# yudaohai666/Sparse_Matrix_Tuning

Hardware: AMD Instinct MI355X
Metric: train tokens/sec + peak GB HBM, LLaMA-3-8B SMT(0.71%) at 1/2/4/8 MI355X (higher is better)
Workload: dtype bf16

## Files before the change

### include/smt_attention.h

```cpp
#ifndef SMT_ATTENTION_H
#define SMT_ATTENTION_H

#include <stdint.h>
#include <hip/hip_runtime_api.h>

#ifdef __cplusplus
extern "C" {
#endif

#define SMT_ATTN_HEAD_DIM 128

typedef struct smt_attn_tensor {
    void* ptr;
    int64_t sb, sh, ss;
} smt_attn_tensor;

typedef struct smt_attn_shape {
    int32_t B, Hq, Hkv, S;
    float scale;
    int32_t dtype;
} smt_attn_shape;

const char* smt_attn_last_error(void);

int smt_attn_fwd(const smt_attn_tensor* q, const smt_attn_tensor* k, const smt_attn_tensor* v,
                 const smt_attn_tensor* o, float* lse, const smt_attn_shape* shape, hipStream_t stream);

int smt_attn_bwd(const smt_attn_tensor* q, const smt_attn_tensor* k, const smt_attn_tensor* v,
                 const smt_attn_tensor* o, const smt_attn_tensor* d_o, const float* lse, float* delta_ws,
                 const smt_attn_tensor* dq, const smt_attn_tensor* dk, const smt_attn_tensor* dv,
                 const smt_attn_shape* shape, hipStream_t stream);

int smt_attn_fwd_kmask(const smt_attn_tensor* q, const smt_attn_tensor* k, const smt_attn_tensor* v,
                       const smt_attn_tensor* o, float* lse, const uint64_t* key_mask, int64_t key_mask_ld,
                       const smt_attn_shape* shape, hipStream_t stream);
int smt_attn_bwd_kmask(const smt_attn_tensor* q, const smt_attn_tensor* k, const smt_attn_tensor* v,
                       const smt_attn_tensor* o, const smt_attn_tensor* d_o, const float* lse, float* delta_ws,
                       const smt_attn_tensor* dq, const smt_attn_tensor* dk, const smt_attn_tensor* dv,
                       const uint64_t* key_mask, int64_t key_mask_ld, const smt_attn_shape* shape,
                       hipStream_t stream);

#ifdef __cplusplus
}
#endif
#endif
```

### sparse_matrix_tuning_amd/_hip.py

```python
from __future__ import annotations

import ctypes
import os
import threading
from typing import NamedTuple, Optional, Sequence

import torch

from . import build as _build

BLOCK = 256
TILE_ELEMS = BLOCK * BLOCK

DTYPE_BF16, DTYPE_FP32, DTYPE_FP16 = 0, 1, 2
SCORE_MEAN_ABS, SCORE_ABS_MEAN, SCORE_L1, SCORE_L2 = 0, 1, 2, 3
ADAM_DEEPSPEED, ADAM_TORCH = 0, 1

_DT = {torch.bfloat16: DTYPE_BF16, torch.float32: DTYPE_FP32, torch.float16: DTYPE_FP16}
ABI_VERSION = 13

ABI_FUNCTIONS = (
    "smt_last_error", "smt_abi_version", "smt_wgrad_workspace_bytes", "smt_tile_wgrad", "smt_wgrad_batch_workspace_bytes",
    "smt_tile_wgrad_batch", "smt_wgrad_seq_workspace_bytes", "smt_tile_wgrad_batch_seq", "smt_colblock_gather", "smt_tile_scatter_t",
    "smt_tile_gather", "smt_tile_scatter", "smt_grad_accumulate", "smt_block_score",
    "smt_sq_norm", "smt_adamw_step", "smt_adamw_multi",
    "smt_mx_quant_cols", "smt_wgrad_mx_workspace_bytes", "smt_tile_wgrad_mx", "smt_tile_wgrad_mx_batch",
    "smt_row_gather", "smt_row_scatter", "smt_column_gather", "smt_act_accumulate",
    "smt_channel_score_workspace_bytes", "smt_channel_score",
    "smt_channel_mean_aten_workspace_bytes", "smt_channel_mean_aten",
    "smt_model_ops_last_error", "smt_rmsnorm_fwd", "smt_rmsnorm_bwd_waves", "smt_rmsnorm_bwd", "smt_rmsnorm_bwd_add_dw",
    "smt_add_rmsnorm_fwd", "smt_rmsnorm_bwd_add", "smt_colblock_recompute",
    "smt_rope_fwd", "smt_rope_bwd", "smt_swiglu_fwd", "smt_swiglu_bwd", "smt_ce_fwd", "smt_ce_bwd",
    "smt_attn_last_error", "smt_attn_fwd", "smt_attn_bwd", "smt_attn_fwd_kmask", "smt_attn_bwd_kmask",
    "smt_fp8_last_error", "smt_quant_rows_e4m3", "smt_quant_cols_t_e4m3", "smt_quant_rows_cat_e4m3",
    "smt_swiglu_fwd_quant_e4m3", "smt_swiglu_bwd_quant_e4m3", "smt_swiglu_bwd_quant_e4m3_packed",
    "smt_rmsnorm_fwd_quant_e4m3",
    "smt_rmsnorm_bwd_add_quant_e4m3",
)


class TileDesc(ctypes.Structure):
    _fields_ = [("weight", ctypes.c_void_p), ("ld_weight", ctypes.c_int64),
                ("row_block", ctypes.c_int32), ("col_block", ctypes.c_int32),
                ("flat_offset", ctypes.c_int64)]


class WgradModule(ctypes.Structure):
    _fields_ = [("grad_out", ctypes.c_void_p), ("x", ctypes.c_void_p), ("ld_grad_out", ctypes.c_int64),
                ("ld_x", ctypes.c_int64), ("x_block_stride", ctypes.c_int64), ("grad_tiles", ctypes.c_void_p),
                ("accumulate", ctypes.c_int32), ("operand_dtype", ctypes.c_int32)]


class WgradMxModule(ctypes.Structure):
    _fields_ = [("qg", ctypes.c_void_p), ("sg", ctypes.c_void_p), ("qx", ctypes.c_void_p), ("sx", ctypes.c_void_p),
                ("grad_tiles", ctypes.c_void_p), ("accumulate", ctypes.c_int32), ("reserved", ctypes.c_int32)]


WGRAD_MAX_MODULES = 16


class AccumEntry(ctypes.Structure):
    _fields_ = [("src", ctypes.c_void_p), ("dst", ctypes.c_void_p), ("n", ctypes.c_int64),
                ("chunk_begin", ctypes.c_int64), ("src_dtype", ctypes.c_int32), ("assign", ctypes.c_int32)]


class ScoreEntry(ctypes.Structure):
    _fields_ = [("src", ctypes.c_void_p), ("ld", ctypes.c_int64), ("d1", ctypes.c_int32),
                ("d2", ctypes.c_int32), ("block_begin", ctypes.c_int64), ("out", ctypes.c_void_p),
                ("strategy", ctypes.c_int32), ("pad_", ctypes.c_int32)]


class AdamWArgs(ctypes.Structure):
    _fields_ = [("lr", ctypes.c_float), ("beta1", ctypes.c_float), ("beta2", ctypes.c_float),
                ("eps", ctypes.c_float), ("weight_decay", ctypes.c_float),
                ("bias_correction1", ctypes.c_float), ("bias_correction2", ctypes.c_float),
                ("max_grad_norm", ctypes.c_float), ("grad_scale", ctypes.c_float),
                ("mode", ctypes.c_int32), ("grad_dtype", ctypes.c_int32),
                ("param_dtype", ctypes.c_int32), ("reserved", ctypes.c_int32)]


class AdamWTensor(ctypes.Structure):
    _fields_ = [("grad", ctypes.c_void_p), ("master", ctypes.c_void_p), ("exp_avg", ctypes.c_void_p),
                ("exp_avg_sq", ctypes.c_void_p), ("param", ctypes.c_void_p), ("n", ctypes.c_int64)]


class RopeTensor(ctypes.Structure):
    _fields_ = [("inp", ctypes.c_void_p), ("out", ctypes.c_void_p),
                ("in_sb", ctypes.c_int64), ("in_sh", ctypes.c_int64), ("in_ss", ctypes.c_int64),
                ("out_sb", ctypes.c_int64), ("out_sh", ctypes.c_int64), ("out_ss", ctypes.c_int64),
                ("heads", ctypes.c_int32), ("pad_", ctypes.c_int32)]


class QuantSrc(ctypes.Structure):
    _fields_ = [("ptr", ctypes.c_void_p), ("ld", ctypes.c_int64), ("cols", ctypes.c_int32), ("pad_", ctypes.c_int32)]


class AttnTensor(ctypes.Structure):
    _fields_ = [("ptr", ctypes.c_void_p), ("sb", ctypes.c_int64), ("sh", ctypes.c_int64), ("ss", ctypes.c_int64)]


class AttnShape(ctypes.Structure):
    _fields_ = [("B", ctypes.c_int32), ("Hq", ctypes.c_int32), ("Hkv", ctypes.c_int32), ("S", ctypes.c_int32),
                ("scale", ctypes.c_float), ("dtype", ctypes.c_int32)]


ACC_CHUNK = 4096
_lock = threading.Lock()
_lib: Optional[ctypes.CDLL] = None

_P, _I64, _I32, _SZ = ctypes.c_void_p, ctypes.c_int64, ctypes.c_int32, ctypes.c_size_t
_SIGS = {
    "smt_last_error": (ctypes.c_char_p, []),
    "smt_abi_version": (ctypes.c_int, []),
    "smt_wgrad_workspace_bytes": (_SZ, [_I64, _I32]),
    "smt_tile_wgrad": (ctypes.c_int, [_P, _I64, _P, _I64, _I64, _I64, _P, _P, _I32, _P, _I32, _I32, _P, _SZ, _P]),
    "smt_wgrad_batch_workspace_bytes": (_SZ, [_I64, _I32]),
    "smt_tile_wgrad_batch": (ctypes.c_int, [ctypes.POINTER(WgradModule), _I32, _I64, _P, _P, _I32, _I32, _P, _SZ, _P]),
    "smt_wgrad_seq_workspace_bytes": (_SZ, [_I64, _I64, _I32]),
    "smt_tile_wgrad_batch_seq": (ctypes.c_int, [ctypes.POINTER(WgradModule), _I32, _I64, _I64, _P, _P, _I32, _I32, _P,
                                                _SZ, _P]),
    "smt_colblock_gather": (ctypes.c_int, [_P, _I64, _I64, _P, _I32, _P, _P]),
    "smt_tile_scatter_t": (ctypes.c_int, [_P, _I32, _P, _P]),
    "smt_tile_gather": (ctypes.c_int, [_P, _I64, _I32, _P, _I32, _P, _P]),
    "smt_tile_scatter": (ctypes.c_int, [_P, _I64, _I32, _P, _I32, _P, _P]),
    "smt_grad_accumulate": (ctypes.c_int, [_P, _I32, _I64, _P]),
    "smt_block_score": (ctypes.c_int, [_P, _I32, _I64, _P]),
    "smt_sq_norm": (ctypes.c_int, [_P, _I64, _P, _I32, _P, _P]),
    "smt_adamw_step": (ctypes.c_int, [_P, _P, _P, _P, _P, _P, _I32, _I64, _P, ctypes.POINTER(AdamWArgs), _P]),
    "smt_adamw_multi": (ctypes.c_int, [_P, _P, _I32, _I64, _P, ctypes.POINTER(AdamWArgs), _P]),
    "smt_mx_quant_cols": (ctypes.c_int, [_P, _I64, _I64, _P, _I32, _I64, _P, _P, _P]),
    "smt_wgrad_mx_workspace_bytes": (_SZ, [_I64, _I32]),
    "smt_tile_wgrad_mx": (ctypes.c_int, [_P, _P, _P, _P, _I64, _P, _P, _I32, _P, _I32, _I32, _P, _SZ, _P]),
    "smt_tile_wgrad_mx_batch": (ctypes.c_int, [ctypes.POINTER(WgradMxModule), _I32, _I64, _P, _P, _I32, _I32, _P, _SZ, _P]),
    "smt_row_gather": (ctypes.c_int, [_P, _I64, _I32, _I64, _P, _I32, _P, _I64, _P]),
    "smt_row_scatter": (ctypes.c_int, [_P, _I64, _I32, _I64, _P, _I32, _P, _I64, _P]),
    "smt_column_gather": (ctypes.c_int, [_P, _I64, _I64, _I64, _P, _I32, _P, _I64, _P]),
    "smt_act_accumulate": (ctypes.c_int, [_P, _I32, _I64, _I64, _I32, _I32, _I32, _P, _I32, _P]),
    "smt_channel_score_workspace_bytes": (_SZ, [_I32, _I32]),
    "smt_channel_score": (ctypes.c_int, [_P, _I32, _I32, _I32, _I32, _P, _SZ, _P, _P]),
    "smt_channel_mean_aten_workspace_bytes": (_SZ, [_I32, _I32]),
    "smt_channel_mean_aten": (ctypes.c_int, [_P, _I32, _I32, _I32, _P, _SZ, _P, _P]),
    "smt_attn_last_error": (ctypes.c_char_p, []),
    "smt_attn_fwd": (ctypes.c_int, [ctypes.POINTER(AttnTensor)] * 4 + [_P, ctypes.POINTER(AttnShape), _P]),
    "smt_attn_bwd": (ctypes.c_int, [ctypes.POINTER(AttnTensor)] * 5 + [_P, _P] + [ctypes.POINTER(AttnTensor)] * 3
                     + [ctypes.POINTER(AttnShape), _P]),
    "smt_attn_fwd_kmask": (ctypes.c_int, [ctypes.POINTER(AttnTensor)] * 4 + [_P, _P, _I64, ctypes.POINTER(AttnShape), _P]),
    "smt_attn_bwd_kmask": (ctypes.c_int, [ctypes.POINTER(AttnTensor)] * 5 + [_P, _P] + [ctypes.POINTER(AttnTensor)] * 3
                           + [_P, _I64, ctypes.POINTER(AttnShape), _P]),
    "smt_model_ops_last_error": (ctypes.c_char_p, []),
    "smt_rmsnorm_fwd": (ctypes.c_int, [_P, _I64, _P, _P, _I64, _P, _I64, _I32, ctypes.c_float, _I32, _P]),
    "smt_rmsnorm_bwd_waves": (ctypes.c_int, [_I64]),
    "smt_add_rmsnorm_fwd": (ctypes.c_int, [_P, _I64, _P, _I64, _P, _P, _I64, _P, _I64, _P, _I64, _I32, ctypes.c_float,
                                           _I32, _P]),
    "smt_rmsnorm_bwd_add": (ctypes.c_int, [_P, _I64, _P, _I64, _P, _P, _P, _I64, _P, _I64, _I64, _I32, _I32, _P]),
    "smt_rmsnorm_bwd": (ctypes.c_int, [_P, _I64, _P, _I64, _P, _P, _P, _I64, _P, _P, _I64, _I32, _I32, _P]),
    "smt_rmsnorm_bwd_add_dw": (ctypes.c_int, [_P, _I64, _P, _I64, _P, _P, _P, _I64, _P, _I64, _P, _P, _I64, _I32, _I32, _P]),
    "smt_rope_fwd": (ctypes.c_int, [ctypes.POINTER(RopeTensor), ctypes.POINTER(RopeTensor), _P, _P, _I64, _I64, _I64, _I32,
                                    _I32, _I32, _P]),
    "smt_rope_bwd": (ctypes.c_int, [ctypes.POINTER(RopeTensor), ctypes.POINTER(RopeTensor), _P, _P, _I64, _I64, _I64, _I32,
                                    _I32, _I32, _P]),
    "smt_swiglu_fwd": (ctypes.c_int, [_P, _P, _P, _I64, _I32, _P]),
    "smt_colblock_recompute": (ctypes.c_int, [_I32, _P, _I64, _P, _I64, _P, _P, _I64, _P, _I32, _P, _I32, _P]),
    "smt_swiglu_bwd": (ctypes.c_int, [_P, _P, _P, _P, _P, _I64, _I32, _P]),
    "smt_ce_fwd": (ctypes.c_int, [_P, _I64, _P, _I64, _I64, _I64, _P, _P, _I32, _P]),
    "smt_ce_bwd": (ctypes.c_int, [_P, _I64, _P, _P, _P, _I64, _I64, _I64, _P, _I64, _I32, _P]),
    "smt_fp8_last_error": (ctypes.c_char_p, []),
    "smt_quant_rows_e4m3": (ctypes.c_int, [_P, _I64, _I64, _I32, _P, _I32, _P, _I64, _P, _P]),
    "smt_quant_cols_t_e4m3": (ctypes.c_int, [_P, _I64, _I32, _I32, _P, _I32, _P, _I64, _P, _P]),
    "smt_quant_rows_cat_e4m3": (ctypes.c_int, [ctypes.POINTER(QuantSrc), _I32, _I64, _P, _I64, _P, _P]),
    "smt_rmsnorm_fwd_quant_e4m3": (ctypes.c_int, [_P, _I64, _P, _I64, _P, _P, _I64, _P, _I64, _P, _P, _I64, _P,
                                                   _I64, _I32, ctypes.c_float, _P]),
    "smt_rmsnorm_bwd_add_quant_e4m3": (ctypes.c_int, [_P, _I64, _P, _I64, _P, _P, _P, _I64, _P, _I64, _P, _I64, _P,
                                                       _I64, _I32, _P]),
    "smt_swiglu_fwd_quant_e4m3": (ctypes.c_int, [_P, _P, _I64, _I32, _P, _I64, _P, _P, _P]),
    "smt_swiglu_bwd_quant_e4m3": (ctypes.c_int, [_P, _P, _P, _I64, _I32, _P, _I64, _P, _P, _P, _P]),
    "smt_swiglu_bwd_quant_e4m3_packed": (ctypes.c_int, [_P, _P, _P, _I64, _I32, _P, _I64, _P, _P, _P, _I64, _P, _P,
                                                         _I64, _P]),
}


def dtype_code16(dtype: torch.dtype, what: str) -> int:
    if dtype == torch.bfloat16:
        return DTYPE_BF16
    if dtype == torch.float16:
        return DTYPE_FP16
    raise RuntimeError(f"{what}: bf16 or fp16 tensors only (got {dtype})")


def lib_path() -> str:
    return _build.LIB_PATH


def load(build_if_missing: bool = False) -> ctypes.CDLL:
    global _lib
    if _lib is not None:
        return _lib
    with _lock:
        if _lib is None:
            if build_if_missing and _build.is_stale():
                _build.build()
            path = os.environ.get("SMT_HIP_LIB") or _build.LIB_PATH
            if not os.path.exists(path):
                raise RuntimeError(
                    f"SMT HIP library not built ({path}); run `python -c 'import __graft_entry__ as g; g.build()'`"
                    " or `python -m sparse_matrix_tuning_amd.build`")
            lib = ctypes.CDLL(path)
            for name, (res, args) in _SIGS.items():
                fn = getattr(lib, name)
                fn.restype = res
                fn.argtypes = args
            if lib.smt_abi_version() != ABI_VERSION:
                raise RuntimeError(f"{path} implements C ABI v{lib.smt_abi_version()}, this package v{ABI_VERSION}: "
                                   "rebuild it (`python -c 'import __graft_entry__ as g; g.build()'`)")
            _lib = lib
    return _lib


def _check(rc: int, what: str) -> None:
    if rc != 0:
        lib = load()
        if what.startswith(("smt_quant", "smt_swiglu_fwd_quant", "smt_swiglu_bwd_quant")):
            err = lib.smt_fp8_last_error
        elif what.startswith(("smt_rmsnorm", "smt_add_rmsnorm", "smt_rope", "smt_swiglu", "smt_ce_",
                              "smt_colblock_recompute")):
            err = lib.smt_model_ops_last_error
        elif what.startswith("smt_attn"):
            err = lib.smt_attn_last_error
        else:
            err = lib.smt_last_error
        raise RuntimeError(f"{what} failed (status {rc}): {err().decode(errors='replace')}")


def _require_device(*tensors: torch.Tensor) -> torch.device:
    dev = None
    for t in tensors:
        if t is None:
            continue
        if t.device.type != "cuda":
            raise RuntimeError(
                f"SMT HIP path needs tensors on a ROCm device, got {t.device} "
                "(there is no CPU fallback: the CPU restatement lives in oracle/ and is test-only)")
        if dev is None:
            dev = t.device
        elif t.device != dev:
            raise RuntimeError(f"tensors on different devices: {dev} vs {t.device}")
    return dev


def _stream(dev: torch.device) -> int:
    return torch.cuda.current_stream(dev).cuda_stream


def _ptr(t: Optional[torch.Tensor]) -> Optional[int]:
    return None if t is None else t.data_ptr()


def _device_table(structs: Sequence[ctypes.Structure], cls, dev: torch.device) -> torch.Tensor:
    n = len(structs)
    arr = (cls * n)(*structs)
    host = torch.frombuffer(bytearray(bytes(arr)), dtype=torch.uint8)
    return host.to(dev, non_blocking=False)


def tile_table(index_list: Sequence[Sequence[int]], device: torch.device) -> torch.Tensor:
    flat = [int(v) for rc in index_list for v in (rc[0], rc[1])]
    return torch.tensor(flat, dtype=torch.int32).view(-1, 2).to(device)


def schedule_order(index_list: Sequence[Sequence[int]]) -> list:
    rows = {int(rc[0]) for rc in index_list}
    cols = {int(rc[1]) for rc in index_list}
    if len(cols) <= len(rows):
        key = lambda i: (int(index_list[i][1]), int(index_list[i][0]))
    else:
        key = lambda i: (int(index_list[i][0]), int(index_list[i][1]))
    return sorted(range(len(index_list)), key=key)


def order_table(index_list: Sequence[Sequence[int]], device: torch.device) -> torch.Tensor:
    return torch.tensor(schedule_order(index_list), dtype=torch.int32).to(device)


def wgrad_workspace_bytes(T: int, n_tiles: int) -> int:
    return int(load().smt_wgrad_workspace_bytes(int(T), int(n_tiles)))


def tile_wgrad(grad_out2d: torch.Tensor, x: torch.Tensor, tile_rc: torch.Tensor, out: torch.Tensor,
               accumulate: bool = False, order: Optional[torch.Tensor] = None,
               seq_len: Optional[int] = None) -> torch.Tensor:
    if grad_out2d.dtype != torch.bfloat16 and grad_out2d.shape[0] == 0:
        if not accumulate:
            out.zero_()
        return out
    if seq_len or grad_out2d.dtype != torch.bfloat16:
        n = tile_rc.shape[0]
        tab = torch.zeros(n, 4, dtype=torch.int32, device=tile_rc.device)
        tab[:, 1:3] = tile_rc
        tab[:, 3] = torch.arange(n, dtype=torch.int32, device=tile_rc.device)
        tile_wgrad_batch([(grad_out2d, x, out, accumulate)], tab, order, seq_len=seq_len)
        return out
    dev = _require_device(grad_out2d, x, tile_rc, out, order)
    if grad_out2d.dtype != torch.bfloat16 or x.dtype != torch.bfloat16:
        raise NotImplementedError(f"tile_wgrad: bf16 operands only (got {grad_out2d.dtype}, {x.dtype})")
    if out.dtype not in (torch.bfloat16, torch.float32) or not out.is_contiguous():
        raise ValueError("tile_wgrad: out must be a contiguous bf16/fp32 tensor")
    n = tile_rc.shape[0]
    if out.numel() != n * TILE_ELEMS:
        raise ValueError(f"tile_wgrad: out has {out.numel()} elements, expected {n * TILE_ELEMS}")
    T = grad_out2d.shape[0]
    if x.dim() == 3:
        if not x.is_contiguous() or x.shape[1:] != (T, BLOCK):
            raise ValueError("tile_wgrad: a block-major x must be a contiguous [n_cb, T, 256] tensor")
        ld_x, xbs = BLOCK, T * BLOCK
    else:
        if x.dim() != 2 or x.shape[0] != T or x.stride(1) != 1:
            raise ValueError("tile_wgrad: x must be [T, features] with unit feature stride")
        ld_x, xbs = x.stride(0), BLOCK
    if grad_out2d.stride(1) != 1:
        raise ValueError("tile_wgrad: grad_out must be [T, features] with unit feature stride")
    ws_bytes = wgrad_workspace_bytes(T, n)
    ws = torch.empty(max(ws_bytes, 16), dtype=torch.uint8, device=dev)
    if order is not None and (order.dtype != torch.int32 or order.numel() != n):
        raise ValueError("tile_wgrad: order must be int32 [n_tiles]")
    rc = load().smt_tile_wgrad(_ptr(grad_out2d), grad_out2d.stride(0), _ptr(x), ld_x, xbs, T,
                               _ptr(tile_rc), _ptr(order), n, _ptr(out), _DT[out.dtype], int(bool(accumulate)),
                               _ptr(ws), ws_bytes, _stream(dev))
    _check(rc, "smt_tile_wgrad")
    return out


def _wgrad_x_layout(x: torch.Tensor, T: int, what: str):
    if x.dim() == 3:
        if not x.is_contiguous() or x.shape[1:] != (T, BLOCK):
            raise ValueError(f"{what}: a block-major x must be a contiguous [n_cb, T, 256] tensor")
        return BLOCK, T * BLOCK
    if x.dim() != 2 or x.shape[0] != T or x.stride(1) != 1:
        raise ValueError(f"{what}: x must be [T, features] with unit feature stride")
    return x.stride(0), BLOCK


def tile_wgrad_batch(items: Sequence[tuple], tile_tab: torch.Tensor, order: Optional[torch.Tensor] = None,
                     seq_len: Optional[int] = None) -> None:
    if not items:
        return
    if len(items) > WGRAD_MAX_MODULES:
        raise ValueError(f"tile_wgrad_batch: {len(items)} modules > {WGRAD_MAX_MODULES}")
    dev = _require_device(tile_tab, order, *[t for it in items for t in it[:3]])
    T = items[0][0].shape[0]
    out_dtype = items[0][2].dtype
    op_dtype = items[0][0].dtype
    if op_dtype not in (torch.bfloat16, torch.float16, torch.float32):
        raise NotImplementedError(f"tile_wgrad_batch: operands bf16, fp16 or fp32 (got {op_dtype})")
    if out_dtype not in (op_dtype, torch.float32) or out_dtype == torch.float64:
        raise ValueError(f"tile_wgrad_batch: {op_dtype} operands give {op_dtype} or fp32 tiles (got {out_dtype})")
    mods = (WgradModule * len(items))()
    for i, (g, x, out, acc) in enumerate(items):
        if g.dtype != op_dtype or x.dtype != op_dtype:
            raise NotImplementedError(f"tile_wgrad_batch: one operand dtype per launch (got {g.dtype}, {x.dtype})")
        if g.dim() != 2 or g.shape[0] != T or g.stride(1) != 1:
            raise ValueError("tile_wgrad_batch: every grad_out must be [T, features] with the same T")
        if out.dtype != out_dtype or not out.is_contiguous():
            raise ValueError("tile_wgrad_batch: outputs must be contiguous and of one dtype")
        ld_x, xbs = _wgrad_x_layout(x, T, "tile_wgrad_batch")
        mods[i] = WgradModule(_ptr(g), _ptr(x), g.stride(0), ld_x, xbs, _ptr(out), int(bool(acc)), _DT[op_dtype])
    if tile_tab.dtype != torch.int32 or tile_tab.dim() != 2 or tile_tab.shape[1] != 4:
        raise ValueError("tile_wgrad_batch: tile_tab must be int32 [n, 4]")
    n = tile_tab.shape[0]
    if order is not None and (order.dtype != torch.int32 or order.numel() != n):
        raise ValueError("tile_wgrad_batch: order must be int32 [n_tiles]")
    if seq_len:
        if T % int(seq_len):
            raise ValueError(f"tile_wgrad_batch: T = {T} is not a whole number of {seq_len}-row samples")
        ws_bytes = int(load().smt_wgrad_seq_workspace_bytes(T, int(seq_len), n))
        ws = torch.empty(max(ws_bytes, 16), dtype=torch.uint8, device=dev)
        rc = load().smt_tile_wgrad_batch_seq(mods, len(items), T, int(seq_len), _ptr(tile_tab), _ptr(order), n,
                                             _DT[out_dtype], _ptr(ws), ws_bytes, _stream(dev))
        _check(rc, "smt_tile_wgrad_batch_seq")
        return
    ws_bytes = int(load().smt_wgrad_batch_workspace_bytes(T, n))
    ws = torch.empty(max(ws_bytes, 16), dtype=torch.uint8, device=dev)
    rc = load().smt_tile_wgrad_batch(mods, len(items), T, _ptr(tile_tab), _ptr(order), n, _DT[out_dtype],
                                     _ptr(ws), ws_bytes, _stream(dev))
    _check(rc, "smt_tile_wgrad_batch")


def wgrad_batch_table(module_tiles: Sequence[Sequence[Sequence[int]]], device: torch.device):
    rows, order = [], []
    for m, tl in enumerate(module_tiles):
        base = len(rows)
        rows.extend((m, int(r), int(c), k) for k, (r, c) in enumerate(tl))
        order.extend(base + i for i in schedule_order(tl))
    flat = [v for row in rows for v in row]
    tab = torch.tensor(flat, dtype=torch.int32).view(-1, 4).to(device)
    return tab, torch.tensor(order, dtype=torch.int32).to(device)


def colblock_gather(x2d: torch.Tensor, col_blocks: torch.Tensor) -> torch.Tensor:
    dev = _require_device(x2d, col_blocks)
    if x2d.dim() != 2 or x2d.stride(1) != 1 or x2d.element_size() != 2:
        raise ValueError("colblock_gather: x must be a 2-D row-major 16-bit tensor")
    n_cb = col_blocks.numel()
    out = torch.empty(n_cb, x2d.shape[0], BLOCK, dtype=x2d.dtype, device=dev)
    rc = load().smt_colblock_gather(_ptr(x2d), x2d.stride(0), x2d.shape[0], _ptr(col_blocks), n_cb, _ptr(out),
                                    _stream(dev))
    _check(rc, "smt_colblock_gather")
    return out


RECOMPUTE_RMSNORM, RECOMPUTE_SWIGLU = 0, 1


def colblock_recompute(op: int, a2d: torch.Tensor, col_blocks: torch.Tensor, b2d: torch.Tensor = None,
                       weight: torch.Tensor = None, rstd: torch.Tensor = None) -> torch.Tensor:
    dev = _require_device(a2d, col_blocks, b2d, weight, rstd)
    for t in (a2d, b2d):
        if t is not None and (t.dim() != 2 or t.stride(1) != 1 or t.dtype not in (torch.bfloat16, torch.float16)):
            raise ValueError("colblock_recompute: operands must be 2-D row-major bf16 / fp16")
    if b2d is not None and b2d.dtype != a2d.dtype or weight is not None and weight.dtype != a2d.dtype:
        raise ValueError("colblock_recompute: operands of one dtype")
    if b2d is not None and b2d.shape != a2d.shape:
        raise ValueError("colblock_recompute: gate and up shapes differ")
    if rstd is not None and (rstd.dtype != torch.float32 or rstd.numel() != a2d.shape[0] or not rstd.is_contiguous()):
        raise ValueError("colblock_recompute: rstd must be a contiguous fp32 [T]")
    if weight is not None and (weight.numel() != a2d.shape[1] or not weight.is_contiguous()):
        raise ValueError("colblock_recompute: weight must be a contiguous [cols]")
    n_cb = col_blocks.numel()
    out = torch.empty(n_cb, a2d.shape[0], BLOCK, dtype=a2d.dtype, device=dev)
    rc = load().smt_colblock_recompute(op, _ptr(a2d), a2d.stride(0), _ptr(b2d) if b2d is not None else None,
                                       b2d.stride(0) if b2d is not None else 0,
                                       _ptr(weight) if weight is not None else None,
                                       _ptr(rstd) if rstd is not None else None, a2d.shape[0], _ptr(col_blocks), n_cb,
                                       _ptr(out), dtype_code16(a2d.dtype, "colblock_recompute"), _stream(dev))
    _check(rc, "smt_colblock_recompute")
    return out


class MxBlocks(NamedTuple):
    q: torch.Tensor
    scales: torch.Tensor
    T: int

    @property
    def ldq(self) -> int:
        return self.q.shape[1] * 64


def mx_ld(T: int) -> int:
    return (T + 63) // 64 * 64


def mx_quant_cols(x2d: torch.Tensor, blocks: torch.Tensor) -> MxBlocks:
# ... 304 lines not shown
```

### sparse_matrix_tuning_amd/build.py

```python
from __future__ import annotations

import os
import shutil
import subprocess
import sys

PKG_DIR = os.path.dirname(os.path.abspath(__file__))
REPO_DIR = os.path.dirname(PKG_DIR)
SRCS = [os.path.join(PKG_DIR, "csrc", n) for n in ("smt_kernels.hip", "llama_kernels.hip", "attn_kernels.hip",
                                                   "fp8_kernels.hip")]
HEADERS = [os.path.join(REPO_DIR, "include", n) for n in ("smt_hip.h", "smt_model_ops.h", "smt_attention.h",
                                                          "smt_fp8.h")]
HEADERS += [os.path.join(PKG_DIR, "csrc", n) for n in ("silu_math.h", "fp8_math.h")]
LIB_DIR = os.path.join(PKG_DIR, "_lib")
LIB_PATH = os.path.join(LIB_DIR, "libsmt_hip.so")
ARCH = "gfx950"


def hipcc() -> str:
    for cand in (os.environ.get("HIPCC"), "/opt/rocm/bin/hipcc", shutil.which("hipcc")):
        if cand and os.path.exists(cand):
            return cand
    raise RuntimeError("hipcc not found (set HIPCC or install ROCm under /opt/rocm)")


def is_stale() -> bool:
    if not os.path.exists(LIB_PATH):
        return True
    t = os.path.getmtime(LIB_PATH)
    return any(os.path.getmtime(p) > t for p in (*SRCS, *HEADERS, __file__))


FILE_FLAGS = {"attn_kernels.hip": ["-fno-slp-vectorize"]}


def compile_commands(out: str, defines=()) -> list:
    base = [hipcc(), f"--offload-arch={ARCH}", "-O3", "-std=c++17", "-fPIC", "-Wall", "-Wno-unused-function",
            "-I", os.path.join(REPO_DIR, "include"), *defines]
    objs, cmds = [], []
    for src in SRCS:
        obj = out + "." + os.path.splitext(os.path.basename(src))[0] + ".o"
        objs.append(obj)
        cmds.append(base + FILE_FLAGS.get(os.path.basename(src), []) + ["-c", "-o", obj, src])
    link = [hipcc(), f"--offload-arch={ARCH}", "-shared", "-fPIC", "-o", out, *objs]
    return cmds, link, objs


def run_build(out: str, defines=(), verbose: bool = False) -> None:
    cmds, link, objs = compile_commands(out, defines)
    if verbose:
        for c in cmds + [link]:
            print(" ".join(c), file=sys.stderr)
    procs = [subprocess.Popen(c, stdout=subprocess.PIPE, stderr=subprocess.PIPE, text=True) for c in cmds]
    errs = []
    for c, p in zip(cmds, procs):
        so, se = p.communicate()
        if p.returncode != 0:
            errs.append(f"{' '.join(c)}\n{so}\n{se}")
    if not errs:
        res = subprocess.run(link, capture_output=True, text=True)
        if res.returncode != 0:
            errs.append(f"{' '.join(link)}\n{res.stdout}\n{res.stderr}")
    for o in objs:
        if os.path.exists(o):
            os.remove(o)
    if errs:
        raise RuntimeError("hipcc failed:\n" + "\n".join(errs))


def build(force: bool = False, verbose: bool = False) -> str:
    if not force and not is_stale():
        return LIB_PATH
    os.makedirs(LIB_DIR, exist_ok=True)
    tmp = f"{LIB_PATH}.tmp{os.getpid()}"
    run_build(tmp, verbose=verbose)
    os.replace(tmp, LIB_PATH)
    return LIB_PATH


if __name__ == "__main__":
    print(build(force="--force" in sys.argv, verbose=True))
```

### sparse_matrix_tuning_amd/csrc/attn_kernels.hip

```cpp
#include <hip/hip_runtime.h>
#include <stdarg.h>
#include <stdint.h>
#include <stdio.h>
#include <stdlib.h>

#include <utility>

#include "smt_attention.h"
#include "smt_hip.h"

namespace {

thread_local char g_err[512] = "";

int fail(int code, const char* fmt, ...) {
    va_list ap;
    va_start(ap, fmt);
    vsnprintf(g_err, sizeof(g_err), fmt, ap);
    va_end(ap);
    return code;
}

int check_launch(const char* what) {
    hipError_t e = hipGetLastError();
    if (e != hipSuccess) return fail(-4, "%s: %s", what, hipGetErrorString(e));
    return 0;
}

typedef __bf16 bf16x8_t __attribute__((ext_vector_type(8)));
typedef __bf16 bf16x2_t __attribute__((ext_vector_type(2)));
typedef _Float16 f16x8_t __attribute__((ext_vector_type(8)));
typedef _Float16 f16x2_t __attribute__((ext_vector_type(2)));
typedef float f32x2_t __attribute__((ext_vector_type(2)));
typedef short s16x4_t __attribute__((ext_vector_type(4)));
typedef short s16x8_t __attribute__((ext_vector_type(8)));
typedef float f32x16_t __attribute__((ext_vector_type(16)));
typedef uint32_t u32x4_t __attribute__((ext_vector_type(4)));
typedef __attribute__((address_space(3))) s16x4_t lds_s16x4_t;

constexpr int kD = 128;
constexpr int kRowB = 256;
constexpr float kNegInf = -__builtin_huge_valf();

struct Tns {
    const uint16_t* p;
    int64_t sb, sh, ss;
};

__device__ __forceinline__ uint32_t swz(uint32_t row) { return ((row & 3u) << 2) | ((row >> 2) & 3u); }
__device__ __forceinline__ uint32_t lds_off(uint32_t row, uint32_t byte) { return row * kRowB + (byte ^ (swz(row) << 4)); }

__device__ __forceinline__ bf16x8_t row_frag(const uint8_t* img, uint32_t row, uint32_t byte) {
    return *reinterpret_cast<const bf16x8_t*>(img + lds_off(row, byte));
}

struct TrLane {
    uint32_t krow, feat_byte;
};
__device__ __forceinline__ TrLane tr_lane(int lane) {
    const int gi = lane >> 4, q = (lane >> 2) & 3, p = lane & 3;
    return TrLane{8u * (gi >> 1) + q, 2u * (16u * (gi & 1) + 4u * p)};
}
__device__ __forceinline__ bf16x8_t tr_frag(const uint8_t* img, TrLane tl, uint32_t row0, uint32_t col0) {
    const uint32_t r = row0 + tl.krow, byte = 2u * col0 + tl.feat_byte;
    s16x4_t lo = __builtin_amdgcn_ds_read_tr16_b64_v4i16((lds_s16x4_t*)(img + lds_off(r, byte)));
    s16x4_t hi = __builtin_amdgcn_ds_read_tr16_b64_v4i16((lds_s16x4_t*)(img + lds_off(r + 4, byte)));
    const s16x8_t both = __builtin_shufflevector(lo, hi, 0, 1, 2, 3, 4, 5, 6, 7);
    return __builtin_bit_cast(bf16x8_t, both);
}

template <int F>
__device__ __forceinline__ f32x16_t mfma(bf16x8_t a, bf16x8_t b, f32x16_t c) {
    if constexpr (F == SMT_DTYPE_FP16)
        return __builtin_amdgcn_mfma_f32_32x32x16_f16(__builtin_bit_cast(f16x8_t, a), __builtin_bit_cast(f16x8_t, b), c,
                                                      0, 0, 0);
    else return __builtin_amdgcn_mfma_f32_32x32x16_bf16(a, b, c, 0, 0, 0);
}

constexpr bool kPkFwd = false, kPkDq = true, kPkDkv = true;
template <bool PK>
__device__ __forceinline__ f32x2_t fma2(f32x2_t a, f32x2_t b, f32x2_t c) {
    if (PK) return __builtin_elementwise_fma(a, b, c);
    return f32x2_t{__builtin_fmaf(a.x, b.x, c.x), __builtin_fmaf(a.y, b.y, c.y)};
}
template <bool PK>
__device__ __forceinline__ f32x2_t submul2(f32x2_t a, f32x2_t d, f32x2_t p) {
    if (PK) return (a - d) * p;
    return f32x2_t{(a.x - d.x) * p.x, (a.y - d.y) * p.y};
}
template <bool PK>
__device__ __forceinline__ f32x2_t add2(f32x2_t a, f32x2_t b) {
    if (PK) return a + b;
    return f32x2_t{a.x + b.x, a.y + b.y};
}

template <int F>
__device__ __forceinline__ uint32_t pk16(float a, float b) {
    f32x2_t v = {a, b};
    if constexpr (F == SMT_DTYPE_FP16) return __builtin_bit_cast(uint32_t, __builtin_convertvector(v, f16x2_t));
    else return __builtin_bit_cast(uint32_t, __builtin_convertvector(v, bf16x2_t));
}
template <int F>
__device__ __forceinline__ float lo16(uint32_t w) {
    if constexpr (F == SMT_DTYPE_FP16) return (float)__builtin_bit_cast(_Float16, (uint16_t)(w & 0xffffu));
    else return __uint_as_float(w << 16);
}
template <int F>
__device__ __forceinline__ float hi16(uint32_t w) {
    if constexpr (F == SMT_DTYPE_FP16) return (float)__builtin_bit_cast(_Float16, (uint16_t)(w >> 16));
    else return __uint_as_float(w & 0xffff0000u);
}

__device__ __forceinline__ float other_half_max(float x) {
    auto r = __builtin_amdgcn_permlane32_swap(__float_as_uint(x), __float_as_uint(x), false, false);
    return fmaxf(__uint_as_float(r[0]), __uint_as_float(r[1]));
}
__device__ __forceinline__ float halves_sum(float x) {
    auto r = __builtin_amdgcn_permlane32_swap(__float_as_uint(x), __float_as_uint(x), false, false);
    return __uint_as_float(r[0]) + __uint_as_float(r[1]);
}

template <int F>
__device__ __forceinline__ void pack_b_frags(const float (&p)[16], bf16x8_t& f0, bf16x8_t& f1) {
    uint32_t w[8];
#pragma unroll
    for (int i = 0; i < 8; ++i) w[i] = pk16<F>(p[2 * i], p[2 * i + 1]);
#pragma unroll
    for (int h = 0; h < 2; ++h) {
        auto a = __builtin_amdgcn_permlane32_swap(w[4 * h + 0], w[4 * h + 2], false, false);
        auto b = __builtin_amdgcn_permlane32_swap(w[4 * h + 1], w[4 * h + 3], false, false);
        u32x4_t v = {a[0], b[0], a[1], b[1]};
        if (h == 0) f0 = __builtin_bit_cast(bf16x8_t, v);
        else f1 = __builtin_bit_cast(bf16x8_t, v);
    }
}

__device__ __forceinline__ int xcd_logical(int bid, int total) {
    const int q8 = total >> 3, r8 = total & 7, xcd = bid & 7;
    return (xcd < r8 ? xcd * (q8 + 1) : r8 * (q8 + 1) + (xcd - r8) * q8) + (bid >> 3);
}

__device__ __forceinline__ uint32_t opaque(uint32_t v) {
    asm volatile("" : "+v"(v));
    return v;
}
template <int IMG>
__device__ __forceinline__ bf16x8_t rowx(const uint8_t* lds, uint32_t lo, int ks) {
    return *reinterpret_cast<const bf16x8_t*>(lds + IMG + (lo ^ (uint32_t)(ks << 5)));
}
template <int IMG>
__device__ __forceinline__ bf16x8_t trx(const uint8_t* lds, uint32_t t0, uint32_t t4, int kq, int dt) {
    const uint32_t x = (uint32_t)(dt << 6);
    s16x4_t lo = __builtin_amdgcn_ds_read_tr16_b64_v4i16((lds_s16x4_t*)(lds + IMG + 4096 * kq + (t0 ^ x)));
    s16x4_t hi = __builtin_amdgcn_ds_read_tr16_b64_v4i16((lds_s16x4_t*)(lds + IMG + 4096 * kq + (t4 ^ x)));
    const s16x8_t both = __builtin_shufflevector(lo, hi, 0, 1, 2, 3, 4, 5, 6, 7);
    return __builtin_bit_cast(bf16x8_t, both);
}

typedef __attribute__((address_space(3))) uint8_t lds_u8_t;
__device__ __forceinline__ void dma16(__amdgpu_buffer_rsrc_t rsrc, uint32_t lds_base, int voff) {
    uint32_t keep;
    asm volatile("s_mov_b32 %0, m0\n\ts_mov_b32 m0, %3\n\ts_nop 0\n\t"
                 "buffer_load_dwordx4 %1, %2, 0 offen lds\n\ts_mov_b32 m0, %0"
                 : "=&s"(keep) : "v"(voff), "s"(rsrc), "s"(lds_base) : "memory");
}
__device__ __forceinline__ uint32_t lds_addr(const uint8_t* p) { return (uint32_t)(uintptr_t)(const lds_u8_t*)p; }
__device__ __forceinline__ __amdgpu_buffer_rsrc_t uniform_rsrc(const void* base, int64_t bytes) {
    const uint64_t a = (uint64_t)(uintptr_t)base;
    const uint32_t lo = __builtin_amdgcn_readfirstlane((uint32_t)a);
    const uint32_t hi = __builtin_amdgcn_readfirstlane((uint32_t)(a >> 32));
    const int n = __builtin_amdgcn_readfirstlane((int)bytes);
    return __builtin_amdgcn_make_buffer_rsrc((void*)(((uint64_t)hi << 32) | lo), 0, n, 0x00020000);
}
__device__ __forceinline__ void vm_wait_all() { asm volatile("s_waitcnt vmcnt(0)" ::: "memory"); }
__device__ __forceinline__ void vm_wait_all_known() { __builtin_amdgcn_s_waitcnt(0x0F70); }
__device__ __forceinline__ void vm_wait_upto(int n) {
    if (n >= 8) asm volatile("s_waitcnt vmcnt(8)" ::: "memory");
    else if (n >= 6) asm volatile("s_waitcnt vmcnt(6)" ::: "memory");
    else if (n >= 4) asm volatile("s_waitcnt vmcnt(4)" ::: "memory");
    else if (n >= 3) asm volatile("s_waitcnt vmcnt(3)" ::: "memory");
    else if (n >= 2) asm volatile("s_waitcnt vmcnt(2)" ::: "memory");
    else asm volatile("s_waitcnt vmcnt(0)" ::: "memory");
}

__device__ __forceinline__ void dma_rows(__amdgpu_buffer_rsrc_t rsrc, int64_t ss, uint32_t img, int img_row0,
                                         int row0, int pieces, int lane) {
#pragma unroll 4
    for (int i = 0; i < pieces; ++i) {
        const int r = row0 + 4 * i + (lane >> 4);
        const uint32_t ir = (uint32_t)(r - img_row0);
        const uint32_t ch = (uint32_t)(lane & 15) ^ swz(ir);
        const uint32_t base = __builtin_amdgcn_readfirstlane(img + (uint32_t)(r - (lane >> 4) - img_row0) * kRowB);
        dma16(rsrc, base, (int)((int64_t)r * ss * 2 + ch * 16));
    }
}

constexpr int kFwdQW = 32, kFwdWaves = 4, kFwdQB = kFwdQW * kFwdWaves, kKV = 64;
constexpr int kDqWaves = 4, kDqQB = kFwdQW * kDqWaves;
constexpr int kTileB = kKV * kRowB;

__device__ __forceinline__ bool key_bit(uint64_t w, int key) { return (w >> (key & 63)) & 1ull; }

struct FwdArgs {
    Tns q, k, v;
    uint16_t* o;
    int64_t o_sb, o_sh, o_ss;
    float* lse;
    const uint64_t* kmask;
    int64_t kmask_ld;
    int B, Hq, Hkv, S;
    float sl2;
};

struct PairTask {
    int b, hk, hh, blk[2], n;
};
__device__ __forceinline__ PairTask pair_task(int L, int nblk, int G, int Hkv) {
    const int npair = (nblk + 1) / 2;
    const int per_group = G * npair;
    const int grp = L / per_group;
    const int rem = L - grp * per_group;
    const int p = rem / G;
    PairTask t;
    t.b = grp / Hkv;
    t.hk = grp % Hkv;
    t.hh = rem % G;
    t.blk[0] = nblk - 1 - p;
    t.blk[1] = p;
    t.n = (t.blk[1] == t.blk[0]) ? 1 : 2;
    return t;
}

constexpr float kFwdThr = 8.f;


__device__ __forceinline__ float max3f(float a, float b, float c) {
    float r;
    asm("v_max3_f32 %0, %1, %2, %3" : "=v"(r) : "v"(a), "v"(b), "v"(c));
    return r;
}

template <bool KMASK, int F>
struct FwdLean {
    const FwdArgs& a;
    uint8_t* lds;
    __amdgpu_buffer_rsrc_t rk, rv;
    uint32_t lds0;
    const uint64_t* km;
    bf16x8_t qf[8];
    f32x16_t o[4];
    float m_run, l_run;
    int qw, qrow, hi, l32, wave, lane, nt, last;
    TrLane tl;

    __device__ __forceinline__ FwdLean(const FwdArgs& a_, uint8_t* lds_) : a(a_), lds(lds_) {}

    __device__ __forceinline__ void issue(int t) {
        const uint32_t slot = lds0 + (uint32_t)((t & 1) * 2 * kTileB);
        dma_rows(rk, a.k.ss, slot, t * kKV, t * kKV + 16 * wave, 4, lane);
        dma_rows(rv, a.v.ss, slot + kTileB, t * kKV, t * kKV + 16 * wave, 4, lane);
    }

    template <int SLOT, bool DIAG_>
    __device__ __forceinline__ void compute(int t, bool DIAG) {
        const uint8_t* K = lds + SLOT * 2 * kTileB;
        const uint8_t* V = K + kTileB;
        const int k0 = t * kKV;
        f32x16_t sc[2];
        bf16x8_t kf[3][2];
#pragma unroll
        for (int p = 0; p < 2; ++p)
#pragma unroll
            for (int j = 0; j < 2; ++j) kf[p][j] = row_frag(K, 32 * j + l32, 32 * p + 16 * hi);
#pragma unroll
        for (int ks = 0; ks < 8; ++ks) {
            if (ks + 2 < 8) {
#pragma unroll
                for (int j = 0; j < 2; ++j) kf[(ks + 2) % 3][j] = row_frag(K, 32 * j + l32, 32 * (ks + 2) + 16 * hi);
            }
            __builtin_amdgcn_sched_barrier(0);
#pragma unroll
            for (int j = 0; j < 2; ++j) sc[j] = mfma<F>(kf[ks % 3][j], qf[ks], ks ? sc[j] : f32x16_t{});
            __builtin_amdgcn_sched_barrier(0);
        }
        bf16x8_t vf[3];
        vf[0] = tr_frag(V, tl, 0, 0);
        vf[1] = tr_frag(V, tl, 16, 0);
        float x[32];
#pragma unroll
        for (int j = 0; j < 2; ++j)
#pragma unroll
            for (int i = 0; i < 16; ++i) x[16 * j + i] = sc[j][i];
        if (DIAG) {
#pragma unroll
            for (int i = 0; i < 32; ++i) {
                const int key = k0 + 32 * (i >> 4) + (i & 3) + 8 * ((i & 15) >> 2) + 4 * hi;
                if (key > qrow) x[i] = kNegInf;
            }
        }
        if (KMASK) {
            const uint64_t w = km[k0 >> 6];
            if (~w != 0ull) {
#pragma unroll
                for (int i = 0; i < 32; ++i) {
                    const int key = k0 + 32 * (i >> 4) + (i & 3) + 8 * ((i & 15) >> 2) + 4 * hi;
                    if (!key_bit(w, key)) x[i] = kNegInf;
                }
            }
        }
        float mx[11];
#pragma unroll
        for (int i = 0; i < 10; ++i) mx[i] = max3f(x[3 * i], x[3 * i + 1], x[3 * i + 2]);
        mx[10] = max3f(x[30], x[31], mx[0]);
        mx[0] = max3f(mx[0], mx[1], mx[2]);
        mx[3] = max3f(mx[3], mx[4], mx[5]);
        mx[6] = max3f(mx[6], mx[7], mx[8]);
        mx[9] = max3f(mx[9], mx[10], mx[0]);
        const float m_tile = other_half_max(max3f(mx[3], mx[6], mx[9])) * a.sl2;
        const bool move = m_tile > m_run + kFwdThr;
        const float m_new = move ? m_tile : m_run;
        const float alpha = move ? __builtin_amdgcn_exp2f(m_run - m_new) : 1.f;
        const float m_use = (KMASK && m_new == kNegInf) ? 0.f : m_new;
        const f32x2_t sl2v = {a.sl2, a.sl2}, mv = {-m_use, -m_use};
        f32x2_t sm[16];
#pragma unroll
        for (int i = 0; i < 16; ++i) {
            const f32x2_t e = fma2<kPkFwd>(f32x2_t{x[2 * i], x[2 * i + 1]}, sl2v, mv);
            x[2 * i] = __builtin_amdgcn_exp2f(e.x);
            x[2 * i + 1] = __builtin_amdgcn_exp2f(e.y);
            sm[i] = f32x2_t{x[2 * i], x[2 * i + 1]};
        }
#pragma unroll
        for (int w = 8; w >= 1; w >>= 1)
#pragma unroll
            for (int i = 0; i < w; ++i) sm[i] = add2<kPkFwd>(sm[i], sm[i + w]);
        l_run = l_run * alpha + (sm[0].x + sm[0].y);
        m_run = m_new;
        if (__builtin_amdgcn_ballot_w64(move) != 0) {
#pragma unroll
            for (int dt = 0; dt < 4; ++dt)
#pragma unroll
                for (int i = 0; i < 16; ++i) o[dt][i] *= alpha;
        }
        bf16x8_t pf[4];
        pack_b_frags<F>(*reinterpret_cast<const float(*)[16]>(&x[0]), pf[0], pf[1]);
        pack_b_frags<F>(*reinterpret_cast<const float(*)[16]>(&x[16]), pf[2], pf[3]);
#pragma unroll
        for (int n = 0; n < 16; ++n) {
            if (n + 2 < 16) vf[(n + 2) % 3] = tr_frag(V, tl, 16 * ((n + 2) & 3), 32 * ((n + 2) >> 2));
            __builtin_amdgcn_sched_barrier(0);
            o[n >> 2] = mfma<F>(vf[n % 3], pf[n & 3], o[n >> 2]);
            __builtin_amdgcn_sched_barrier(0);
        }
    }

    template <int SLOT>
    __device__ __forceinline__ void tile(int t) {
        if (t + 1 < nt) issue(t + 1);
        if (t <= last) compute<SLOT, true>(t, t == last);
        vm_wait_all();
        __syncthreads();
    }

    __device__ __forceinline__ void run(int b, int h, int hk, int qb) {
        const int tid = threadIdx.x;
        lane = tid & 63;
        wave = __builtin_amdgcn_readfirstlane(tid >> 6);
        hi = lane >> 5;
        l32 = lane & 31;
        const int q0 = qb * kFwdQB;
        qw = q0 + wave * kFwdQW;
        qrow = qw + l32;
        const uint16_t* qp = a.q.p + b * a.q.sb + h * a.q.sh;
        const uint16_t* kp = a.k.p + b * a.k.sb + hk * a.k.sh;
        const uint16_t* vp = a.v.p + b * a.v.sb + hk * a.v.sh;
        km = KMASK ? a.kmask + (int64_t)b * a.kmask_ld : nullptr;
#pragma unroll
        for (int ks = 0; ks < 8; ++ks) {
            if (qrow < a.S) qf[ks] = *reinterpret_cast<const bf16x8_t*>(qp + qrow * a.q.ss + 16 * ks + 8 * hi);
            else qf[ks] = __builtin_bit_cast(bf16x8_t, u32x4_t{0u, 0u, 0u, 0u});
        }
        const int kv_end = min(a.S, q0 + kFwdQB);
        nt = (kv_end + kKV - 1) / kKV;
        last = min(nt - 1, qw / kKV);
        rk = uniform_rsrc(kp, (int64_t)a.S * a.k.ss * 2);
        rv = uniform_rsrc(vp, (int64_t)a.S * a.v.ss * 2);
        lds0 = lds_addr(lds);
        tl = tr_lane(lane);
#pragma unroll
        for (int dt = 0; dt < 4; ++dt)
#pragma unroll
            for (int i = 0; i < 16; ++i) o[dt][i] = 0.f;
        m_run = kNegInf;
        l_run = 0.f;
        issue(0);
        vm_wait_all();
        vm_wait_all_known();
        __syncthreads();
        for (int t = 0; t < nt; t += 2) {
            tile<0>(t);
            if (t + 1 < nt) tile<1>(t + 1);
        }
        const float l_tot = halves_sum(l_run);
        if (qrow < a.S) {
            const float inv = (KMASK && !(l_tot > 0.f)) ? 0.f : 1.f / l_tot;
            uint16_t* op = a.o + b * a.o_sb + h * a.o_sh + (int64_t)qrow * a.o_ss;
#pragma unroll
            for (int dt = 0; dt < 4; ++dt)
#pragma unroll
                for (int g = 0; g < 4; ++g) {
                    const int d = 32 * dt + 8 * g + 4 * hi;
                    uint2 w;
                    w.x = pk16<F>(o[dt][4 * g] * inv, o[dt][4 * g + 1] * inv);
                    w.y = pk16<F>(o[dt][4 * g + 2] * inv, o[dt][4 * g + 3] * inv);
                    *reinterpret_cast<uint2*>(op + d) = w;
                }
            if (hi == 0)
                a.lse[((int64_t)b * a.Hq + h) * a.S + qrow] =
                    (KMASK && !(l_tot > 0.f)) ? __builtin_huge_valf() : m_run + __log2f(l_tot);
        }
    }
};

template <bool KMASK, int F>
__global__ __launch_bounds__(64 * kFwdWaves, 2)
void attn_fwd_kernel(FwdArgs a) {
    __shared__ __attribute__((aligned(16))) uint8_t lds[2 * 2 * kTileB];
    const int nqb = (a.S + kFwdQB - 1) / kFwdQB;
    const int G = a.Hq / a.Hkv;
    const int total = nqb * a.Hq * a.B;
    const int L = xcd_logical(blockIdx.x, total);
    const int per_group = G * nqb;
    const int grp = L / per_group;
    const int rem = L - grp * per_group;
    const int hk = grp % a.Hkv;
    FwdLean<KMASK, F> fl(a, lds);
    fl.run(grp / a.Hkv, hk * G + rem % G, hk, nqb - 1 - rem / G);
}


struct DqArgs {
    Tns q, k, v, dout, o;
    uint16_t* dq;
    int64_t dq_sb, dq_sh, dq_ss;
    const float* lse;
    float* delta;
    const uint64_t* kmask;
    int64_t kmask_ld;
    int B, Hq, Hkv, S;
    float sl2, scale;
};

template <bool KMASK, int F>
struct DqLean {
    const DqArgs& a;
    uint8_t* lds;
    bf16x8_t qf[8], df[8];
    f32x16_t dq[4];
    float lse, dlt;
    const uint64_t* km;
    __amdgpu_buffer_rsrc_t rk, rv;
    uint32_t lds0, lo_row, lo_t0, lo_t4;
    int lane, wave, hi, l32, qw, qrow, nt, last;

    __device__ __forceinline__ DqLean(const DqArgs& a_, uint8_t* lds_) : a(a_), lds(lds_) {}

    __device__ __forceinline__ void issue(int t) {
        const uint32_t slot = lds0 + (uint32_t)((t & 1) * 2 * kTileB);
        constexpr int rows_w = kKV / kDqWaves;
        dma_rows(rk, a.k.ss, slot, t * kKV, t * kKV + rows_w * wave, rows_w / 4, lane);
        dma_rows(rv, a.v.ss, slot + kTileB, t * kKV, t * kKV + rows_w * wave, rows_w / 4, lane);
    }

    template <int SLOT>
    __device__ __forceinline__ void compute(int t, bool diag) {
        constexpr int KI = SLOT * 2 * kTileB, VI = KI + kTileB;
        const int k0 = t * kKV;
        const uint32_t lr = opaque(lo_row);
        constexpr int KH = KI + 32 * kRowB, VH = VI + 32 * kRowB;
        f32x16_t s[2], dp[2];
        s[0] = mfma<F>(rowx<KI>(lds, lr, 0), qf[0], f32x16_t{});
        s[1] = mfma<F>(rowx<KH>(lds, lr, 0), qf[0], f32x16_t{});
        dp[0] = mfma<F>(rowx<VI>(lds, lr, 0), df[0], f32x16_t{});
        dp[1] = mfma<F>(rowx<VH>(lds, lr, 0), df[0], f32x16_t{});
#pragma unroll
        for (int ks = 1; ks < 8; ++ks) {
            s[0] = mfma<F>(rowx<KI>(lds, lr, ks), qf[ks], s[0]);
            s[1] = mfma<F>(rowx<KH>(lds, lr, ks), qf[ks], s[1]);
            dp[0] = mfma<F>(rowx<VI>(lds, lr, ks), df[ks], dp[0]);
            dp[1] = mfma<F>(rowx<VH>(lds, lr, ks), df[ks], dp[1]);
            if (ks & 1) __builtin_amdgcn_sched_barrier(0);
        }
        float pr[32];
        const f32x2_t sl2v = {a.sl2, a.sl2}, lv = {-lse, -lse}, dv = {dlt, dlt};
#pragma unroll
        for (int i = 0; i < 32; i += 2) {
            const int j = i >> 4, ii = i & 15;
            const f32x2_t e = fma2<kPkDq>(f32x2_t{s[j][ii], s[j][ii + 1]}, sl2v, lv);
            pr[i] = __builtin_amdgcn_exp2f(e.x);
            pr[i + 1] = __builtin_amdgcn_exp2f(e.y);
        }
        if (diag) {
#pragma unroll
            for (int i = 0; i < 32; ++i) {
                const int key = k0 + 32 * (i >> 4) + (i & 3) + 8 * ((i & 15) >> 2) + 4 * hi;
                if (key > qrow) pr[i] = 0.f;
            }
        }
        if (KMASK) {
            const uint64_t w = km[k0 >> 6];
            if (~w != 0ull) {
#pragma unroll
                for (int i = 0; i < 32; ++i) {
                    const int key = k0 + 32 * (i >> 4) + (i & 3) + 8 * ((i & 15) >> 2) + 4 * hi;
                    if (!key_bit(w, key)) pr[i] = 0.f;
                }
            }
        }
#pragma unroll
        for (int i = 0; i < 32; i += 2) {
            const int j = i >> 4, ii = i & 15;
            const f32x2_t r = submul2<kPkDq>(f32x2_t{dp[j][ii], dp[j][ii + 1]}, dv, f32x2_t{pr[i], pr[i + 1]});
            pr[i] = r.x;
            pr[i + 1] = r.y;
        }
        bf16x8_t sf[4];
        pack_b_frags<F>(*reinterpret_cast<const float(*)[16]>(&pr[0]), sf[0], sf[1]);
        pack_b_frags<F>(*reinterpret_cast<const float(*)[16]>(&pr[16]), sf[2], sf[3]);
        const uint32_t t0 = opaque(lo_t0), t4 = opaque(lo_t4);
#pragma unroll
        for (int dt = 0; dt < 4; ++dt) {
#pragma unroll
            for (int kst = 0; kst < 4; ++kst) dq[dt] = mfma<F>(trx<KI>(lds, t0, t4, kst, dt), sf[kst], dq[dt]);
            __builtin_amdgcn_sched_barrier(0);
        }
    }

    template <int SLOT>
    __device__ __forceinline__ void tile(int t) {
        if (t + 1 < nt) issue(t + 1);
        if (t <= last) compute<SLOT>(t, t == last);
        vm_wait_all();
        __syncthreads();
    }

    __device__ __forceinline__ void run(int b, int h, int hk, int qb) {
        const int tid = threadIdx.x;
        lane = tid & 63;
        wave = __builtin_amdgcn_readfirstlane(tid >> 6);
        hi = lane >> 5;
        l32 = lane & 31;
        const int q0 = qb * kDqQB;
        qw = q0 + wave * kFwdQW;
        qrow = qw + l32;
        const bool qvalid = qrow < a.S;
        const uint16_t* qp = a.q.p + b * a.q.sb + h * a.q.sh;
        const uint16_t* dop = a.dout.p + b * a.dout.sb + h * a.dout.sh;
        const uint16_t* kp = a.k.p + b * a.k.sb + hk * a.k.sh;
        const uint16_t* vp = a.v.p + b * a.v.sb + hk * a.v.sh;
        km = KMASK ? a.kmask + (int64_t)b * a.kmask_ld : nullptr;
#pragma unroll
        for (int ks = 0; ks < 8; ++ks) {
            if (qvalid) {
                qf[ks] = *reinterpret_cast<const bf16x8_t*>(qp + qrow * a.q.ss + 16 * ks + 8 * hi);
                df[ks] = *reinterpret_cast<const bf16x8_t*>(dop + qrow * a.dout.ss + 16 * ks + 8 * hi);
            } else {
                qf[ks] = __builtin_bit_cast(bf16x8_t, u32x4_t{0u, 0u, 0u, 0u});
                df[ks] = qf[ks];
            }
        }
        const int64_t srow = ((int64_t)b * a.Hq + h) * a.S + (qvalid ? qrow : 0);
        lse = qvalid ? a.lse[srow] : 0.f;
        {
            const uint16_t* op = a.o.p + b * a.o.sb + h * a.o.sh;
            float part = 0.f;
#pragma unroll
            for (int ks = 0; ks < 8; ++ks) {
                const u32x4_t ov = qvalid ? *reinterpret_cast<const u32x4_t*>(op + qrow * a.o.ss + 16 * ks + 8 * hi)
                                          : u32x4_t{0u, 0u, 0u, 0u};
                const u32x4_t dv = __builtin_bit_cast(u32x4_t, df[ks]);
#pragma unroll
                for (int j = 0; j < 4; ++j) {
                    part += lo16<F>(ov[j]) * lo16<F>(dv[j]);
                    part += hi16<F>(ov[j]) * hi16<F>(dv[j]);
                }
            }
            dlt = halves_sum(part);
            if (qvalid && hi == 0) a.delta[srow] = dlt;
        }
        const int kv_end = min(a.S, q0 + kDqQB);
        nt = (kv_end + kKV - 1) / kKV;
        last = min(nt - 1, qw / kKV);
        rk = uniform_rsrc(kp, (int64_t)a.S * a.k.ss * 2);
        rv = uniform_rsrc(vp, (int64_t)a.S * a.v.ss * 2);
        lds0 = lds_addr(lds);
        {
            const uint32_t r = (uint32_t)l32;
            lo_row = r * kRowB + ((16u * hi) ^ (swz(r) << 4));
            const TrLane tl = tr_lane(lane);
            lo_t0 = tl.krow * kRowB + (tl.feat_byte ^ (swz(tl.krow) << 4));
            lo_t4 = (tl.krow + 4) * kRowB + (tl.feat_byte ^ (swz(tl.krow + 4) << 4));
        }
#pragma unroll
        for (int dt = 0; dt < 4; ++dt)
#pragma unroll
            for (int i = 0; i < 16; ++i) dq[dt][i] = 0.f;
        if (nt > 0) issue(0);
        vm_wait_all();
        vm_wait_all_known();
        __syncthreads();
        for (int t = 0; t < nt; t += 2) {
            tile<0>(t);
            if (t + 1 < nt) tile<1>(t + 1);
        }
        if (qvalid) {
            uint16_t* out = a.dq + b * a.dq_sb + h * a.dq_sh + (int64_t)qrow * a.dq_ss;
#pragma unroll
            for (int dt = 0; dt < 4; ++dt)
#pragma unroll
                for (int g = 0; g < 4; ++g) {
                    const int d = 32 * dt + 8 * g + 4 * hi;
                    uint2 w;
                    w.x = pk16<F>(dq[dt][4 * g] * a.scale, dq[dt][4 * g + 1] * a.scale);
                    w.y = pk16<F>(dq[dt][4 * g + 2] * a.scale, dq[dt][4 * g + 3] * a.scale);
                    *reinterpret_cast<uint2*>(out + d) = w;
                }
        }
    }
};

template <bool KMASK, int F>
__global__ __launch_bounds__(64 * kDqWaves, 8 / kDqWaves)
void attn_dq_kernel(DqArgs a) {
    __shared__ __attribute__((aligned(16))) uint8_t lds[2 * 2 * kTileB];
    const int nqb = (a.S + kDqQB - 1) / kDqQB;
    const int G = a.Hq / a.Hkv;
    const int total = nqb * a.Hq * a.B;
    const int L = xcd_logical(blockIdx.x, total);
    const int per_group = G * nqb;
    const int grp = L / per_group;
    const int rem = L - grp * per_group;
    const int hk = grp % a.Hkv;
    DqLean<KMASK, F> dl(a, lds);
    dl.run(grp / a.Hkv, hk * G + rem % G, hk, nqb - 1 - rem / G);
}

constexpr int kKB = 256, kKW = 32, kDkvWaves = kKB / kKW, kSlice = 32;
constexpr int kSliceB = kSlice * kRowB;
constexpr int kSliceBuf = 2 * kSliceB + 256;
constexpr int kVImg = kKB * kRowB;

struct DkvArgs {
    Tns q, k, v, dout;
    uint16_t* dk;
    int64_t dk_sb, dk_sh, dk_ss;
    uint16_t* dv;
    int64_t dv_sb, dv_sh, dv_ss;
    const float* lse;
    const float* delta;
    const uint64_t* kmask;
    int64_t kmask_ld;
    int B, Hq, Hkv, S;
    float sl2, scale;
};

constexpr int kDkvLeanRing = 2;
static_assert(kDkvLeanRing >= 2 && kDkvLeanRing * kSliceBuf + kVImg <= 160 * 1024, "dK/dV lean ring");
template <bool KMASK, int F>
struct DkvLean {
    const DkvArgs& a;
    uint8_t* lds;
    bf16x8_t kf[8];
    f32x16_t dvt[4], dkt[4];
    int G, lane, wave, hi, l32, k0, kw, key, n_sl, n_it, b, hk, per_slice;
    bool kvalid;
    uint32_t lds0;
    uint32_t lo_row, lo_v, lo_t0, lo_t4;

    __device__ __forceinline__ DkvLean(const DkvArgs& a_, uint8_t* lds_) : a(a_), lds(lds_) {}

    __device__ __forceinline__ void issue(int it) {
        const int hh = it / n_sl, sl = n_sl - 1 - (it - hh * n_sl);
        const int h = hk * G + hh;
        const int s0 = k0 + sl * kSlice;
        const uint32_t buf = lds0 + (uint32_t)((it % kDkvLeanRing) * kSliceBuf);
        if (kDkvWaves == 8) {
            const bool is_q = wave < 4;
            const Tns& src = is_q ? a.q : a.dout;
            const uint16_t* base = src.p + b * src.sb + h * src.sh;
            dma_rows(uniform_rsrc(base, (int64_t)a.S * src.ss * 2), src.ss, buf + (is_q ? 0u : (uint32_t)kSliceB), s0,
                     s0 + 8 * (wave & 3), 2, lane);
        } else {
            const uint16_t* qb = a.q.p + b * a.q.sb + h * a.q.sh;
            const uint16_t* db = a.dout.p + b * a.dout.sb + h * a.dout.sh;
            dma_rows(uniform_rsrc(qb, (int64_t)a.S * a.q.ss * 2), a.q.ss, buf, s0, s0 + 8 * wave, 2, lane);
            dma_rows(uniform_rsrc(db, (int64_t)a.S * a.dout.ss * 2), a.dout.ss, buf + (uint32_t)kSliceB, s0,
                     s0 + 8 * wave, 2, lane);
        }
        if (wave < 2 && lane < 8) {
            const float* row = (wave == 0 ? a.lse : a.delta) + ((int64_t)b * a.Hq + h) * a.S;
            dma16(uniform_rsrc(row, (int64_t)a.S * 4), __builtin_amdgcn_readfirstlane(buf + 2 * kSliceB + 128 * wave),
                  (s0 + 4 * lane) * 4);
        }
    }

    __device__ __forceinline__ int slice_s0(int it) const {
        const int sl = n_sl - 1 - it % n_sl;
        const int s0 = k0 + sl * kSlice;
        return (s0 + kSlice - 1 < kw) ? -1 : s0;
    }

    template <int SLOT>
    __device__ __forceinline__ void qk(f32x16_t& s, f32x16_t& dp) {
        constexpr int QI = SLOT * kSliceBuf, DI = QI + kSliceB;
        const uint32_t lr = opaque(lo_row), lv = opaque(lo_v);
        s = mfma<F>(rowx<QI>(lds, lr, 0), kf[0], f32x16_t{});
        dp = mfma<F>(rowx<DI>(lds, lr, 0), rowx<0>(lds, lv, 0), f32x16_t{});
#pragma unroll
        for (int ks = 1; ks < 8; ++ks) {
            s = mfma<F>(rowx<QI>(lds, lr, ks), kf[ks], s);
            dp = mfma<F>(rowx<DI>(lds, lr, ks), rowx<0>(lds, lv, ks), dp);
            if (ks & 1) __builtin_amdgcn_sched_barrier(0);
        }
    }

    template <int SLOT>
    __device__ __forceinline__ void pv(int s0, const f32x16_t& s, const f32x16_t& dp) {
        constexpr int QI = SLOT * kSliceBuf, DI = QI + kSliceB;
        const float* cst = reinterpret_cast<const float*>(lds + QI + 2 * kSliceB);
        float pr[16], dsv[16];
        const f32x2_t sl2v = {a.sl2, a.sl2};
#pragma unroll
        for (int g = 0; g < 4; ++g) {
            const float4 lz = *reinterpret_cast<const float4*>(cst + 8 * g + 4 * hi);
#pragma unroll
            for (int h = 0; h < 2; ++h) {
                const int i = 4 * g + 2 * h;
                const f32x2_t l2 = h ? f32x2_t{lz.z, lz.w} : f32x2_t{lz.x, lz.y};
                const f32x2_t e = fma2<kPkDkv>(f32x2_t{s[i], s[i + 1]}, sl2v, -l2);
                pr[i] = __builtin_amdgcn_exp2f(e.x);
                pr[i + 1] = __builtin_amdgcn_exp2f(e.y);
            }
        }
        if (s0 < kw + kKW - 1) {
#pragma unroll
            for (int i = 0; i < 16; ++i) {
                const int q = s0 + (i & 3) + 8 * (i >> 2) + 4 * hi;
                if (key > q) pr[i] = 0.f;
            }
        }
        if (KMASK && !kvalid) {
#pragma unroll
            for (int i = 0; i < 16; ++i) pr[i] = 0.f;
        }
#pragma unroll
        for (int g = 0; g < 4; ++g) {
            const float4 dz = *reinterpret_cast<const float4*>(cst + 32 + 8 * g + 4 * hi);
#pragma unroll
            for (int h = 0; h < 2; ++h) {
                const int i = 4 * g + 2 * h;
                const f32x2_t d2 = h ? f32x2_t{dz.z, dz.w} : f32x2_t{dz.x, dz.y};
                const f32x2_t r = submul2<kPkDkv>(f32x2_t{dp[i], dp[i + 1]}, d2, f32x2_t{pr[i], pr[i + 1]});
                dsv[i] = r.x;
                dsv[i + 1] = r.y;
            }
        }
        bf16x8_t pf[2], sf[2];
        pack_b_frags<F>(pr, pf[0], pf[1]);
        pack_b_frags<F>(dsv, sf[0], sf[1]);
        const uint32_t t0 = opaque(lo_t0), t4 = opaque(lo_t4);
#pragma unroll
        for (int dt = 0; dt < 4; ++dt)
#pragma unroll
            for (int kq = 0; kq < 2; ++kq) {
                dvt[dt] = mfma<F>(trx<DI>(lds, t0, t4, kq, dt), pf[kq], dvt[dt]);
                dkt[dt] = mfma<F>(trx<QI>(lds, t0, t4, kq, dt), sf[kq], dkt[dt]);
                if (kq) __builtin_amdgcn_sched_barrier(0);
            }
    }

    template <int SLOT>
    __device__ __forceinline__ void step(int it) {
        constexpr int R = kDkvLeanRing;
        if (it + R - 1 < n_it) issue(it + R - 1);
        const int s0 = slice_s0(it);
        if (s0 >= 0) {
            f32x16_t s, dp;
            qk<SLOT>(s, dp);
            pv<SLOT>(s0, s, dp);
        }
        vm_wait_upto(per_slice * max(0, min(R - 2, n_it - 2 - it)));
        __syncthreads();
    }

    template <int SLOT>
    __device__ __forceinline__ void steps(int it0) {
        if (it0 + SLOT < n_it) {
            step<SLOT>(it0 + SLOT);
            if constexpr (SLOT + 1 < kDkvLeanRing) steps<SLOT + 1>(it0);
        }
    }

    __device__ __forceinline__ void run(int b_, int hk_, int kb) {
        b = b_;
        hk = hk_;
        G = a.Hq / a.Hkv;
        const int tid = threadIdx.x;
        lane = tid & 63;
        wave = __builtin_amdgcn_readfirstlane(tid >> 6);
        hi = lane >> 5;
        l32 = lane & 31;
        k0 = kb * kKB;
        kw = k0 + wave * kKW;
        key = kw + l32;
        kvalid = !KMASK || (key < a.S && key_bit(a.kmask[(int64_t)b * a.kmask_ld + (key >> 6)], key));
        const uint16_t* kp = a.k.p + b * a.k.sb + hk * a.k.sh;
        const uint16_t* vp = a.v.p + b * a.v.sb + hk * a.v.sh;
        lds0 = lds_addr(lds);
        dma_rows(uniform_rsrc(vp, (int64_t)a.S * a.v.ss * 2), a.v.ss, lds0 + kDkvLeanRing * kSliceBuf, k0, kw, kKW / 4, lane);
        {
            const uint32_t r = (uint32_t)l32;
            lo_row = r * kRowB + ((16u * hi) ^ (swz(r) << 4));
            lo_v = lo_row + (uint32_t)(kDkvLeanRing * kSliceBuf + wave * kKW * kRowB);
            const TrLane tl = tr_lane(lane);
            lo_t0 = tl.krow * kRowB + (tl.feat_byte ^ (swz(tl.krow) << 4));
            lo_t4 = (tl.krow + 4) * kRowB + (tl.feat_byte ^ (swz(tl.krow + 4) << 4));
        }
#pragma unroll
        for (int ks = 0; ks < 8; ++ks) {
            if (key < a.S) kf[ks] = *reinterpret_cast<const bf16x8_t*>(kp + (int64_t)key * a.k.ss + 16 * ks + 8 * hi);
            else kf[ks] = __builtin_bit_cast(bf16x8_t, u32x4_t{0u, 0u, 0u, 0u});
        }
        n_sl = (a.S - k0 + kSlice - 1) / kSlice;
        n_it = G * n_sl;
#pragma unroll
        for (int dt = 0; dt < 4; ++dt)
#pragma unroll
            for (int i = 0; i < 16; ++i) { dvt[dt][i] = 0.f; dkt[dt][i] = 0.f; }
        per_slice = (kDkvWaves == 8 ? 2 : 4) + (wave < 2 ? 1 : 0);
#pragma unroll
        for (int i = 0; i < kDkvLeanRing - 1; ++i)
            if (i < n_it) issue(i);
        vm_wait_all();
        vm_wait_all_known();
        __syncthreads();
        for (int it = 0; it < n_it; it += kDkvLeanRing) steps<0>(it);
        if (key < a.S) {
            uint16_t* dkr = a.dk + b * a.dk_sb + hk * a.dk_sh + (int64_t)key * a.dk_ss;
            uint16_t* dvr = a.dv + b * a.dv_sb + hk * a.dv_sh + (int64_t)key * a.dv_ss;
#pragma unroll
            for (int dt = 0; dt < 4; ++dt)
#pragma unroll
                for (int g = 0; g < 4; ++g) {
                    const int d = 32 * dt + 8 * g + 4 * hi;
                    uint2 w;
                    w.x = pk16<F>(dkt[dt][4 * g] * a.scale, dkt[dt][4 * g + 1] * a.scale);
                    w.y = pk16<F>(dkt[dt][4 * g + 2] * a.scale, dkt[dt][4 * g + 3] * a.scale);
                    *reinterpret_cast<uint2*>(dkr + d) = w;
                    w.x = pk16<F>(dvt[dt][4 * g], dvt[dt][4 * g + 1]);
                    w.y = pk16<F>(dvt[dt][4 * g + 2], dvt[dt][4 * g + 3]);
                    *reinterpret_cast<uint2*>(dvr + d) = w;
                }
        }
    }
};

template <bool KMASK, int F>
__global__ __launch_bounds__(kDkvWaves * 64, 2)
void attn_dkdv_kernel(DkvArgs a) {
    __shared__ __attribute__((aligned(16))) uint8_t lds[kVImg + kDkvLeanRing * kSliceBuf];
    const int nkb = (a.S + kKB - 1) / kKB;
    const int total = ((nkb + 1) / 2) * a.Hkv * a.B;
    const PairTask t = pair_task(xcd_logical(blockIdx.x, total), nkb, 1, a.Hkv);
#pragma nounroll
    for (int i = 0; i < t.n; ++i) {
        if (i) __syncthreads();
        DkvLean<KMASK, F> dl(a, lds);
        dl.run(t.b, t.hk, t.blk[1 - i]);
    }
}

inline bool al16(const void* p) { return (reinterpret_cast<uintptr_t>(p) & 15u) == 0; }

int check_tensor(const smt_attn_tensor* t, const char* what, const char* fn) {
    if (!t || !t->ptr) return fail(-1, "%s: null %s", fn, what);
    if (!al16(t->ptr) || (t->sb & 7) || (t->sh & 7) || (t->ss & 7))
        return fail(-2, "%s: %s needs 16-byte aligned rows (strides %% 8 == 0)", fn, what);
    return 0;
}

int check_shape(const smt_attn_shape* s, const char* fn) {
    if (!s) return fail(-1, "%s: null shape", fn);
    if (s->B <= 0 || s->Hq <= 0 || s->Hkv <= 0 || s->S <= 0 || s->Hq % s->Hkv)
        return fail(-1, "%s: bad shape B=%d Hq=%d Hkv=%d S=%d", fn, s->B, s->Hq, s->Hkv, s->S);
    if (!(s->scale > 0.f)) return fail(-1, "%s: scale must be > 0", fn);
    if (s->dtype != SMT_DTYPE_BF16 && s->dtype != SMT_DTYPE_FP16)
        return fail(-1, "%s: dtype %d is not a 16-bit format (SMT_DTYPE_BF16 / SMT_DTYPE_FP16)", fn, (int)s->dtype);
    return 0;
}

#define SMT_ATTN_LAUNCH(kernel, kmask, dtype, grid, block, stream, args)                                         \
    do {                                                                                                      \
        if ((dtype) == SMT_DTYPE_FP16) {                                                                      \
            if (kmask) hipLaunchKernelGGL((kernel<true, SMT_DTYPE_FP16>), grid, block, 0, stream, args);     \
            else hipLaunchKernelGGL((kernel<false, SMT_DTYPE_FP16>), grid, block, 0, stream, args);          \
        } else {                                                                                              \
            if (kmask) hipLaunchKernelGGL((kernel<true, SMT_DTYPE_BF16>), grid, block, 0, stream, args);     \
            else hipLaunchKernelGGL((kernel<false, SMT_DTYPE_BF16>), grid, block, 0, stream, args);          \
        }                                                                                                     \
    } while (0)

Tns tns(const smt_attn_tensor* t) { return Tns{static_cast<const uint16_t*>(t->ptr), t->sb, t->sh, t->ss}; }

}

extern "C" {

const char* smt_attn_last_error(void) { return g_err; }


int smt_attn_fwd_kmask(const smt_attn_tensor* q, const smt_attn_tensor* k, const smt_attn_tensor* v,
                       const smt_attn_tensor* o, float* lse, const uint64_t* key_mask, int64_t key_mask_ld,
                       const smt_attn_shape* shape, hipStream_t stream) {
    int rc;
    const char* fn = key_mask ? "smt_attn_fwd_kmask" : "smt_attn_fwd";
    if ((rc = check_shape(shape, fn)) || (rc = check_tensor(q, "q", fn)) || (rc = check_tensor(k, "k", fn)) ||
        (rc = check_tensor(v, "v", fn)) || (rc = check_tensor(o, "o", fn)))
        return rc;
    if (!lse) return fail(-1, "%s: null lse", fn);
    if (key_mask && key_mask_ld < (shape->S + 63) / 64)
        return fail(-1, "%s: key_mask_ld %lld < ceil(S / 64)", fn, (long long)key_mask_ld);
    FwdArgs a;
    a.q = tns(q); a.k = tns(k); a.v = tns(v);
    a.o = static_cast<uint16_t*>(o->ptr); a.o_sb = o->sb; a.o_sh = o->sh; a.o_ss = o->ss;
    a.lse = lse;
    a.kmask = key_mask; a.kmask_ld = key_mask_ld;
    a.B = shape->B; a.Hq = shape->Hq; a.Hkv = shape->Hkv; a.S = shape->S;
    a.sl2 = shape->scale * 1.4426950408889634f;
    const int64_t nqb = (shape->S + kFwdQB - 1) / kFwdQB;
    const int64_t blocks = nqb * shape->Hq * shape->B;
    if (blocks > 0x7fffffffLL) return fail(-1, "%s: too many blocks", fn);
    SMT_ATTN_LAUNCH(attn_fwd_kernel, key_mask, shape->dtype, dim3((unsigned)blocks), dim3(64 * kFwdWaves), stream, a);
    return check_launch("attn_fwd_kernel");
}

int smt_attn_fwd(const smt_attn_tensor* q, const smt_attn_tensor* k, const smt_attn_tensor* v,
                 const smt_attn_tensor* o, float* lse, const smt_attn_shape* shape, hipStream_t stream) {
    return smt_attn_fwd_kmask(q, k, v, o, lse, nullptr, 0, shape, stream);
}

int smt_attn_bwd_kmask(const smt_attn_tensor* q, const smt_attn_tensor* k, const smt_attn_tensor* v,
                       const smt_attn_tensor* o, const smt_attn_tensor* d_o, const float* lse, float* delta_ws,
                       const smt_attn_tensor* dq, const smt_attn_tensor* dk, const smt_attn_tensor* dv,
                       const uint64_t* key_mask, int64_t key_mask_ld, const smt_attn_shape* shape,
                       hipStream_t stream) {
    int rc;
    const char* fn = key_mask ? "smt_attn_bwd_kmask" : "smt_attn_bwd";
    if ((rc = check_shape(shape, fn)) || (rc = check_tensor(q, "q", fn)) || (rc = check_tensor(k, "k", fn)) ||
        (rc = check_tensor(v, "v", fn)) || (rc = check_tensor(o, "o", fn)) || (rc = check_tensor(d_o, "do", fn)) ||
        (rc = check_tensor(dq, "dq", fn)) || (rc = check_tensor(dk, "dk", fn)) || (rc = check_tensor(dv, "dv", fn)))
        return rc;
    if (!lse || !delta_ws) return fail(-1, "%s: null lse / delta workspace", fn);
    if (!al16(lse) || !al16(delta_ws) || (shape->S & 3)) return fail(-2, "%s: lse / delta need 16-byte rows (S %% 4 == 0)", fn);
    if (key_mask && key_mask_ld < (shape->S + 63) / 64)
        return fail(-1, "%s: key_mask_ld %lld < ceil(S / 64)", fn, (long long)key_mask_ld);
    const int B = shape->B, Hq = shape->Hq, Hkv = shape->Hkv, S = shape->S;
    const float sl2 = shape->scale * 1.4426950408889634f;

    DqArgs qa;
    qa.q = tns(q); qa.k = tns(k); qa.v = tns(v); qa.dout = tns(d_o); qa.o = tns(o);
    qa.dq = static_cast<uint16_t*>(dq->ptr); qa.dq_sb = dq->sb; qa.dq_sh = dq->sh; qa.dq_ss = dq->ss;
    qa.lse = lse; qa.delta = delta_ws;
    qa.kmask = key_mask; qa.kmask_ld = key_mask_ld;
    qa.B = B; qa.Hq = Hq; qa.Hkv = Hkv; qa.S = S; qa.sl2 = sl2; qa.scale = shape->scale;
    const int64_t nqb = (S + kDqQB - 1) / kDqQB;
    const dim3 qgrid((unsigned)(nqb * Hq * B)), qblock(64 * kDqWaves);
    SMT_ATTN_LAUNCH(attn_dq_kernel, key_mask, shape->dtype, qgrid, qblock, stream, qa);
    if ((rc = check_launch("attn_dq_kernel"))) return rc;

    DkvArgs ka;
    ka.q = tns(q); ka.k = tns(k); ka.v = tns(v); ka.dout = tns(d_o);
    ka.dk = static_cast<uint16_t*>(dk->ptr); ka.dk_sb = dk->sb; ka.dk_sh = dk->sh; ka.dk_ss = dk->ss;
    ka.dv = static_cast<uint16_t*>(dv->ptr); ka.dv_sb = dv->sb; ka.dv_sh = dv->sh; ka.dv_ss = dv->ss;
    ka.lse = lse; ka.delta = delta_ws;
    ka.kmask = key_mask; ka.kmask_ld = key_mask_ld;
    ka.B = B; ka.Hq = Hq; ka.Hkv = Hkv; ka.S = S; ka.sl2 = sl2; ka.scale = shape->scale;
    const int64_t nkb = (S + kKB - 1) / kKB;
    const dim3 grid((unsigned)(((nkb + 1) / 2) * Hkv * B));
    SMT_ATTN_LAUNCH(attn_dkdv_kernel, key_mask, shape->dtype, grid, dim3(kDkvWaves * 64), stream, ka);
    return check_launch("attn_dkdv_kernel");
}

int smt_attn_bwd(const smt_attn_tensor* q, const smt_attn_tensor* k, const smt_attn_tensor* v,
                 const smt_attn_tensor* o, const smt_attn_tensor* d_o, const float* lse, float* delta_ws,
                 const smt_attn_tensor* dq, const smt_attn_tensor* dk, const smt_attn_tensor* dv,
                 const smt_attn_shape* shape, hipStream_t stream) {
    return smt_attn_bwd_kmask(q, k, v, o, d_o, lse, delta_ws, dq, dk, dv, nullptr, 0, shape, stream);
}

}
```

### sparse_matrix_tuning_amd/csrc/llama_kernels.hip

```cpp

#include <hip/hip_runtime.h>
#include <stdint.h>
#include <stdarg.h>
#include <stdio.h>

#include "smt_hip.h"
#include "smt_model_ops.h"
#include "silu_math.h"
#include "fp8_math.h"
#include "smt_fp8.h"

namespace {

thread_local char g_err[512] = "";

int fail(int code, const char* fmt, ...) {
    va_list ap;
    va_start(ap, fmt);
    vsnprintf(g_err, sizeof(g_err), fmt, ap);
    va_end(ap);
    return code;
}

int check_launch(const char* what) {
    hipError_t e = hipGetLastError();
    if (e != hipSuccess) return fail(-4, "%s: %s", what, hipGetErrorString(e));
    return 0;
}

inline bool aligned16(const void* p) { return (reinterpret_cast<uintptr_t>(p) & 15u) == 0; }

template <int F> __device__ __forceinline__ float u2f(uint32_t b16) {
    if constexpr (F == SMT_DTYPE_FP16) return (float)__builtin_bit_cast(_Float16, (uint16_t)b16);
    else return __uint_as_float(b16 << 16);
}
template <int F> __device__ __forceinline__ uint32_t f2u(float f) {
    if constexpr (F == SMT_DTYPE_FP16) return (uint32_t)__builtin_bit_cast(uint16_t, (_Float16)f);
    else return (uint32_t)__builtin_bit_cast(uint16_t, (__bf16)f);
}
template <int F> __device__ __forceinline__ float rnd(float f) {
    uint32_t b = f2u<F>(f);
    if constexpr (F == SMT_DTYPE_FP16) asm("" : "+v"(b));
    return u2f<F>(b);
}

struct F8 { float v[8]; };

template <int F> __device__ __forceinline__ F8 unpack8(const uint4 a) {
    F8 r;
    const uint32_t w[4] = {a.x, a.y, a.z, a.w};
#pragma unroll
    for (int j = 0; j < 4; ++j) { r.v[2 * j] = u2f<F>(w[j] & 0xffffu); r.v[2 * j + 1] = u2f<F>(w[j] >> 16); }
    return r;
}

template <int F> __device__ __forceinline__ F8 ld8(const uint16_t* p) {
    return unpack8<F>(*reinterpret_cast<const uint4*>(p));
}

template <int F> __device__ __forceinline__ uint4 pack8(const F8& r) {
    uint32_t w[4];
#pragma unroll
    for (int j = 0; j < 4; ++j) w[j] = f2u<F>(r.v[2 * j]) | (f2u<F>(r.v[2 * j + 1]) << 16);
    return make_uint4(w[0], w[1], w[2], w[3]);
}

template <int F> __device__ __forceinline__ F8 rnd8(const F8& v) {
    F8 r;
#pragma unroll
    for (int j = 0; j < 8; ++j) r.v[j] = rnd<F>(v.v[j]);
    return r;
}
template <bool PACK, int F> struct RowReg;
template <int F> struct RowReg<false, F> {
    typedef F8 T;
    static __device__ __forceinline__ T keep(const uint4 raw) { return unpack8<F>(raw); }
    static __device__ __forceinline__ T put(const F8& v) { return v; }
    static __device__ __forceinline__ F8 get(const T& v) { return v; }
};
template <int F> struct RowReg<true, F> {
    typedef uint4 T;
    static __device__ __forceinline__ T keep(const uint4 raw) { return raw; }
    static __device__ __forceinline__ T put(const F8& v) { return pack8<F>(v); }
    static __device__ __forceinline__ F8 get(const T& v) { return unpack8<F>(v); }
};

template <int F> __device__ __forceinline__ void st8(uint16_t* p, const F8& r) {
    *reinterpret_cast<uint4*>(p) = pack8<F>(r);
}

__device__ __forceinline__ float wave_max_f(float v) {
#pragma unroll
    for (int off = 32; off > 0; off >>= 1) v = fmaxf(v, __shfl_xor(v, off, 64));
    return v;
}

__device__ __forceinline__ float wave_sum_f(float v) {
#pragma unroll
    for (int off = 32; off > 0; off >>= 1) v += __shfl_xor(v, off, 64);
    return v;
}

template <int F>
__global__ __launch_bounds__(256)
void rmsnorm_fwd_kernel(const uint16_t* __restrict__ x, int64_t ldx, const uint16_t* __restrict__ w,
                        uint16_t* __restrict__ y, int64_t ldy, float* __restrict__ rstd,
                        int64_t rows, int H, float eps) {
    const int lane = threadIdx.x & 63;
    const int64_t row = (int64_t)blockIdx.x * 4 + (threadIdx.x >> 6);
    if (row >= rows) return;
    const uint16_t* xr = x + row * ldx;
    const int nch = H >> 3;
    float ss = 0.f;
    for (int c = lane; c < nch; c += 64) {
        const F8 v = ld8<F>(xr + c * 8);
#pragma unroll
        for (int j = 0; j < 8; ++j) ss += v.v[j] * v.v[j];
    }
    ss = wave_sum_f(ss);
    const float r = 1.0f / sqrtf(ss / (float)H + eps);
    if (lane == 0) rstd[row] = r;
    uint16_t* yr = y + row * ldy;
    for (int c = lane; c < nch; c += 64) {
        const F8 v = ld8<F>(xr + c * 8);
        const F8 wv = ld8<F>(w + c * 8);
        F8 o;
#pragma unroll
        for (int j = 0; j < 8; ++j) o.v[j] = wv.v[j] * rnd<F>(v.v[j] * r);
        st8<F>(yr + c * 8, o);
    }
}

template <int F>
__global__ __launch_bounds__(256)
void rmsnorm_bwd_kernel(const uint16_t* __restrict__ dy, int64_t lddy, const uint16_t* __restrict__ x, int64_t ldx,
                        const uint16_t* __restrict__ w, const float* __restrict__ rstd,
                        uint16_t* __restrict__ dx, int64_t lddx, int64_t rows, int H) {
    const int lane = threadIdx.x & 63;
    const int64_t wave = (int64_t)blockIdx.x * 4 + (threadIdx.x >> 6);
    const int64_t n_waves = (int64_t)gridDim.x * 4;
    const int nch = H >> 3;
    for (int64_t row = wave; row < rows; row += n_waves) {
        const float r = rstd[row];
        const uint16_t* xr = x + row * ldx;
        const uint16_t* dyr = dy + row * lddy;
        float dot = 0.f;
        for (int c = lane; c < nch; c += 64) {
            const F8 xv = ld8<F>(xr + c * 8), gv = ld8<F>(dyr + c * 8), wv = ld8<F>(w + c * 8);
#pragma unroll
            for (int j = 0; j < 8; ++j) dot += rnd<F>(gv.v[j] * wv.v[j]) * xv.v[j];
        }
        dot = wave_sum_f(dot);
        const float coef = r * r * r * dot / (float)H;
        uint16_t* dxr = dx + row * lddx;
        for (int c = lane; c < nch; c += 64) {
            const F8 xv = ld8<F>(xr + c * 8), gv = ld8<F>(dyr + c * 8), wv = ld8<F>(w + c * 8);
            F8 o;
#pragma unroll
            for (int j = 0; j < 8; ++j) o.v[j] = r * rnd<F>(gv.v[j] * wv.v[j]) - xv.v[j] * coef;
            st8<F>(dxr + c * 8, o);
        }
    }
}

constexpr int kDwChunk = 64;

__global__ __launch_bounds__(256)
void rmsnorm_dw_chunk_kernel(float* __restrict__ partial, int64_t n_waves, int H) {
    const int col = blockIdx.x * 256 + threadIdx.x;
    if (col >= H) return;
    const int64_t r0 = (int64_t)blockIdx.y * kDwChunk;
    const int64_t r1 = r0 + kDwChunk < n_waves ? r0 + kDwChunk : n_waves;
    float s = 0.f;
    for (int64_t i = r0; i < r1; ++i) s += partial[i * H + col];
    partial[r0 * H + col] = s;
}

template <int F>
__global__ __launch_bounds__(256)
void rmsnorm_dw_kernel(const float* __restrict__ partial, int64_t n_waves, int H, uint16_t* __restrict__ dw) {
    const int col = blockIdx.x * 256 + threadIdx.x;
    if (col >= H) return;
    float s = 0.f;
    for (int64_t i = 0; i < n_waves; i += kDwChunk) s += partial[i * H + col];
    dw[col] = (uint16_t)f2u<F>(s);
}

template <int CPL, bool ADD, bool QUANT = false, int F = SMT_DTYPE_BF16>
__global__ __launch_bounds__(256)
void rmsnorm_fwd_reg_kernel(const uint16_t* __restrict__ x, int64_t ldx, const uint16_t* __restrict__ res, int64_t ldr,
                            const uint16_t* __restrict__ w, uint16_t* __restrict__ h, int64_t ldh,
                            uint16_t* __restrict__ y, int64_t ldy, float* __restrict__ rstd, int64_t rows, int H,
                            float eps, uint8_t* __restrict__ q8, int64_t ldq, float* __restrict__ qscale) {
    const int lane = threadIdx.x & 63;
    const int64_t row = (int64_t)blockIdx.x * 4 + (threadIdx.x >> 6);
    if (row >= rows) return;
    F8 v[CPL];
    float ss = 0.f;
#pragma unroll
    for (int k = 0; k < CPL; ++k) {
        const int c = lane + 64 * k;
        v[k] = ld8<F>(x + row * ldx + c * 8);
        if (ADD) {
            const F8 rv = ld8<F>(res + row * ldr + c * 8);
#pragma unroll
            for (int j = 0; j < 8; ++j) v[k].v[j] = rnd<F>(v[k].v[j] + rv.v[j]);
            st8<F>(h + row * ldh + c * 8, v[k]);
        }
#pragma unroll
        for (int j = 0; j < 8; ++j) ss += v[k].v[j] * v[k].v[j];
    }
    ss = wave_sum_f(ss);
    const float r = 1.0f / sqrtf(ss / (float)H + eps);
    if (lane == 0) rstd[row] = r;
    if (!QUANT) {
#pragma unroll
        for (int k = 0; k < CPL; ++k) {
            const int c = lane + 64 * k;
            const F8 wv = ld8<F>(w + c * 8);
            F8 o;
#pragma unroll
            for (int j = 0; j < 8; ++j) o.v[j] = wv.v[j] * rnd<F>(v[k].v[j] * r);
            st8<F>(y + row * ldy + c * 8, o);
        }
        return;
    }
    float amax = 0.f;
#pragma unroll
    for (int k = 0; k < CPL; ++k) {
        const int c = lane + 64 * k;
        const F8 wv = ld8<F>(w + c * 8);
#pragma unroll
        for (int j = 0; j < 8; ++j) {
            v[k].v[j] = rnd<F>(wv.v[j] * rnd<F>(v[k].v[j] * r));
            amax = fmaxf(amax, fabsf(v[k].v[j]));
        }
        if (y) st8<F>(y + row * ldy + c * 8, v[k]);
    }
    amax = wave_max_f(amax);
    const float scale = e4m3_scale(amax);
    if (lane == 0) qscale[row] = scale;
#pragma unroll
    for (int k = 0; k < CPL; ++k) {
        const int c = lane + 64 * k;
        uint2 o;
        o.x = pack4(qv(v[k].v[0], scale), qv(v[k].v[1], scale), qv(v[k].v[2], scale), qv(v[k].v[3], scale));
        o.y = pack4(qv(v[k].v[4], scale), qv(v[k].v[5], scale), qv(v[k].v[6], scale), qv(v[k].v[7], scale));
        *reinterpret_cast<uint2*>(q8 + row * ldq + c * 8) = o;
    }
}

template <int CPL, bool ADD, bool QUANT = false, int F = SMT_DTYPE_BF16>
__global__ __launch_bounds__(256, CPL <= 10 ? 2 : 1)
void rmsnorm_bwd_reg_kernel(const uint16_t* __restrict__ dy, int64_t lddy, const uint16_t* __restrict__ x, int64_t ldx,
                            const uint16_t* __restrict__ w, const float* __restrict__ rstd,
                            const uint16_t* __restrict__ dres, int64_t lddr, uint16_t* __restrict__ dx, int64_t lddx,
                            int64_t rows, int H, uint8_t* __restrict__ q8 = nullptr, int64_t ldq = 0,
                            float* __restrict__ qscale = nullptr) {
    const int lane = threadIdx.x & 63;
    const int64_t row = (int64_t)blockIdx.x * 4 + (threadIdx.x >> 6);
    if (row >= rows) return;
    const float r = rstd[row];
    constexpr bool PACK = CPL > 8;
    typename RowReg<PACK, F>::T xr[CPL], gr[CPL];
    constexpr bool PRE = ADD && !PACK;
    uint4 drr[PRE ? CPL : 1];
    if constexpr (PRE) {
#pragma unroll
        for (int k = 0; k < CPL; ++k) drr[k] = *reinterpret_cast<const uint4*>(dres + row * lddr + (lane + 64 * k) * 8);
    }
    float dot = 0.f;
#pragma unroll
    for (int k = 0; k < CPL; ++k) {
        const int c = lane + 64 * k;
        const uint4 xraw = *reinterpret_cast<const uint4*>(x + row * ldx + c * 8);
        xr[k] = RowReg<PACK, F>::keep(xraw);
        const F8 xv = unpack8<F>(xraw), gv = ld8<F>(dy + row * lddy + c * 8), wv = ld8<F>(w + c * 8);
        F8 gw;
#pragma unroll
        for (int j = 0; j < 8; ++j) {
            gw.v[j] = rnd<F>(gv.v[j] * wv.v[j]);
            dot += gw.v[j] * xv.v[j];
        }
        gr[k] = RowReg<PACK, F>::put(gw);
    }
    if constexpr (PRE) {
#pragma unroll
        for (int k = 0; k < CPL; ++k)
            asm volatile("" : "+v"(drr[k].x), "+v"(drr[k].y), "+v"(drr[k].z), "+v"(drr[k].w));
    }
    dot = wave_sum_f(dot);
    const float coef = r * r * r * dot / (float)H;
    if constexpr (PACK) asm volatile("" ::: "memory");
#pragma unroll
    for (int k = 0; k < CPL; ++k) {
        const int c = lane + 64 * k;
        const F8 xv = RowReg<PACK, F>::get(xr[k]), gw = RowReg<PACK, F>::get(gr[k]);
        F8 o;
#pragma unroll
        for (int j = 0; j < 8; ++j) o.v[j] = r * gw.v[j] - xv.v[j] * coef;
        if (ADD) {
            F8 dr;
            if constexpr (PRE) dr = unpack8<F>(drr[k]);
            else dr = ld8<F>(dres + row * lddr + c * 8);
#pragma unroll
            for (int j = 0; j < 8; ++j) o.v[j] = rnd<F>(o.v[j]) + dr.v[j];
        }
        st8<F>(dx + row * lddx + c * 8, o);
        if (QUANT) gr[k] = RowReg<PACK, F>::put(rnd8<F>(o));
    }
    if (QUANT) {
        float amax = 0.f;
#pragma unroll
        for (int k = 0; k < CPL; ++k) {
            const F8 d = RowReg<PACK, F>::get(gr[k]);
#pragma unroll
            for (int j = 0; j < 8; ++j) amax = fmaxf(amax, fabsf(d.v[j]));
        }
        amax = wave_max_f(amax);
        const float scale = e4m3_scale(amax);
        if (lane == 0) qscale[row] = scale;
#pragma unroll
        for (int k = 0; k < CPL; ++k) {
            const int c = lane + 64 * k;
            const F8 d = RowReg<PACK, F>::get(gr[k]);
            uint2 q;
            q.x = pack4(qv(d.v[0], scale), qv(d.v[1], scale), qv(d.v[2], scale), qv(d.v[3], scale));
            q.y = pack4(qv(d.v[4], scale), qv(d.v[5], scale), qv(d.v[6], scale), qv(d.v[7], scale));
            *reinterpret_cast<uint2*>(q8 + row * ldq + c * 8) = q;
        }
    }
}

template <int F>
__global__ __launch_bounds__(256)
void rmsnorm_dw_rows_kernel(const uint16_t* __restrict__ dy, int64_t lddy, const uint16_t* __restrict__ x,
                            int64_t ldx, const float* __restrict__ rstd, float* __restrict__ dw_partial,
                            int64_t rows, int64_t rows_per_chunk, int H) {
    const int c = (blockIdx.x * 256 + threadIdx.x) * 8;
    if (c >= H) return;
    const int64_t r0 = (int64_t)blockIdx.y * rows_per_chunk;
    const int64_t r1 = r0 + rows_per_chunk < rows ? r0 + rows_per_chunk : rows;
    float acc[8];
#pragma unroll
    for (int j = 0; j < 8; ++j) acc[j] = 0.f;
#pragma unroll 4
    for (int64_t row = r0; row < r1; ++row) {
        const float r = rstd[row];
        const F8 xv = ld8<F>(x + row * ldx + c), gv = ld8<F>(dy + row * lddy + c);
#pragma unroll
        for (int j = 0; j < 8; ++j) acc[j] += rnd<F>(gv.v[j] * rnd<F>(xv.v[j] * r));
    }
    float4* d = reinterpret_cast<float4*>(dw_partial + (int64_t)blockIdx.y * H + c);
    d[0] = make_float4(acc[0], acc[1], acc[2], acc[3]);
    d[1] = make_float4(acc[4], acc[5], acc[6], acc[7]);
}

struct RopeT {
    const uint16_t* in; uint16_t* out;
    int64_t sb, sh, ss;
    int64_t ob, oh, os;
    int H;
};

template <bool BWD, int F>
__device__ __forceinline__ void rope_row(const RopeT& t, const uint16_t* cos, const uint16_t* sin, int64_t cb,
                                         int64_t cs, int64_t b, int h, int idx, int S, int D) {
    const int half = D >> 1;
    const int cpr = half >> 3;
    const int s = idx / cpr;
    if (s >= S) return;
    const int d = (idx - s * cpr) * 8;
    const uint16_t* ip = t.in + b * t.sb + h * t.sh + (int64_t)s * t.ss;
    uint16_t* op = t.out + b * t.ob + h * t.oh + (int64_t)s * t.os;
    const uint16_t* cp = cos + b * cb + (int64_t)s * cs;
    const uint16_t* sp = sin + b * cb + (int64_t)s * cs;
    const F8 lo = ld8<F>(ip + d), hi = ld8<F>(ip + half + d);
    const F8 clo = ld8<F>(cp + d), chi = ld8<F>(cp + half + d), slo = ld8<F>(sp + d), shi = ld8<F>(sp + half + d);
    F8 olo, ohi;
#pragma unroll
    for (int j = 0; j < 8; ++j) {
        if (!BWD) {
            olo.v[j] = rnd<F>(lo.v[j] * clo.v[j]) + rnd<F>(-hi.v[j] * slo.v[j]);
            ohi.v[j] = rnd<F>(hi.v[j] * chi.v[j]) + rnd<F>(lo.v[j] * shi.v[j]);
        } else {
            olo.v[j] = rnd<F>(lo.v[j] * clo.v[j]) + rnd<F>(hi.v[j] * shi.v[j]);
            ohi.v[j] = rnd<F>(hi.v[j] * chi.v[j]) - rnd<F>(lo.v[j] * slo.v[j]);
        }
    }
    st8<F>(op + d, olo);
    st8<F>(op + half + d, ohi);
}

constexpr int kRopeHG = 8;
template <bool BWD, int F>
__global__ __launch_bounds__(256)
void rope_hg_kernel(RopeT q, RopeT k, const uint16_t* __restrict__ cos, const uint16_t* __restrict__ sin,
                    int64_t cb, int64_t cs, int S, int D) {
    const int qg = q.H / kRopeHG, groups = qg + k.H / kRopeHG;
    const int y = blockIdx.y;
    const int64_t b = y / groups;
    const int g = y - (int)b * groups;
    const RopeT& t = g < qg ? q : k;
    const int h0 = (g < qg ? g : g - qg) * kRopeHG;
    const int half = D >> 1;
    const int cpr = half >> 3;
    const int idx = blockIdx.x * 256 + threadIdx.x;
    const int s = idx / cpr;
    if (s >= S) return;
    const int d = (idx - s * cpr) * 8;
    const uint16_t* cp = cos + b * cb + (int64_t)s * cs;
    const uint16_t* sp = sin + b * cb + (int64_t)s * cs;
    const F8 clo = ld8<F>(cp + d), chi = ld8<F>(cp + half + d), slo = ld8<F>(sp + d), shi = ld8<F>(sp + half + d);
#pragma unroll 4
    for (int h = h0; h < h0 + kRopeHG; ++h) {
        const uint16_t* ip = t.in + b * t.sb + h * t.sh + (int64_t)s * t.ss;
        uint16_t* op = t.out + b * t.ob + h * t.oh + (int64_t)s * t.os;
        const F8 lo = ld8<F>(ip + d), hi = ld8<F>(ip + half + d);
        F8 olo, ohi;
#pragma unroll
        for (int j = 0; j < 8; ++j) {
            if (!BWD) {
                olo.v[j] = rnd<F>(lo.v[j] * clo.v[j]) + rnd<F>(-hi.v[j] * slo.v[j]);
                ohi.v[j] = rnd<F>(hi.v[j] * chi.v[j]) + rnd<F>(lo.v[j] * shi.v[j]);
            } else {
                olo.v[j] = rnd<F>(lo.v[j] * clo.v[j]) + rnd<F>(hi.v[j] * shi.v[j]);
                ohi.v[j] = rnd<F>(hi.v[j] * chi.v[j]) - rnd<F>(lo.v[j] * slo.v[j]);
            }
        }
        st8<F>(op + d, olo);
        st8<F>(op + half + d, ohi);
    }
}

template <bool BWD, int F>
__global__ __launch_bounds__(256)
void rope_kernel(RopeT q, RopeT k, const uint16_t* __restrict__ cos, const uint16_t* __restrict__ sin,
                 int64_t cb, int64_t cs, int64_t B, int S, int D) {
    const int heads = q.H + k.H;
    const int y = blockIdx.y;
    const int64_t b = y / heads;
    const int hh = y - (int)b * heads;
    const int idx = blockIdx.x * 256 + threadIdx.x;
    if (hh < q.H) rope_row<BWD, F>(q, cos, sin, cb, cs, b, hh, idx, S, D);
    else rope_row<BWD, F>(k, cos, sin, cb, cs, b, hh - q.H, idx, S, D);
}

template <int F>
__global__ __launch_bounds__(256)
void swiglu_fwd_kernel(const uint16_t* __restrict__ g, const uint16_t* __restrict__ u, uint16_t* __restrict__ h,
                       int64_t n8) {
    const int64_t i = (int64_t)blockIdx.x * 256 + threadIdx.x;
    if (i >= n8) return;
    const F8 gv = ld8<F>(g + i * 8), uv = ld8<F>(u + i * 8);
    F8 o;
#pragma unroll
    for (int j = 0; j < 8; ++j) {
        const float s = rnd<F>(gv.v[j] * smt_sigmoid(gv.v[j]));
        o.v[j] = s * uv.v[j];
    }
    st8<F>(h + i * 8, o);
}

template <int OP, int F>
__global__ __launch_bounds__(256)
void colblock_recompute_kernel(const uint16_t* __restrict__ a, int64_t lda, const uint16_t* __restrict__ b, int64_t ldb,
                               const uint16_t* __restrict__ w, const float* __restrict__ rstd, int64_t T,
                               const int32_t* __restrict__ col_blocks, int32_t n_cb, uint16_t* __restrict__ out) {
    const int64_t per_row = (int64_t)n_cb * 32;
    const int64_t v = (int64_t)blockIdx.x * 256 + threadIdx.x;
    const int64_t t = v / per_row;
    if (t >= T) return;
    const int r = (int)(v - t * per_row);
    const int j = r >> 5, ch = r & 31;
    const int64_t c = (int64_t)col_blocks[j] * 256 + ch * 8;
    const F8 av = ld8<F>(a + t * lda + c);
    F8 o;
    if (OP == 0) {
        const float rs = rstd[t];
        const F8 wv = ld8<F>(w + c);
#pragma unroll
        for (int k = 0; k < 8; ++k) o.v[k] = wv.v[k] * rnd<F>(av.v[k] * rs);
    } else {
        const F8 bv = ld8<F>(b + t * ldb + c);
#pragma unroll
        for (int k = 0; k < 8; ++k) o.v[k] = rnd<F>(av.v[k] * smt_sigmoid(av.v[k])) * bv.v[k];
    }
    st8<F>(out + ((int64_t)j * T + t) * 256 + ch * 8, o);
}

template <int F>
__global__ __launch_bounds__(256)
void swiglu_bwd_kernel(const uint16_t* __restrict__ g, const uint16_t* __restrict__ u, const uint16_t* __restrict__ dh,
                       uint16_t* __restrict__ dg, uint16_t* __restrict__ du, int64_t n8) {
    const int64_t i = (int64_t)blockIdx.x * 256 + threadIdx.x;
    if (i >= n8) return;
    const F8 gv = ld8<F>(g + i * 8), uv = ld8<F>(u + i * 8), hv = ld8<F>(dh + i * 8);
    F8 og, ou;
#pragma unroll
    for (int j = 0; j < 8; ++j) {
        const float x = gv.v[j];
        const float sig = smt_sigmoid(x);
        const float s = rnd<F>(x * sig);
        const float ds = rnd<F>(hv.v[j] * uv.v[j]);
        ou.v[j] = hv.v[j] * s;
        og.v[j] = ds * sig * (1.0f + x * (1.0f - sig));
    }
    st8<F>(dg + i * 8, og);
    st8<F>(du + i * 8, ou);
}

constexpr float kLog2e = 1.4426950408889634f;
constexpr float kLn2 = 0.6931471805599453f;
constexpr float kNegInf = -__builtin_huge_valf();
constexpr int kCeThreads = 256;

__device__ __forceinline__ void lse_merge(float& m, float& s, float m2, float s2) {
    const float M = fmaxf(m, m2);
    if (M == kNegInf) return;
    s = s * __builtin_amdgcn_exp2f(m - M) + s2 * __builtin_amdgcn_exp2f(m2 - M);
    m = M;
}

__device__ __forceinline__ void lse_chunk(const F8& v, float& m, float& s) {
    float y[8];
    float cm = kNegInf;
#pragma unroll
    for (int j = 0; j < 8; ++j) {
        y[j] = v.v[j] * kLog2e;
        cm = fmaxf(cm, y[j]);
    }
    if (cm > m) {
        s *= __builtin_amdgcn_exp2f(m - cm);
        m = cm;
    }
    if (m == kNegInf) return;
#pragma unroll
    for (int j = 0; j < 8; ++j) s += __builtin_amdgcn_exp2f(y[j] - m);
}

template <int F>
__global__ __launch_bounds__(kCeThreads)
void ce_fwd_kernel(const uint16_t* __restrict__ logits, int64_t ld, const int64_t* __restrict__ labels, int64_t V,
                   int64_t ignore_index, float* __restrict__ lse, float* __restrict__ loss) {
    __shared__ float wm[kCeThreads / 64], wsum[kCeThreads / 64];
    const int64_t row = blockIdx.x;
    const uint16_t* xr = logits + row * ld;
    const int tid = threadIdx.x;
    const int64_t n8 = V >> 3;
    float m = kNegInf, s = 0.f;
    int64_t c = tid;
    for (; c + 3 * kCeThreads < n8; c += 4 * kCeThreads) {
        const F8 a = ld8<F>(xr + c * 8), b = ld8<F>(xr + (c + kCeThreads) * 8);
        const F8 d = ld8<F>(xr + (c + 2 * kCeThreads) * 8), e = ld8<F>(xr + (c + 3 * kCeThreads) * 8);
        lse_chunk(a, m, s);
        lse_chunk(b, m, s);
        lse_chunk(d, m, s);
        lse_chunk(e, m, s);
    }
    for (; c < n8; c += kCeThreads) lse_chunk(ld8<F>(xr + c * 8), m, s);
#pragma unroll
    for (int off = 32; off > 0; off >>= 1) {
        const float m2 = __shfl_xor(m, off, 64), s2 = __shfl_xor(s, off, 64);
        lse_merge(m, s, m2, s2);
    }
    if ((tid & 63) == 0) {
        wm[tid >> 6] = m;
        wsum[tid >> 6] = s;
    }
    __syncthreads();
    if (tid == 0) {
#pragma unroll
        for (int w = 1; w < kCeThreads / 64; ++w) lse_merge(m, s, wm[w], wsum[w]);
        const float l = (m + log2f(s)) * kLn2;
        lse[row] = l;
        const int64_t lab = labels[row];
        float out;
        if (lab == ignore_index) out = 0.f;
        else if (lab < 0 || lab >= V) out = __builtin_nanf("");
        else out = l - u2f<F>((uint32_t)xr[lab]);
        loss[row] = out;
    }
}

__device__ __forceinline__ F8 ce_grad8(const F8& v, int64_t col0, int64_t lab, float l2, float w) {
    F8 o;
#pragma unroll
    for (int j = 0; j < 8; ++j) {
        const float p = __builtin_amdgcn_exp2f(fmaf(v.v[j], kLog2e, -l2)) * w;
        o.v[j] = (col0 + j == lab) ? p - w : p;
    }
    return o;
}

template <int F>
__global__ __launch_bounds__(kCeThreads)
void ce_bwd_kernel(const uint16_t* logits, int64_t ld, const int64_t* __restrict__ labels,
                   const float* __restrict__ lse, const float* __restrict__ scale, int64_t V, int64_t ignore_index,
                   uint16_t* dlogits, int64_t ldd) {
    const int64_t row = blockIdx.x;
    const int64_t lab = labels[row];
    const float w = (lab == ignore_index) ? 0.f : scale[0];
    const float l2 = lse[row] * kLog2e;
    const uint16_t* xr = logits + row * ld;
    uint16_t* dr = dlogits + row * ldd;
    const int64_t n8 = V >> 3;
    int64_t c = threadIdx.x;
    for (; c + kCeThreads < n8; c += 2 * kCeThreads) {
        const F8 a = ld8<F>(xr + c * 8), b = ld8<F>(xr + (c + kCeThreads) * 8);
        st8<F>(dr + c * 8, ce_grad8(a, c * 8, lab, l2, w));
        st8<F>(dr + (c + kCeThreads) * 8, ce_grad8(b, (c + kCeThreads) * 8, lab, l2, w));
    }
    for (; c < n8; c += kCeThreads) st8<F>(dr + c * 8, ce_grad8(ld8<F>(xr + c * 8), c * 8, lab, l2, w));
}

template <bool ADD, int F>
int fwd_reg_dispatch(int cpl, dim3 grid, hipStream_t stream, const uint16_t* x, int64_t ldx, const uint16_t* r, int64_t ldr,
                     const uint16_t* w, uint16_t* h, int64_t ldh, uint16_t* y, int64_t ldy, float* rstd, int64_t rows,
                     int H, float eps) {
#define FWD_REG(C) case C: hipLaunchKernelGGL((rmsnorm_fwd_reg_kernel<C, ADD, false, F>), grid, dim3(256), 0, stream, x, ldx, r, ldr, w, h, ldh, y, ldy, rstd, rows, H, eps, nullptr, 0, nullptr); break;
    switch (cpl) {
        FWD_REG(1) FWD_REG(2) FWD_REG(3) FWD_REG(4) FWD_REG(5) FWD_REG(6) FWD_REG(7) FWD_REG(8)
        FWD_REG(9) FWD_REG(10) FWD_REG(11) FWD_REG(12) FWD_REG(13) FWD_REG(14) FWD_REG(15) FWD_REG(16)
        default: return fail(-1, "rmsnorm: hidden %d", H);
    }
#undef FWD_REG
    return check_launch("rmsnorm_fwd_reg_kernel");
}

template <int F>
int launch_fwd_reg(bool add, const void* x, int64_t ldx, const void* r, int64_t ldr, const void* w, void* h, int64_t ldh,
                   void* y, int64_t ldy, float* rstd, int64_t rows, int H, float eps, hipStream_t stream) {
    const dim3 grid((unsigned)((rows + 3) / 4));
    const int cpl = H / 512;
    if (add)
        return fwd_reg_dispatch<true, F>(cpl, grid, stream, (const uint16_t*)x, ldx, (const uint16_t*)r, ldr,
                                         (const uint16_t*)w, (uint16_t*)h, ldh, (uint16_t*)y, ldy, rstd, rows, H, eps);
    return fwd_reg_dispatch<false, F>(cpl, grid, stream, (const uint16_t*)x, ldx, nullptr, 0, (const uint16_t*)w, nullptr,
                                      0, (uint16_t*)y, ldy, rstd, rows, H, eps);
}

template <bool ADD, int F>
int bwd_reg_dispatch(int cpl, dim3 grid, hipStream_t stream, const uint16_t* dy, int64_t lddy, const uint16_t* x, int64_t ldx,
                     const uint16_t* w, const float* rstd, const uint16_t* dres, int64_t lddr, uint16_t* dx, int64_t lddx,
                     int64_t rows, int H) {
#define BWD_REG(C) case C: hipLaunchKernelGGL((rmsnorm_bwd_reg_kernel<C, ADD, false, F>), grid, dim3(256), 0, stream, dy, lddy, x, ldx, w, rstd, dres, lddr, dx, lddx, rows, H, nullptr, 0, nullptr); break;
    switch (cpl) {
        BWD_REG(1) BWD_REG(2) BWD_REG(3) BWD_REG(4) BWD_REG(5) BWD_REG(6) BWD_REG(7) BWD_REG(8)
        BWD_REG(9) BWD_REG(10) BWD_REG(11) BWD_REG(12) BWD_REG(13) BWD_REG(14) BWD_REG(15) BWD_REG(16)
        default: return fail(-1, "rmsnorm: hidden %d", H);
    }
#undef BWD_REG
    return check_launch("rmsnorm_bwd_reg_kernel");
}

template <int F>
int launch_bwd_reg(bool add, const void* dy, int64_t lddy, const void* x, int64_t ldx, const void* w, const float* rstd,
                   const void* dres, int64_t lddr, void* dx, int64_t lddx, int64_t rows, int H, hipStream_t stream) {
    const dim3 grid((unsigned)((rows + 3) / 4));
    const int cpl = H / 512;
    if (add)
        return bwd_reg_dispatch<true, F>(cpl, grid, stream, (const uint16_t*)dy, lddy, (const uint16_t*)x, ldx,
                                         (const uint16_t*)w, rstd, (const uint16_t*)dres, lddr, (uint16_t*)dx, lddx, rows, H);
    return bwd_reg_dispatch<false, F>(cpl, grid, stream, (const uint16_t*)dy, lddy, (const uint16_t*)x, ldx,
                                      (const uint16_t*)w, rstd, nullptr, 0, (uint16_t*)dx, lddx, rows, H);
}

template <int F>
int launch_bwd_dw(const void* dres, int64_t lddr, const void* dy, int64_t lddy, const void* x, int64_t ldx,
                  const void* w, const float* rstd, void* dx, int64_t lddx, float* dw_partial, void* dw, int64_t rows,
                  int H, hipStream_t stream) {
    if (!dw_partial || !dw || (H % 512) || H > 8192)
        return fail(-1, "smt_rmsnorm_bwd: weight grad needs hidden %% 512 == 0, <= 8192 and a partial buffer");
    int rc = launch_bwd_reg<F>(dres != nullptr, dy, lddy, x, ldx, w, rstd, dres, lddr, dx, lddx, rows, H, stream);
    if (rc) return rc;
    const int64_t cap = smt_rmsnorm_bwd_waves(rows);
    int64_t per = (rows + cap - 1) / cap;
    if (per < 64) per = 64;
    const int64_t n_chunks = (rows + per - 1) / per;
    const unsigned col_blocks = (unsigned)((H / 8 + 255) / 256);
    hipLaunchKernelGGL(rmsnorm_dw_rows_kernel<F>, dim3(col_blocks, (unsigned)n_chunks), dim3(256), 0, stream,
                       (const uint16_t*)dy, lddy, (const uint16_t*)x, ldx, rstd, dw_partial, rows, per, H);
    rc = check_launch("rmsnorm_dw_rows_kernel");
    if (rc) return rc;
    const unsigned out_blocks = (unsigned)((H + 255) / 256);
    hipLaunchKernelGGL(rmsnorm_dw_chunk_kernel, dim3(out_blocks, (unsigned)((n_chunks + kDwChunk - 1) / kDwChunk)),
                       dim3(256), 0, stream, dw_partial, n_chunks, H);
    rc = check_launch("rmsnorm_dw_chunk_kernel");
    if (rc) return rc;
    hipLaunchKernelGGL(rmsnorm_dw_kernel<F>, dim3(out_blocks), dim3(256), 0, stream, (const float*)dw_partial, n_chunks, H,
                       (uint16_t*)dw);
    return check_launch("rmsnorm_dw_kernel");
}

#define SMT_FMT_CALL(what, dtype, fn, ...)                                                                     \
    ((dtype) == SMT_DTYPE_BF16   ? fn<SMT_DTYPE_BF16>(__VA_ARGS__)                                              \
     : (dtype) == SMT_DTYPE_FP16 ? fn<SMT_DTYPE_FP16>(__VA_ARGS__)                                              \
                                 : fail(-1, "%s: dtype %d is not a 16-bit format (SMT_DTYPE_BF16 / SMT_DTYPE_FP16)", \
                                        what, (int)(dtype)))

template <int F>
int ce_fwd_impl(const void* logits, int64_t ld, const int64_t* labels, int64_t rows, int64_t vocab, int64_t ignore_index,
                float* lse, float* loss, hipStream_t stream) {
    hipLaunchKernelGGL(ce_fwd_kernel<F>, dim3((unsigned)rows), dim3(kCeThreads), 0, stream, (const uint16_t*)logits, ld,
                       labels, vocab, ignore_index, lse, loss);
    return check_launch("ce_fwd_kernel");
}

template <int F>
int ce_bwd_impl(const void* logits, int64_t ld, const int64_t* labels, const float* lse, const float* scale, int64_t rows,
                int64_t vocab, int64_t ignore_index, void* dlogits, int64_t ld_d, hipStream_t stream) {
    hipLaunchKernelGGL(ce_bwd_kernel<F>, dim3((unsigned)rows), dim3(kCeThreads), 0, stream, (const uint16_t*)logits, ld,
                       labels, lse, scale, vocab, ignore_index, (uint16_t*)dlogits, ld_d);
    return check_launch("ce_bwd_kernel");
}

template <int F>
int rmsnorm_fwd_impl(const void* x, int64_t ld_x, const void* weight, void* y, int64_t ld_y, float* rstd, int64_t rows,
                     int32_t hidden, float eps, hipStream_t stream) {
    if (hidden % 512 == 0 && hidden <= 8192)
        return launch_fwd_reg<F>(false, x, ld_x, nullptr, 0, weight, nullptr, 0, y, ld_y, rstd, rows, hidden, eps, stream);
    hipLaunchKernelGGL(rmsnorm_fwd_kernel<F>, dim3((unsigned)((rows + 3) / 4)), dim3(256), 0, stream,
                       (const uint16_t*)x, ld_x, (const uint16_t*)weight, (uint16_t*)y, ld_y, rstd, rows, hidden, eps);
    return check_launch("rmsnorm_fwd_kernel");
}

template <int F>
int rmsnorm_bwd_impl(const void* dy, int64_t ld_dy, const void* x, int64_t ld_x, const void* weight, const float* rstd,
                     void* dx, int64_t ld_dx, float* dw_partial, void* dw, int64_t rows, int32_t hidden, hipStream_t stream) {
    if (dw != nullptr)
        return launch_bwd_dw<F>(nullptr, 0, dy, ld_dy, x, ld_x, weight, rstd, dx, ld_dx, dw_partial, dw, rows, hidden,
// ... 294 lines not shown
```

### sparse_matrix_tuning_amd/fused_llama.py

```python
from __future__ import annotations

import ctypes
import os
import weakref

import torch
from torch import nn

from . import _hip


def _stream(t):
    return torch.cuda.current_stream(t.device).cuda_stream


def _need(t: torch.Tensor, what: str, like: torch.Tensor = None):
    if t.device.type != "cuda" or t.dtype not in (torch.bfloat16, torch.float16):
        raise RuntimeError(f"fused {what}: bf16 / fp16 ROCm tensors only (got {t.dtype} on {t.device})")
    if like is not None and t.dtype != like.dtype:
        raise RuntimeError(f"fused {what}: {t.dtype} beside {like.dtype} (one model dtype)")


def _dt(t: torch.Tensor) -> int:
    return _hip.dtype_code16(t.dtype, "fused op")


def _tag(out, op, a2d, b2d=None, w=None, rstd=None):
    from .smt.smt import tag_recompute
    return tag_recompute(out, op, a2d, b2d, w, rstd)


def _rows2d(t: torch.Tensor):
    t2 = t.reshape(-1, t.shape[-1])
    if t2.stride(-1) != 1 or t2.stride(0) % 8 or t2.data_ptr() % 16:
        t2 = t2.contiguous()
    return t2


class FusedRMSNormFn(torch.autograd.Function):
    @staticmethod
    def forward(ctx, x, weight, eps):
        _need(x, "rmsnorm")
        _need(weight, "rmsnorm", like=x)
        x2 = _rows2d(x)
        rows, H = x2.shape
        y = torch.empty((rows, H), dtype=x.dtype, device=x.device)
        rstd = torch.empty(rows, dtype=torch.float32, device=x.device)
        w = weight.contiguous()
        rc = _hip.load().smt_rmsnorm_fwd(x2.data_ptr(), x2.stride(0), w.data_ptr(), y.data_ptr(), y.stride(0),
                                         rstd.data_ptr(), rows, H, float(eps), _dt(x), _stream(x))
        _hip._check(rc, "smt_rmsnorm_fwd")
        ctx.save_for_backward(x2, w, rstd)
        ctx.shape = x.shape
        return _tag(y.view(x.shape), _hip.RECOMPUTE_RMSNORM, x2, None, w, rstd)

    @staticmethod
    def backward(ctx, dy):
        x2, w, rstd = ctx.saved_tensors
        dx, dw = _rmsnorm_bwd(x2, w, rstd, dy, ctx.needs_input_grad[1])
        return dx.view(ctx.shape), dw, None


def _rmsnorm_bwd(x2, w, rstd, dy, need_dw: bool, dres=None):
    rows, H = x2.shape
    dy2 = _rows2d(dy)
    dx = torch.empty_like(x2)
    lib = _hip.load()
    dw = partial = None
    if need_dw:
        waves = lib.smt_rmsnorm_bwd_waves(rows)
        partial = torch.empty(waves, H, dtype=torch.float32, device=x2.device)
        dw = torch.empty(H, dtype=w.dtype, device=w.device)
    if dres is not None and need_dw and H % 512 == 0 and H <= 8192:
        dr2 = _rows2d(dres)
        rc = lib.smt_rmsnorm_bwd_add_dw(dy2.data_ptr(), dy2.stride(0), x2.data_ptr(), x2.stride(0), w.data_ptr(),
                                        rstd.data_ptr(), dr2.data_ptr(), dr2.stride(0), dx.data_ptr(), dx.stride(0),
                                        partial.data_ptr(), dw.data_ptr(), rows, H, _dt(x2), _stream(x2))
        _hip._check(rc, "smt_rmsnorm_bwd_add_dw")
        return dx, dw
    rc = lib.smt_rmsnorm_bwd(dy2.data_ptr(), dy2.stride(0), x2.data_ptr(), x2.stride(0), w.data_ptr(),
                             rstd.data_ptr(), dx.data_ptr(), dx.stride(0),
                             None if partial is None else partial.data_ptr(),
                             None if dw is None else dw.data_ptr(), rows, H, _dt(x2), _stream(x2))
    _hip._check(rc, "smt_rmsnorm_bwd")
    if dres is not None:
        dx = dx + _rows2d(dres)
    return dx, dw


def fused_rmsnorm_forward(self, hidden_states):
    return FusedRMSNormFn.apply(hidden_states, self.weight, self.variance_epsilon)


class FusedRMSNormResFn(torch.autograd.Function):

    @staticmethod
    def forward(ctx, x, weight, eps, quant=False, need_y=True):
        if not quant:
            y = FusedRMSNormFn.forward(ctx, x, weight, eps)
            return y, x.view_as(x)
        from .fp8 import rmsnorm_quant
        _need(x, "rmsnorm")
        x2, w = _rows2d(x), weight.contiguous()
        _h, y, rstd, q, sq = rmsnorm_quant(x2, None, w, eps, need_y)
        ctx.save_for_backward(x2, w, rstd)
        ctx.shape = x.shape
        ctx.quant_grad = True
        y = y.view(x.shape) if y is not None else x.new_zeros(()).expand(x.shape)
        y._smt_q8 = (y._version, q, sq)
        return y, x.view_as(x)

    @staticmethod
    def backward(ctx, dy, dres):
        x2, w, rstd = ctx.saved_tensors
        if dres is None or ctx.needs_input_grad[1] or x2.shape[1] % 512 or x2.shape[1] > 8192:
            dx, dw = _rmsnorm_bwd(x2, w, rstd, dy, ctx.needs_input_grad[1], dres)
            return dx.view(ctx.shape), dw, None, None, None
        rows, H = x2.shape
        dy2, dr2 = _rows2d(dy), _rows2d(dres)
        if getattr(ctx, "quant_grad", False):
            from .fp8 import rmsnorm_bwd_add_quant
            dx, q, sq = rmsnorm_bwd_add_quant(dy2, x2, w, rstd, dr2)
            dx = dx.view(ctx.shape)
            dx._smt_q8 = (dx._version, q, sq)
            return dx, None, None, None, None
        dx = torch.empty_like(x2)
        rc = _hip.load().smt_rmsnorm_bwd_add(dy2.data_ptr(), dy2.stride(0), x2.data_ptr(), x2.stride(0), w.data_ptr(),
                                             rstd.data_ptr(), dr2.data_ptr(), dr2.stride(0), dx.data_ptr(), H, rows, H,
                                             _dt(x2), _stream(x2))
        _hip._check(rc, "smt_rmsnorm_bwd_add")
        return dx.view(ctx.shape), None, None, None, None


class FusedAddRMSNormFn(torch.autograd.Function):

    @staticmethod
    def forward(ctx, x, residual, weight, eps, quant=False, need_y=True):
        for t, n in ((x, "x"), (residual, "residual"), (weight, "weight")):
            _need(t, "add+rmsnorm " + n, like=x)
        x2, r2 = _rows2d(x), _rows2d(residual)
        rows, H = x2.shape
        if quant:
            from .fp8 import rmsnorm_quant
            w = weight.contiguous()
            h, y, rstd, q, sq = rmsnorm_quant(x2, r2, w, eps, need_y)
            ctx.save_for_backward(h, w, rstd)
            ctx.shape = x.shape
            ctx.quant_grad = True
            y = y.view(x.shape) if y is not None else x.new_zeros(()).expand(x.shape)
            y._smt_q8 = (y._version, q, sq)
            return h.view(x.shape), y
        h = torch.empty((rows, H), dtype=x.dtype, device=x.device)
        y = torch.empty((rows, H), dtype=x.dtype, device=x.device)
        rstd = torch.empty(rows, dtype=torch.float32, device=x.device)
        w = weight.contiguous()
        rc = _hip.load().smt_add_rmsnorm_fwd(x2.data_ptr(), x2.stride(0), r2.data_ptr(), r2.stride(0), w.data_ptr(),
                                             h.data_ptr(), H, y.data_ptr(), H, rstd.data_ptr(), rows, H, float(eps),
                                             _dt(x), _stream(x))
        _hip._check(rc, "smt_add_rmsnorm_fwd")
        ctx.save_for_backward(h, w, rstd)
        ctx.shape = x.shape
        return h.view(x.shape), _tag(y.view(x.shape), _hip.RECOMPUTE_RMSNORM, h, None, w, rstd)

    @staticmethod
    def backward(ctx, dh, dy):
        h, w, rstd = ctx.saved_tensors
        rows, H = h.shape
        lib = _hip.load()
        dw = None
        if dy is None:
            dx = dh
        elif ctx.needs_input_grad[2] or dh is None:
            dx, dw = _rmsnorm_bwd(h, w, rstd, dy, ctx.needs_input_grad[2], dh)
            dx = dx.view(ctx.shape)
        elif getattr(ctx, "quant_grad", False):
            from .fp8 import rmsnorm_bwd_add_quant
            dx, q, sq = rmsnorm_bwd_add_quant(_rows2d(dy), h, w, rstd, _rows2d(dh))
            dx = dx.view(ctx.shape)
            dx._smt_q8 = (dx._version, q, sq)
        else:
            dy2, dh2 = _rows2d(dy), _rows2d(dh)
            dx = torch.empty_like(h)
            rc = lib.smt_rmsnorm_bwd_add(dy2.data_ptr(), dy2.stride(0), h.data_ptr(), H, w.data_ptr(), rstd.data_ptr(),
                                         dh2.data_ptr(), dh2.stride(0), dx.data_ptr(), H, rows, H, _dt(h), _stream(h))
            _hip._check(rc, "smt_rmsnorm_bwd_add")
            dx = dx.view(ctx.shape)
        return dx, dx, dw, None, None, None


_RESIDUAL_NORM = os.environ.get("SMT_FUSED_RESIDUAL_NORM", "1") != "0"
_LAYER_TAIL = os.environ.get("SMT_FUSED_LAYER_TAIL", "1") != "0"


def _recomputed(layer) -> bool:
    return bool(getattr(layer, "gradient_checkpointing", False) and layer.training)


def _attn_quant(attn, H):
    if H in (1024, 2048, 4096, 8192) and all(hasattr(attn, n) for n in ("q_proj", "k_proj", "v_proj")):
        from .fp8 import norm_consumers
        return norm_consumers(attn.q_proj, attn.k_proj, attn.v_proj)
    return (False, True)


def fused_decoder_layer_forward(self, hidden_states, attention_mask=None, position_ids=None, past_key_values=None,
                                use_cache=False, position_embeddings=None, **kwargs):
    norm1 = self.input_layernorm
    attn, mlp = self.self_attn, self.mlp
    H = hidden_states.shape[-1]
    q1 = q2 = (False, True)
    if H in (1024, 2048, 4096, 8192) and all(hasattr(attn, n) for n in ("q_proj", "k_proj", "v_proj")):
        from .fp8 import norm_consumers
        q1 = norm_consumers(attn.q_proj, attn.k_proj, attn.v_proj)
        if hasattr(mlp, "gate_proj") and hasattr(mlp, "up_proj"):
            q2 = norm_consumers(mlp.gate_proj, mlp.up_proj)
    st = hidden_states.__dict__.pop("_smt_normed", None)
    if (st is not None and st[0] is norm1.weight and st[1] == q1 and st[3] == hidden_states._version
            and not _recomputed(self)):
        residual, hidden_states = hidden_states, st[2]
    elif _RESIDUAL_NORM:
        hidden_states, residual = FusedRMSNormResFn.apply(hidden_states, norm1.weight, norm1.variance_epsilon, *q1)
    else:
        residual = hidden_states
        hidden_states = norm1(hidden_states)
    hidden_states, _ = self.self_attn(hidden_states=hidden_states, attention_mask=attention_mask,
                                      position_ids=position_ids, past_key_values=past_key_values, use_cache=use_cache,
                                      position_embeddings=position_embeddings, **kwargs)
    norm = self.post_attention_layernorm
    residual, hidden_states = FusedAddRMSNormFn.apply(hidden_states, residual, norm.weight, norm.variance_epsilon, *q2)
    hidden_states = self.mlp(hidden_states)
    ref = self.__dict__.get("_smt_next_layer")
    nxt = ref() if ref is not None else None
    if _LAYER_TAIL and _RESIDUAL_NORM and nxt is not None and not _recomputed(self) and not _recomputed(nxt):
        qn = _attn_quant(nxt.self_attn, H)
        n1 = nxt.input_layernorm
        h, y = FusedAddRMSNormFn.apply(hidden_states, residual, n1.weight, n1.variance_epsilon, *qn)
        h.__dict__["_smt_normed"] = (n1.weight, qn, y, h._version)
        return h
    return residual + hidden_states


def _rope_desc(inp: torch.Tensor, out: torch.Tensor) -> _hip.RopeTensor:
    sb, sh, ss, sd = inp.stride()
    ob, oh, os_, od = out.stride()
    if sd != 1 or od != 1:
        raise RuntimeError("fused rope: head_dim must be the innermost dimension")
    return _hip.RopeTensor(inp.data_ptr(), out.data_ptr(), sb, sh, ss, ob, oh, os_, inp.shape[1], 0)


def _rope_launch(fn_name, q, k, cos, sin, q_layout=None, k_layout=None, in_place=False):
    B, _Hq, S, D = q.shape
    if cos.dim() != 3 or cos.stride(-1) != 1 or cos.shape != sin.shape or cos.stride() != sin.stride():
        cos, sin = cos.contiguous(), sin.contiguous()
    if cos.shape[0] != B:
        cos, sin = cos.expand(B, -1, -1), sin.expand(B, -1, -1)
    q = _rope_ready(q)
    k = _rope_ready(k)
    qs, qst = q_layout or (q.shape, q.stride())
    ks, kst = k_layout or (k.shape, k.stride())
    if in_place:
        qo, ko = q, k
    else:
        qo = torch.empty_strided(qs, qst, dtype=q.dtype, device=q.device)
        ko = torch.empty_strided(ks, kst, dtype=k.dtype, device=k.device)
    dq, dk = _rope_desc(q, qo), _rope_desc(k, ko)
    lib = _hip.load()
    rc = getattr(lib, fn_name)(ctypes.byref(dq), ctypes.byref(dk), cos.data_ptr(), sin.data_ptr(), cos.stride(0),
                               cos.stride(1), B, S, D, _dt(q), _stream(q))
    _hip._check(rc, fn_name)
    return qo, ko


def _rope_ready(t: torch.Tensor) -> torch.Tensor:
    if t.stride(-1) == 1 and not any(s % 8 for s in t.stride()[:3]) and t.data_ptr() % 16 == 0:
        return t
    return t.contiguous()


class FusedRoPEFn(torch.autograd.Function):
    @staticmethod
    def forward(ctx, q, k, cos, sin):
        for t, n in ((q, "q"), (k, "k"), (cos, "cos"), (sin, "sin")):
            _need(t, "rope " + n, like=q)
        qo, ko = _rope_launch("smt_rope_fwd", q, k, cos, sin)
        ctx.save_for_backward(cos, sin)
        ctx.layouts = ((q.shape, q.stride()), (k.shape, k.stride()))
        return qo, ko

    @staticmethod
    def backward(ctx, dqo, dko):
        cos, sin = ctx.saved_tensors
        ql, kl = ctx.layouts
        if dqo is None:
            dqo = torch.zeros(ql[0], dtype=cos.dtype, device=cos.device)
        if dko is None:
            dko = torch.zeros(kl[0], dtype=cos.dtype, device=cos.device)
        joint = (getattr(dqo, "_smt_joint", False) and getattr(dko, "_smt_joint", False)
                 and _rope_ready(dqo) is dqo and _rope_ready(dko) is dko)
        dq, dk = _rope_launch("smt_rope_bwd", dqo, dko, cos, sin, ql, kl, in_place=joint)
        return dq, dk, None, None


def fused_apply_rotary_pos_emb(q, k, cos, sin, unsqueeze_dim=1):
    if unsqueeze_dim != 1:
        raise NotImplementedError("fused rope: unsqueeze_dim=1 layout only")
    return FusedRoPEFn.apply(q, k, cos, sin)


class FusedSwiGLUFn(torch.autograd.Function):

    @staticmethod
    def forward(ctx, gate, up, quant_out=False, need_bf16_out=True):
        _need(gate, "swiglu")
        _need(up, "swiglu", like=gate)
        from .fp8 import swiglu_group
        ctx.fp8 = swiglu_group(gate, up)
        g = gate.contiguous()
        u = up.contiguous()
        ctx.save_for_backward(g, u)
        if quant_out:
            from .fp8 import swiglu_fwd_quant
            q, sq, h = swiglu_fwd_quant(g, u, need_bf16_out)
            if h is None:
                h = g.new_zeros(()).expand(g.shape)
            h._smt_q8 = (h._version, q, sq)
            return h
        h = torch.empty_like(g)
        rc = _hip.load().smt_swiglu_fwd(g.data_ptr(), u.data_ptr(), h.data_ptr(), g.numel(), _dt(g), _stream(g))
        _hip._check(rc, "smt_swiglu_fwd")
        return _tag(h, _hip.RECOMPUTE_SWIGLU, _rows2d(g), _rows2d(u))

    @staticmethod
    def backward(ctx, dh):
        g, u = ctx.saved_tensors
        dh = dh.contiguous()
        if ctx.fp8 is not None and not ctx.fp8[0].parts and ctx.fp8[0].prequant is None:
            from .fp8 import swiglu_bwd_quant
            acc, need_dg, need_du = ctx.fp8
            q, sq, dg, du = swiglu_bwd_quant(g, u, dh, need_dg, need_du)
            out_g, out_u = _grad_or_placeholder(g, dg, need_dg), _grad_or_placeholder(u, du, need_du)
            acc.prequant = (q, sq, (out_g, out_u))
            return out_g, out_u, None, None
        dg = torch.empty_like(g)
        du = torch.empty_like(u)
        rc = _hip.load().smt_swiglu_bwd(g.data_ptr(), u.data_ptr(), dh.data_ptr(), dg.data_ptr(), du.data_ptr(),
                                        g.numel(), _dt(g), _stream(g))
        _hip._check(rc, "smt_swiglu_bwd")
        return dg, du, None, None


def _grad_or_placeholder(like: torch.Tensor, grad, need) -> torch.Tensor:
    if grad is not None and need is True:
        return grad
    ph = like.new_zeros(()).expand_as(like)
    if grad is not None:
        ph._smt_gpack = grad
        from .fp8 import MxRowsNeed
        if isinstance(need, MxRowsNeed):
            need.delivered = True
    return ph


def fused_mlp_forward(self, x):
    from .fp8 import sole_swiglu_consumer
    with sole_swiglu_consumer():
        gate, up = self.gate_proj(x), self.up_proj(x)
    d = self.down_proj
    if getattr(d.weight, "_smt_fp8", None) is not None and gate.shape[-1] <= 16384:
        from . import fp8
        if fp8.FUSED_SWIGLU_QUANT and fp8.FUSED_SWIGLU_FWD_QUANT:
            frozen_plain = type(d) is torch.nn.Linear and not d.weight.requires_grad
            return d(FusedSwiGLUFn.apply(gate, up, True, not frozen_plain))
    return d(FusedSwiGLUFn.apply(gate, up))


class FusedCrossEntropyFn(torch.autograd.Function):

    @staticmethod
    def forward(ctx, logits2d, labels, ignore_index, denom):
        _need(logits2d, "cross entropy logits")
        if logits2d.stride(1) != 1 or logits2d.stride(0) % 8 or logits2d.data_ptr() % 16:
            logits2d = logits2d.contiguous()
        N, V = logits2d.shape
        labels = labels.to(device=logits2d.device, dtype=torch.int64).contiguous()
        if labels.numel() != N:
            raise ValueError(f"cross entropy: {labels.numel()} labels for {N} logit rows")
        lse = torch.empty(N, dtype=torch.float32, device=logits2d.device)
        rows = torch.empty(N, dtype=torch.float32, device=logits2d.device)
        rc = _hip.load().smt_ce_fwd(logits2d.data_ptr(), logits2d.stride(0), labels.data_ptr(), N, V,
                                    int(ignore_index), lse.data_ptr(), rows.data_ptr(), _dt(logits2d), _stream(logits2d))
        _hip._check(rc, "smt_ce_fwd")
        ctx.save_for_backward(logits2d, labels, lse, denom)
        ctx.ignore_index = int(ignore_index)
        return rows.sum() / denom

    @staticmethod
    def backward(ctx, dloss):
        logits2d, labels, lse, denom = ctx.saved_tensors
        N, V = logits2d.shape
        scale = (dloss.float() / denom).reshape(1).contiguous()
        dlogits = torch.empty_like(logits2d)
        rc = _hip.load().smt_ce_bwd(logits2d.data_ptr(), logits2d.stride(0), labels.data_ptr(), lse.data_ptr(),
                                    scale.data_ptr(), N, V, ctx.ignore_index, dlogits.data_ptr(), dlogits.stride(0),
                                    _dt(logits2d), _stream(logits2d))
        _hip._check(rc, "smt_ce_bwd")
        return dlogits, None, None, None


def fused_causal_lm_loss(logits, labels, vocab_size, num_items_in_batch=None, ignore_index=-100,
                         shift_labels=None, **kwargs):
    logits2d = logits.reshape(-1, vocab_size)
    shift = _shifted_labels(labels, ignore_index, shift_labels).to(logits2d.device)
    if num_items_in_batch is None:
        denom = (shift != ignore_index).sum().to(torch.float32)
    else:
        denom = torch.as_tensor(num_items_in_batch, device=logits2d.device).to(torch.float32)
    return FusedCrossEntropyFn.apply(logits2d, shift, ignore_index, denom)


def _shifted_labels(labels, ignore_index, shift_labels):
    if shift_labels is None:
        labels = nn.functional.pad(labels, (0, 1), value=ignore_index)
        shift_labels = labels[..., 1:]
    return shift_labels.reshape(-1)


LM_HEAD_CHUNK_ROWS = int(os.environ.get("SMT_LM_HEAD_CHUNK_ROWS", "4096"))
LM_HEAD_DW_CHUNK_ROWS = int(os.environ.get("SMT_LM_HEAD_DW_CHUNK_ROWS", "16384"))


class FusedLMHeadLossFn(torch.autograd.Function):

    @staticmethod
    def forward(ctx, hidden, weight, weight_t, labels, ignore_index, denom, chunk_rows, grad_enabled=True):
        _need(hidden, "lm head loss")
        _need(weight, "lm head loss", like=hidden)
        h2 = _rows2d(hidden)
        N, H = h2.shape
        V = weight.shape[0]
        if weight.shape[1] != H:
            raise ValueError(f"lm head loss: weight {tuple(weight.shape)} for hidden size {H}")
        if V % 8:
            raise ValueError(f"lm head loss: vocabulary {V} is not a multiple of 8")
        labels = labels.to(device=hidden.device, dtype=torch.int64).contiguous()
        if labels.numel() != N:
            raise ValueError(f"lm head loss: {labels.numel()} labels for {N} rows")
        need_dh = bool(ctx.needs_input_grad[0]) and grad_enabled
        need_dw = bool(ctx.needs_input_grad[1]) and grad_enabled
        lib = _hip.load()
        stream = _stream(hidden)
        dt = _dt(hidden)
        lse = torch.empty(N, dtype=torch.float32, device=hidden.device)
        rows = torch.empty(N, dtype=torch.float32, device=hidden.device)
        dh = torch.empty((N, H), dtype=hidden.dtype, device=hidden.device) if need_dh else None
        scale = (1.0 / denom.to(torch.float32)).reshape(1).contiguous()
        C = max(1, min(max(int(chunk_rows), LM_HEAD_DW_CHUNK_ROWS if need_dw else 0), N))
        buf = torch.empty((C, V), dtype=hidden.dtype, device=hidden.device)
        w_dgrad = weight_t.t() if weight_t is not None else weight
        acc = torch.empty((V, H), dtype=torch.float32, device=hidden.device) if need_dw else None
        for r0 in range(0, N, C):
            c = min(C, N - r0)
            lg = buf[:c]
            hc = h2[r0:r0 + c]
            torch.mm(hc, weight.t(), out=lg)
            rc = lib.smt_ce_fwd(lg.data_ptr(), lg.stride(0), labels[r0:].data_ptr(), c, V, int(ignore_index),
                                lse[r0:].data_ptr(), rows[r0:].data_ptr(), dt, stream)
            _hip._check(rc, "smt_ce_fwd")
            if need_dh or need_dw:
                rc = lib.smt_ce_bwd(lg.data_ptr(), lg.stride(0), labels[r0:].data_ptr(), lse[r0:].data_ptr(),
                                    scale.data_ptr(), c, V, int(ignore_index), lg.data_ptr(), lg.stride(0), dt, stream)
                _hip._check(rc, "smt_ce_bwd")
            if need_dh:
                torch.mm(lg, w_dgrad, out=dh[r0:r0 + c])
            if need_dw:
                if r0 == 0:
                    torch.mm(lg.t(), hc, out_dtype=torch.float32, out=acc)
                else:
                    torch.addmm(acc, lg.t(), hc, out_dtype=torch.float32, out=acc)
        del buf
        dw = None
        if need_dw:
            dw = acc.to(weight.dtype)
            del acc
        ctx.save_for_backward(dh, dw)
        ctx.shape = hidden.shape
        return rows.sum() / denom

    @staticmethod
    def backward(ctx, dloss):
        dh, dw = ctx.saved_tensors
        scale = dloss.float()
        gh = torch.mul(dh, scale).view(ctx.shape) if dh is not None else None
        gw = torch.mul(dw, scale) if dw is not None else None
        return gh, gw, None, None, None, None, None, None


def fused_lm_head_loss(hidden, lm_head: nn.Linear, labels, num_items_in_batch=None, ignore_index=-100,
                       shift_labels=None, chunk_rows=None):
    shift = _shifted_labels(labels, ignore_index, shift_labels).to(hidden.device)
    if num_items_in_batch is None:
        denom = (shift != ignore_index).sum().to(torch.float32)
    else:
        denom = torch.as_tensor(num_items_in_batch, device=hidden.device).to(torch.float32)
    wt = getattr(lm_head.weight, "_smt_weight_t", None)
    return FusedLMHeadLossFn.apply(hidden, lm_head.weight, wt, shift, ignore_index, denom,
                                   LM_HEAD_CHUNK_ROWS if chunk_rows is None else chunk_rows, torch.is_grad_enabled())


def _fusable_lm_head(head) -> bool:
    w = getattr(head, "weight", None)
    return (type(head) is nn.Linear and head.bias is None and isinstance(w, torch.Tensor)
            and w.device.type == "cuda" and w.dtype in (torch.bfloat16, torch.float16)
            and getattr(w, "_smt_fp8", None) is None)


def fused_causal_lm_forward(self, input_ids=None, attention_mask=None, position_ids=None, past_key_values=None,
                            inputs_embeds=None, labels=None, use_cache=None, logits_to_keep=0, **kwargs):
    if (labels is None or not _fusable_lm_head(self.lm_head) or not isinstance(logits_to_keep, int)
            or logits_to_keep != 0 or kwargs.get("return_dict") is False
            or getattr(self, "loss_function", None) is not fused_causal_lm_loss):
        return type(self).forward(self, input_ids=input_ids, attention_mask=attention_mask, position_ids=position_ids,
                                  past_key_values=past_key_values, inputs_embeds=inputs_embeds, labels=labels,
                                  use_cache=use_cache, logits_to_keep=logits_to_keep, **kwargs)
    kwargs.pop("return_dict", None)
    from transformers.modeling_outputs import CausalLMOutputWithPast
    outputs = self.model(input_ids=input_ids, attention_mask=attention_mask, position_ids=position_ids,
                         past_key_values=past_key_values, inputs_embeds=inputs_embeds, use_cache=use_cache, **kwargs)
    loss = fused_lm_head_loss(outputs.last_hidden_state, self.lm_head, labels,
                              num_items_in_batch=kwargs.get("num_items_in_batch"),
                              shift_labels=kwargs.get("shift_labels"))
    return CausalLMOutputWithPast(loss=loss, logits=None, past_key_values=outputs.past_key_values,
                                  hidden_states=outputs.hidden_states, attentions=outputs.attentions)


def _attn_tensor(t: torch.Tensor) -> _hip.AttnTensor:
    sb, sh, ss, sd = t.stride()
    if sd != 1:
        raise RuntimeError("flash attention: head_dim must be the innermost dimension")
    return _hip.AttnTensor(t.data_ptr(), sb, sh, ss)


def _attn_ready(t: torch.Tensor) -> torch.Tensor:
    if t.stride(-1) == 1 and not any(s % 8 for s in t.stride()[:3]) and t.data_ptr() % 16 == 0:
        return t
    return t.contiguous()


class KeyMask:

    __slots__ = ("bits", "S")

    def __init__(self, bits: torch.Tensor, S: int):
        self.bits, self.S = bits, int(S)

    @classmethod
    def from_padding_mask(cls, mask2d: torch.Tensor) -> "KeyMask":
        B, S = mask2d.shape
        W = -(-S // 64)
        m = torch.zeros(B, W * 64, dtype=torch.int64, device=mask2d.device)
        m[:, :S] = mask2d.to(torch.bool).to(torch.int64)
        shifts = torch.arange(64, dtype=torch.int64, device=mask2d.device)
        bits = (m.view(B, W, 64) << shifts).sum(-1)
        return cls(bits.contiguous(), S)


class FlashAttnFn(torch.autograd.Function):

    @staticmethod
    def forward(ctx, q, k, v, scale, key_mask=None, joint=False):
        for t, n in ((q, "q"), (k, "k"), (v, "v")):
            _need(t, "flash attention " + n, like=q)
        B, Hq, S, D = q.shape
        Hkv = k.shape[1]
        if D != 128 or k.shape != (B, Hkv, S, D) or v.shape != k.shape or Hq % Hkv or S % 4:
            raise NotImplementedError(f"flash attention: head_dim 128, Hq % Hkv == 0, S % 4 == 0 "
                                      f"(q {tuple(q.shape)}, k {tuple(k.shape)})")
        q, k, v = _attn_ready(q), _attn_ready(k), _attn_ready(v)
        for t in (q, k, v):
            if S * t.stride(2) * 2 >= 2 ** 31:
                raise NotImplementedError("flash attention: per-head extent must stay below 2 GiB")
        o = torch.empty(B, S, Hq, D, dtype=q.dtype, device=q.device)
        lse = torch.empty(B, Hq, S, dtype=torch.float32, device=q.device)
        ov = o.transpose(1, 2)
        shape = _hip.AttnShape(B, Hq, Hkv, S, float(scale), _dt(q))
        km, km_ld = None, 0
        if key_mask is not None:
            if key_mask.S != S or key_mask.bits.shape[0] != B or key_mask.bits.device != q.device:
                raise ValueError(f"flash attention: key mask for [{key_mask.bits.shape[0]}, {key_mask.S}] keys, "
                                 f"batch has [{B}, {S}]")
            km, km_ld = key_mask.bits.data_ptr(), key_mask.bits.shape[1]
        rc = _hip.load().smt_attn_fwd_kmask(ctypes.byref(_attn_tensor(q)), ctypes.byref(_attn_tensor(k)),
                                            ctypes.byref(_attn_tensor(v)), ctypes.byref(_attn_tensor(ov)),
                                            lse.data_ptr(), km, km_ld, ctypes.byref(shape), _stream(q))
        _hip._check(rc, "smt_attn_fwd")
        ctx.save_for_backward(q, k, v, o, lse, key_mask.bits if key_mask is not None else None)
        ctx.scale = float(scale)
        ctx.joint = bool(joint)
        return o

    @staticmethod
    def backward(ctx, do):
        q, k, v, o, lse, km = ctx.saved_tensors
        B, Hq, S, D = q.shape
        Hkv = k.shape[1]
        do = do if (do.stride(-1) == 1 and not any(s % 8 for s in do.stride()[:3]) and do.data_ptr() % 16 == 0) \
            else do.contiguous()
        if ctx.joint:
            J = torch.empty(B, S, (Hq + 2 * Hkv) * D, dtype=q.dtype, device=q.device)
            dq = J[:, :, :Hq * D].view(B, S, Hq, D).transpose(1, 2)
            dk = J[:, :, Hq * D:(Hq + Hkv) * D].view(B, S, Hkv, D).transpose(1, 2)
            dv = J[:, :, (Hq + Hkv) * D:].view(B, S, Hkv, D).transpose(1, 2)
            dq._smt_joint = dk._smt_joint = True
        else:
            dq = torch.empty_strided(q.shape, q.stride(), dtype=q.dtype, device=q.device)
            dk = torch.empty_strided(k.shape, k.stride(), dtype=k.dtype, device=k.device)
            dv = torch.empty_strided(v.shape, v.stride(), dtype=v.dtype, device=v.device)
        delta = torch.empty(B, Hq, S, dtype=torch.float32, device=q.device)
        if do.dtype != q.dtype:
            do = do.to(q.dtype)
        shape = _hip.AttnShape(B, Hq, Hkv, S, ctx.scale, _dt(q))
        T = _attn_tensor
        rc = _hip.load().smt_attn_bwd_kmask(ctypes.byref(T(q)), ctypes.byref(T(k)), ctypes.byref(T(v)),
                                            ctypes.byref(T(o.transpose(1, 2))), ctypes.byref(T(do.transpose(1, 2))),
                                            lse.data_ptr(), delta.data_ptr(), ctypes.byref(T(dq)),
                                            ctypes.byref(T(dk)), ctypes.byref(T(dv)),
                                            km.data_ptr() if km is not None else None,
                                            km.shape[1] if km is not None else 0, ctypes.byref(shape), _stream(q))
        _hip._check(rc, "smt_attn_bwd")
        return dq, dk, dv, None, None, None


def flash_attention(q, k, v, scale=None, key_mask: "KeyMask" = None, joint: bool = False):
    return FlashAttnFn.apply(q, k, v, scale if scale is not None else q.shape[-1] ** -0.5, key_mask, joint)


def smt_flash_attention_forward(module, query, key, value, attention_mask, dropout=0.0, scaling=None,
                                is_causal=None, **kwargs):
    if attention_mask is not None and not isinstance(attention_mask, KeyMask):
        raise NotImplementedError("smt_flash attention: only key-padding masks built by smt_flash_mask are "
                                  f"supported (got {type(attention_mask).__name__})")
    if dropout:
        raise NotImplementedError("smt_flash attention: dropout is not supported")
    if is_causal is False or not getattr(module, "is_causal", True):
        raise NotImplementedError("smt_flash attention: causal attention only")
    return flash_attention(query, key, value, scaling, attention_mask,
                           joint=getattr(module, "_smt_joint_qkv_grad", False)), None


def smt_flash_mask(batch_size, q_length, kv_length, q_offset=0, kv_offset=0, mask_function=None,
                   attention_mask=None, **kwargs):
    from transformers.masking_utils import causal_mask_function
    if mask_function is not None and mask_function is not causal_mask_function:
        raise NotImplementedError("smt_flash attention: custom / packed-sequence masks are not supported")
    if q_offset or kv_offset or q_length != kv_length:
        raise NotImplementedError("smt_flash attention: training-style self-attention only (no KV cache)")
    if attention_mask is None:
        return None
    am = attention_mask
    if am.dim() != 2 or am.shape[0] != batch_size or am.shape[1] < kv_length:
        raise NotImplementedError(f"smt_flash attention: 2-D [B, S] padding mask expected, got {tuple(am.shape)}")
    am = am[:, :kv_length].to(torch.bool)
    if bool(am.all()):
        return None
    return KeyMask.from_padding_mask(am)


ATTN_NAME = "smt_flash"


def register_attention() -> str:
    from transformers import AttentionInterface
    from transformers.masking_utils import ALL_MASK_ATTENTION_FUNCTIONS
    AttentionInterface.register(ATTN_NAME, smt_flash_attention_forward)
    ALL_MASK_ATTENTION_FUNCTIONS.register(ATTN_NAME, smt_flash_mask)
    return ATTN_NAME


_EAGER = {}


def _ml():
    from transformers.models.llama import modeling_llama as ml
    if "rope" not in _EAGER:
        _EAGER["rope"] = ml.apply_rotary_pos_emb
    return ml


def eager_apply_rotary_pos_emb(*a, **k):
    return _ml() and _EAGER["rope"](*a, **k)


def patch_llama(model: nn.Module, attention: bool = True, loss: bool = True, lm_head_loss: bool = None) -> dict:
    ml = _ml()
    counts = {"rmsnorm": 0, "mlp": 0, "rope": 1, "attention": 0, "loss": 0, "decoder": 0, "lm_head_loss": 0}
    if lm_head_loss is None:
        lm_head_loss = os.environ.get("SMT_LM_HEAD_LOSS", "1") != "0"
    if loss and hasattr(type(model), "loss_function"):
        model.loss_function = fused_causal_lm_loss
        counts["loss"] = 1
        if lm_head_loss and isinstance(model, ml.LlamaForCausalLM):
            model.forward = fused_causal_lm_forward.__get__(model, type(model))
            counts["lm_head_loss"] = 1
    if attention:
        cfg = getattr(model, "config", None)
        if cfg is None:
            raise RuntimeError("patch_llama(attention=True) needs a transformers model with a config")
        if "smt_prev_attn" not in _EAGER:
            _EAGER["smt_prev_attn"] = cfg._attn_implementation
        cfg._attn_implementation = register_attention()
        counts["attention"] = sum(1 for m in model.modules() if isinstance(m, ml.LlamaAttention))
    for m in model.modules():
        if isinstance(m, ml.LlamaRMSNorm):
            m.forward = fused_rmsnorm_forward.__get__(m, type(m))
            counts["rmsnorm"] += 1
        elif isinstance(m, ml.LlamaDecoderLayer):
            m.forward = fused_decoder_layer_forward.__get__(m, type(m))
            counts["decoder"] += 1
        elif isinstance(m, ml.LlamaMLP):
            act = getattr(m, "act_fn", None)
            if act is None or "silu" not in type(act).__name__.lower():
                raise NotImplementedError(f"fused MLP: SiLU activation only (got {type(act).__name__})")
            m.forward = fused_mlp_forward.__get__(m, type(m))
            counts["mlp"] += 1
        elif isinstance(m, nn.ModuleList) and len(m) > 1 and all(isinstance(x, ml.LlamaDecoderLayer) for x in m):
            for i in range(len(m) - 1):
                m[i].__dict__["_smt_next_layer"] = weakref.ref(m[i + 1])
    ml.apply_rotary_pos_emb = fused_apply_rotary_pos_emb
    return counts


def unpatch_llama(model: nn.Module = None) -> None:
    ml = _ml()
    ml.apply_rotary_pos_emb = _EAGER["rope"]
    if model is not None and "smt_prev_attn" in _EAGER and getattr(model, "config", None) is not None:
        model.config._attn_implementation = _EAGER.pop("smt_prev_attn")
    if model is not None:
        if "_loss_function" in model.__dict__:
            del model.__dict__["_loss_function"]
        if "forward" in model.__dict__:
            del model.__dict__["forward"]
        for m in model.modules():
            if isinstance(m, (ml.LlamaRMSNorm, ml.LlamaMLP, ml.LlamaDecoderLayer)) and "forward" in m.__dict__:
                del m.__dict__["forward"]
            m.__dict__.pop("_smt_next_layer", None)
```

Baseline: 39740.

## Fold RoPE backward into flash attention dQ/dK epilogues and widen output stores

Adds a backward attention entry point that applies the inverse rotary embedding to dQ and dK inside the kernel epilogues. The separate RoPE backward kernel and its extra read/write pass over the Q/K gradients go away. dQ stages cos/sin rows in the spare LDS ring via DMA, while dK reads them from global memory. It also switches unmasked output stores to 16-byte permlane-swapped writes, and patches LlamaAttention.forward to route through the fused RoPE+flash autograd function, with an env var to disable it. This adds code complexity and extra LDS traffic in the dQ kernel.

```diff
diff --git a/include/smt_attention.h b/include/smt_attention.h
--- a/include/smt_attention.h
+++ b/include/smt_attention.h
@@ -40,6 +40,12 @@
                        const uint64_t* key_mask, int64_t key_mask_ld, const smt_attn_shape* shape,
                        hipStream_t stream);
 
+int smt_attn_bwd_rope_kmask(const smt_attn_tensor* q, const smt_attn_tensor* k, const smt_attn_tensor* v,
+                            const smt_attn_tensor* o, const smt_attn_tensor* d_o, const float* lse, float* delta_ws,
+                            const smt_attn_tensor* dq, const smt_attn_tensor* dk, const smt_attn_tensor* dv,
+                            const uint64_t* key_mask, int64_t key_mask_ld, const smt_attn_shape* shape,
+                            const void* cos, const void* sin, int64_t cb, int64_t cs, hipStream_t stream);
+
 #ifdef __cplusplus
 }
 #endif
diff --git a/sparse_matrix_tuning_amd/_hip.py b/sparse_matrix_tuning_amd/_hip.py
--- a/sparse_matrix_tuning_amd/_hip.py
+++ b/sparse_matrix_tuning_amd/_hip.py
@@ -32,6 +32,7 @@
     "smt_add_rmsnorm_fwd", "smt_rmsnorm_bwd_add", "smt_colblock_recompute",
     "smt_rope_fwd", "smt_rope_bwd", "smt_swiglu_fwd", "smt_swiglu_bwd", "smt_ce_fwd", "smt_ce_bwd",
     "smt_attn_last_error", "smt_attn_fwd", "smt_attn_bwd", "smt_attn_fwd_kmask", "smt_attn_bwd_kmask",
+    "smt_attn_bwd_rope_kmask",
     "smt_fp8_last_error", "smt_quant_rows_e4m3", "smt_quant_cols_t_e4m3", "smt_quant_rows_cat_e4m3",
     "smt_swiglu_fwd_quant_e4m3", "smt_swiglu_bwd_quant_e4m3", "smt_swiglu_bwd_quant_e4m3_packed",
     "smt_rmsnorm_fwd_quant_e4m3",
@@ -147,6 +148,8 @@
     "smt_attn_fwd_kmask": (ctypes.c_int, [ctypes.POINTER(AttnTensor)] * 4 + [_P, _P, _I64, ctypes.POINTER(AttnShape), _P]),
     "smt_attn_bwd_kmask": (ctypes.c_int, [ctypes.POINTER(AttnTensor)] * 5 + [_P, _P] + [ctypes.POINTER(AttnTensor)] * 3
                            + [_P, _I64, ctypes.POINTER(AttnShape), _P]),
+    "smt_attn_bwd_rope_kmask": (ctypes.c_int, [ctypes.POINTER(AttnTensor)] * 5 + [_P, _P] + [ctypes.POINTER(AttnTensor)] * 3
+                                + [_P, _I64, ctypes.POINTER(AttnShape), _P, _P, _I64, _I64, _P]),
     "smt_model_ops_last_error": (ctypes.c_char_p, []),
     "smt_rmsnorm_fwd": (ctypes.c_int, [_P, _I64, _P, _P, _I64, _P, _I64, _I32, ctypes.c_float, _I32, _P]),
     "smt_rmsnorm_bwd_waves": (ctypes.c_int, [_I64]),
diff --git a/sparse_matrix_tuning_amd/build.py b/sparse_matrix_tuning_amd/build.py
--- a/sparse_matrix_tuning_amd/build.py
+++ b/sparse_matrix_tuning_amd/build.py
@@ -11,7 +11,7 @@
                                                    "fp8_kernels.hip")]
 HEADERS = [os.path.join(REPO_DIR, "include", n) for n in ("smt_hip.h", "smt_model_ops.h", "smt_attention.h",
                                                           "smt_fp8.h")]
-HEADERS += [os.path.join(PKG_DIR, "csrc", n) for n in ("silu_math.h", "fp8_math.h")]
+HEADERS += [os.path.join(PKG_DIR, "csrc", n) for n in ("silu_math.h", "fp8_math.h", "rope_math.h")]
 LIB_DIR = os.path.join(PKG_DIR, "_lib")
 LIB_PATH = os.path.join(LIB_DIR, "libsmt_hip.so")
 ARCH = "gfx950"
diff --git a/sparse_matrix_tuning_amd/csrc/attn_kernels.hip b/sparse_matrix_tuning_amd/csrc/attn_kernels.hip
--- a/sparse_matrix_tuning_amd/csrc/attn_kernels.hip
+++ b/sparse_matrix_tuning_amd/csrc/attn_kernels.hip
@@ -6,6 +6,7 @@
 
 #include <utility>
 
+#include "rope_math.h"
 #include "smt_attention.h"
 #include "smt_hip.h"
 
@@ -36,6 +37,7 @@
 typedef short s16x8_t __attribute__((ext_vector_type(8)));
 typedef float f32x16_t __attribute__((ext_vector_type(16)));
 typedef uint32_t u32x4_t __attribute__((ext_vector_type(4)));
+typedef uint32_t u32x2_t __attribute__((ext_vector_type(2)));
 typedef __attribute__((address_space(3))) s16x4_t lds_s16x4_t;
 
 constexpr int kD = 128;
@@ -132,6 +134,124 @@
         u32x4_t v = {a[0], b[0], a[1], b[1]};
         if (h == 0) f0 = __builtin_bit_cast(bf16x8_t, v);
         else f1 = __builtin_bit_cast(bf16x8_t, v);
+    }
+}
+
+#ifndef SMT_ATTN_WIDE_STORE
+#define SMT_ATTN_WIDE_STORE 1
+#endif
+constexpr bool kWideStore = SMT_ATTN_WIDE_STORE != 0;
+
+struct RopeTab {
+    const uint16_t* cos;
+    const uint16_t* sin;
+    int64_t cb, cs;
+};
+
+template <int F>
+__device__ __forceinline__ u32x4_t piece16(const f32x16_t& acc, int p, float scale) {
+    const int i = 8 * p;
+    const uint32_t ax = pk16<F>(acc[i] * scale, acc[i + 1] * scale), ay = pk16<F>(acc[i + 2] * scale, acc[i + 3] * scale);
+    const uint32_t bx = pk16<F>(acc[i + 4] * scale, acc[i + 5] * scale), by = pk16<F>(acc[i + 6] * scale, acc[i + 7] * scale);
+    auto rx = __builtin_amdgcn_permlane32_swap(ax, bx, false, false);
+    auto ry = __builtin_amdgcn_permlane32_swap(ay, by, false, false);
+    return u32x4_t{rx[0], ry[0], rx[1], ry[1]};
+}
+template <int F>
+__device__ __forceinline__ u32x2_t piece8(const f32x16_t& acc, int g, float scale) {
+    const int i = 4 * g;
+    return u32x2_t{pk16<F>(acc[i] * scale, acc[i + 1] * scale), pk16<F>(acc[i + 2] * scale, acc[i + 3] * scale)};
+}
+
+struct GlobalTab {
+    const uint16_t* cosr;
+    const uint16_t* sinr;
+    __device__ __forceinline__ void ready() const {}
+    template <typename V> __device__ __forceinline__ V cos(int d) const { return *reinterpret_cast<const V*>(cosr + d); }
+    template <typename V> __device__ __forceinline__ V sin(int d) const { return *reinterpret_cast<const V*>(sinr + d); }
+};
+struct LdsTab {
+    const uint8_t* cimg;
+    const uint8_t* simg;
+    uint32_t row;
+    __device__ __forceinline__ void ready() const { asm volatile("s_waitcnt vmcnt(0)" ::: "memory"); }
+    template <typename V> __device__ __forceinline__ V cos(int d) const {
+        return *reinterpret_cast<const V*>(cimg + row * kRowB + ((uint32_t)(2 * d) ^ (swz(row) << 4)));
+    }
+    template <typename V> __device__ __forceinline__ V sin(int d) const {
+        return *reinterpret_cast<const V*>(simg + row * kRowB + ((uint32_t)(2 * d) ^ (swz(row) << 4)));
+    }
+};
+struct NoTab {};
+
+template <int F, typename V, typename TAB>
+__device__ __forceinline__ void rope_bwd_piece(V& lo, V& hi, const TAB& tab, int d) {
+    constexpr int N = sizeof(V) / 4;
+    const V clo = tab.template cos<V>(d), chi = tab.template cos<V>(d + kD / 2);
+    const V slo = tab.template sin<V>(d), shi = tab.template sin<V>(d + kD / 2);
+#pragma unroll
+    for (int w = 0; w < N; ++w) {
+        float l0, h0, l1, h1;
+        smt_rope_pair<true, F>(lo16<F>(lo[w]), lo16<F>(hi[w]), lo16<F>(clo[w]), lo16<F>(chi[w]), lo16<F>(slo[w]),
+                               lo16<F>(shi[w]), l0, h0);
+        smt_rope_pair<true, F>(hi16<F>(lo[w]), hi16<F>(hi[w]), hi16<F>(clo[w]), hi16<F>(chi[w]), hi16<F>(slo[w]),
+                               hi16<F>(shi[w]), l1, h1);
+        lo[w] = pk16<F>(l0, l1);
+        hi[w] = pk16<F>(h0, h1);
+    }
+}
+
+template <int F, bool ROPE, bool WIDE, typename TAB = NoTab>
+__device__ __forceinline__ void store_row(uint16_t* out, const f32x16_t (&acc)[4], float scale, int hi,
+                                          const TAB& tab = TAB{}) {
+    if constexpr (ROPE) {
+#pragma unroll
+        for (int dt = 0; dt < 2; ++dt) {
+            if constexpr (WIDE) {
+                u32x4_t lo[2], up[2];
+#pragma unroll
+                for (int p = 0; p < 2; ++p) {
+                    lo[p] = piece16<F>(acc[dt], p, scale);
+                    up[p] = piece16<F>(acc[dt + 2], p, scale);
+                }
+                if (dt == 0) tab.ready();
+#pragma unroll
+                for (int p = 0; p < 2; ++p) {
+                    const int d = 32 * dt + 16 * p + 8 * hi;
+                    rope_bwd_piece<F>(lo[p], up[p], tab, d);
+                    *reinterpret_cast<u32x4_t*>(out + d) = lo[p];
+                    *reinterpret_cast<u32x4_t*>(out + d + kD / 2) = up[p];
+                }
+            } else {
+                u32x2_t lo[4], up[4];
+#pragma unroll
+                for (int g = 0; g < 4; ++g) {
+                    lo[g] = piece8<F>(acc[dt], g, scale);
+                    up[g] = piece8<F>(acc[dt + 2], g, scale);
+                }
+                if (dt == 0) tab.ready();
+#pragma unroll
+                for (int g = 0; g < 4; ++g) {
+                    const int d = 32 * dt + 8 * g + 4 * hi;
+                    rope_bwd_piece<F>(lo[g], up[g], tab, d);
+                    *reinterpret_cast<u32x2_t*>(out + d) = lo[g];
+                    *reinterpret_cast<u32x2_t*>(out + d + kD / 2) = up[g];
+                }
+            }
+        }
+    } else {
+#pragma unroll
+        for (int dt = 0; dt < 4; ++dt) {
+            if constexpr (WIDE) {
+#pragma unroll
+                for (int p = 0; p < 2; ++p)
+                    *reinterpret_cast<u32x4_t*>(out + 32 * dt + 16 * p + 8 * hi) = piece16<F>(acc[dt], p, scale);
+            } else {
+#pragma unroll
+                for (int g = 0; g < 4; ++g)
+                    *reinterpret_cast<u32x2_t*>(out + 32 * dt + 8 * g + 4 * hi) = piece8<F>(acc[dt], g, scale);
+            }
+        }
     }
 }
 
@@ -242,6 +362,7 @@
 
 template <bool KMASK, int F>
 struct FwdLean {
+    static constexpr bool kWide = kWideStore && !KMASK;
     const FwdArgs& a;
     uint8_t* lds;
     __amdgpu_buffer_rsrc_t rk, rv;
@@ -405,16 +526,7 @@
         if (qrow < a.S) {
             const float inv = (KMASK && !(l_tot > 0.f)) ? 0.f : 1.f / l_tot;
             uint16_t* op = a.o + b * a.o_sb + h * a.o_sh + (int64_t)qrow * a.o_ss;
-#pragma unroll
-            for (int dt = 0; dt < 4; ++dt)
-#pragma unroll
-                for (int g = 0; g < 4; ++g) {
-                    const int d = 32 * dt + 8 * g + 4 * hi;
-                    uint2 w;
-                    w.x = pk16<F>(o[dt][4 * g] * inv, o[dt][4 * g + 1] * inv);
-                    w.y = pk16<F>(o[dt][4 * g + 2] * inv, o[dt][4 * g + 3] * inv);
-                    *reinterpret_cast<uint2*>(op + d) = w;
-                }
+            store_row<F, false, kWide>(op, o, inv, hi);
             if (hi == 0)
                 a.lse[((int64_t)b * a.Hq + h) * a.S + qrow] =
                     (KMASK && !(l_tot > 0.f)) ? __builtin_huge_valf() : m_run + __log2f(l_tot);
@@ -449,10 +561,12 @@
     int64_t kmask_ld;
     int B, Hq, Hkv, S;
     float sl2, scale;
+    RopeTab rope;
 };
 
-template <bool KMASK, int F>
+template <bool KMASK, int F, bool ROPE>
 struct DqLean {
+    static constexpr bool kWide = kWideStore && !KMASK;
     const DqArgs& a;
     uint8_t* lds;
     bf16x8_t qf[8], df[8];
@@ -613,23 +727,27 @@
             tile<0>(t);
             if (t + 1 < nt) tile<1>(t + 1);
         }
-        if (qvalid) {
-            uint16_t* out = a.dq + b * a.dq_sb + h * a.dq_sh + (int64_t)qrow * a.dq_ss;
-#pragma unroll
-            for (int dt = 0; dt < 4; ++dt)
-#pragma unroll
-                for (int g = 0; g < 4; ++g) {
-                    const int d = 32 * dt + 8 * g + 4 * hi;
-                    uint2 w;
-                    w.x = pk16<F>(dq[dt][4 * g] * a.scale, dq[dt][4 * g + 1] * a.scale);
-                    w.y = pk16<F>(dq[dt][4 * g + 2] * a.scale, dq[dt][4 * g + 3] * a.scale);
-                    *reinterpret_cast<uint2*>(out + d) = w;
-                }
+        const auto out_row = [&]() { return a.dq + b * a.dq_sb + h * a.dq_sh + (int64_t)qrow * a.dq_ss; };
+        if constexpr (ROPE) {
+            static_assert(kDqWaves * 2 * kFwdQW * kRowB <= 2 * 2 * kTileB, "cos / sin images fit the K/V ring");
+            if (qw < a.S) {
+                const uint32_t img = (uint32_t)(wave * 2 * kFwdQW * kRowB);
+                const int64_t bytes = (int64_t)a.S * a.rope.cs * 2;
+                const int ln = (int)opaque(__builtin_amdgcn_mbcnt_hi(~0u, __builtin_amdgcn_mbcnt_lo(~0u, 0u)));
+                const int eh = ln >> 5;
+                dma_rows(uniform_rsrc(a.rope.cos + b * a.rope.cb, bytes), a.rope.cs, lds0 + img, qw, qw, kFwdQW / 4, ln);
+                dma_rows(uniform_rsrc(a.rope.sin + b * a.rope.cb, bytes), a.rope.cs, lds0 + img + kFwdQW * kRowB, qw,
+                         qw, kFwdQW / 4, ln);
+                const LdsTab tab{lds + img, lds + img + kFwdQW * kRowB, (uint32_t)(ln & 31)};
+                if (qvalid) store_row<F, true, kWide>(out_row(), dq, a.scale, eh, tab);
+            }
+        } else {
+            if (qvalid) store_row<F, false, kWide>(out_row(), dq, a.scale, hi);
         }
     }
 };
 
-template <bool KMASK, int F>
+template <bool KMASK, int F, bool ROPE = false>
 __global__ __launch_bounds__(64 * kDqWaves, 8 / kDqWaves)
 void attn_dq_kernel(DqArgs a) {
     __shared__ __attribute__((aligned(16))) uint8_t lds[2 * 2 * kTileB];
@@ -641,7 +759,7 @@
     const int grp = L / per_group;
     const int rem = L - grp * per_group;
     const int hk = grp % a.Hkv;
-    DqLean<KMASK, F> dl(a, lds);
+    DqLean<KMASK, F, ROPE> dl(a, lds);
     dl.run(grp / a.Hkv, hk * G + rem % G, hk, nqb - 1 - rem / G);
 }
 
@@ -662,12 +780,14 @@
     int64_t kmask_ld;
     int B, Hq, Hkv, S;
     float sl2, scale;
+    RopeTab rope;
 };
 
 constexpr int kDkvLeanRing = 2;
 static_assert(kDkvLeanRing >= 2 && kDkvLeanRing * kSliceBuf + kVImg <= 160 * 1024, "dK/dV lean ring");
-template <bool KMASK, int F>
+template <bool KMASK, int F, bool ROPE>
 struct DkvLean {
+    static constexpr bool kWide = kWideStore && !KMASK;
     const DkvArgs& a;
     uint8_t* lds;
     bf16x8_t kf[8];
@@ -848,24 +968,15 @@
         if (key < a.S) {
             uint16_t* dkr = a.dk + b * a.dk_sb + hk * a.dk_sh + (int64_t)key * a.dk_ss;
             uint16_t* dvr = a.dv + b * a.dv_sb + hk * a.dv_sh + (int64_t)key * a.dv_ss;
-#pragma unroll
-            for (int dt = 0; dt < 4; ++dt)
-#pragma unroll
-                for (int g = 0; g < 4; ++g) {
-                    const int d = 32 * dt + 8 * g + 4 * hi;
-                    uint2 w;
-                    w.x = pk16<F>(dkt[dt][4 * g] * a.scale, dkt[dt][4 * g + 1] * a.scale);
-                    w.y = pk16<F>(dkt[dt][4 * g + 2] * a.scale, dkt[dt][4 * g + 3] * a.scale);
-                    *reinterpret_cast<uint2*>(dkr + d) = w;
-                    w.x = pk16<F>(dvt[dt][4 * g], dvt[dt][4 * g + 1]);
-                    w.y = pk16<F>(dvt[dt][4 * g + 2], dvt[dt][4 * g + 3]);
-                    *reinterpret_cast<uint2*>(dvr + d) = w;
-                }
+            const int64_t roff = ROPE ? b * a.rope.cb + (int64_t)key * a.rope.cs : 0;
+            store_row<F, false, kWide>(dvr, dvt, 1.f, hi);
+            if constexpr (ROPE) store_row<F, true, kWide>(dkr, dkt, a.scale, hi, GlobalTab{a.rope.cos + roff, a.rope.sin + roff});
+            else store_row<F, false, kWide>(dkr, dkt, a.scale, hi);
         }
     }
 };
 
-template <bool KMASK, int F>
+template <bool KMASK, int F, bool ROPE = false>
 __global__ __launch_bounds__(kDkvWaves * 64, 2)
 void attn_dkdv_kernel(DkvArgs a) {
     __shared__ __attribute__((aligned(16))) uint8_t lds[kVImg + kDkvLeanRing * kSliceBuf];
@@ -875,7 +986,7 @@
 #pragma nounroll
     for (int i = 0; i < t.n; ++i) {
         if (i) __syncthreads();
-        DkvLean<KMASK, F> dl(a, lds);
+        DkvLean<KMASK, F, ROPE> dl(a, lds);
         dl.run(t.b, t.hk, t.blk[1 - i]);
     }
 }
@@ -910,7 +1021,70 @@
         }                                                                                                     \
     } while (0)
 
+#define SMT_ATTN_LAUNCH_BWD(kernel, kmask, dtype, ROPE, grid, block, stream, args)                            \
+    do {                                                                                                      \
+        if ((dtype) == SMT_DTYPE_FP16) {                                                                      \
+            if (kmask) hipLaunchKernelGGL((kernel<true, SMT_DTYPE_FP16, ROPE>), grid, block, 0, stream, args);   \
+            else hipLaunchKernelGGL((kernel<false, SMT_DTYPE_FP16, ROPE>), grid, block, 0, stream, args);        \
+        } else {                                                                                              \
+            if (kmask) hipLaunchKernelGGL((kernel<true, SMT_DTYPE_BF16, ROPE>), grid, block, 0, stream, args);   \
+            else hipLaunchKernelGGL((kernel<false, SMT_DTYPE_BF16, ROPE>), grid, block, 0, stream, args);        \
+        }                                                                                                     \
+    } while (0)
+
 Tns tns(const smt_attn_tensor* t) { return Tns{static_cast<const uint16_t*>(t->ptr), t->sb, t->sh, t->ss}; }
+
+int attn_bwd(const char* fn, const smt_attn_tensor* q, const smt_attn_tensor* k, const smt_attn_tensor* v,
+             const smt_attn_tensor* o, const smt_attn_tensor* d_o, const float* lse, float* delta_ws,
+             const smt_attn_tensor* dq, const smt_attn_tensor* dk, const smt_attn_tensor* dv, const uint64_t* key_mask,
+             int64_t key_mask_ld, const RopeTab* rope, const smt_attn_shape* shape, hipStream_t stream) {
+    int rc;
+    if ((rc = check_shape(shape, fn)) || (rc = check_tensor(q, "q", fn)) || (rc = check_tensor(k, "k", fn)) ||
+        (rc = check_tensor(v, "v", fn)) || (rc = check_tensor(o, "o", fn)) || (rc = check_tensor(d_o, "do", fn)) ||
+        (rc = check_tensor(dq, "dq", fn)) || (rc = check_tensor(dk, "dk", fn)) || (rc = check_tensor(dv, "dv", fn)))
+        return rc;
+    if (!lse || !delta_ws) return fail(-1, "%s: null lse / delta workspace", fn);
+    if (!al16(lse) || !al16(delta_ws) || (shape->S & 3)) return fail(-2, "%s: lse / delta need 16-byte rows (S %% 4 == 0)", fn);
+    if (key_mask && key_mask_ld < (shape->S + 63) / 64)
+        return fail(-1, "%s: key_mask_ld %lld < ceil(S / 64)", fn, (long long)key_mask_ld);
+    if (rope) {
+        if (!rope->cos || !rope->sin) return fail(-1, "%s: null cos / sin", fn);
+        if (!al16(rope->cos) || !al16(rope->sin) || (rope->cb & 7) || (rope->cs & 7) || rope->cb < 0 || rope->cs < kD)
+            return fail(-2, "%s: cos / sin need 16-byte aligned rows of 128 (strides %% 8 == 0, row stride >= 128)", fn);
+        if ((int64_t)shape->S * rope->cs * 2 >= (1LL << 31))
+            return fail(-1, "%s: one sample's cos / sin table must stay below 2 GiB", fn);
+    }
+    const int B = shape->B, Hq = shape->Hq, Hkv = shape->Hkv, S = shape->S;
+    const float sl2 = shape->scale * 1.4426950408889634f;
+    const RopeTab tab = rope ? *rope : RopeTab{nullptr, nullptr, 0, 0};
+
+    DqArgs qa;
+    qa.q = tns(q); qa.k = tns(k); qa.v = tns(v); qa.dout = tns(d_o); qa.o = tns(o);
+    qa.dq = static_cast<uint16_t*>(dq->ptr); qa.dq_sb = dq->sb; qa.dq_sh = dq->sh; qa.dq_ss = dq->ss;
+    qa.lse = lse; qa.delta = delta_ws;
+    qa.kmask = key_mask; qa.kmask_ld = key_mask_ld;
+    qa.B = B; qa.Hq = Hq; qa.Hkv = Hkv; qa.S = S; qa.sl2 = sl2; qa.scale = shape->scale;
+    qa.rope = tab;
+    const int64_t nqb = (S + kDqQB - 1) / kDqQB;
+    const dim3 qgrid((unsigned)(nqb * Hq * B)), qblock(64 * kDqWaves);
+    if (rope) SMT_ATTN_LAUNCH_BWD(attn_dq_kernel, key_mask, shape->dtype, true, qgrid, qblock, stream, qa);
+    else SMT_ATTN_LAUNCH_BWD(attn_dq_kernel, key_mask, shape->dtype, false, qgrid, qblock, stream, qa);
+    if ((rc = check_launch("attn_dq_kernel"))) return rc;
+
+    DkvArgs ka;
+    ka.q = tns(q); ka.k = tns(k); ka.v = tns(v); ka.dout = tns(d_o);
+    ka.dk = static_cast<uint16_t*>(dk->ptr); ka.dk_sb = dk->sb; ka.dk_sh = dk->sh; ka.dk_ss = dk->ss;
+    ka.dv = static_cast<uint16_t*>(dv->ptr); ka.dv_sb = dv->sb; ka.dv_sh = dv->sh; ka.dv_ss = dv->ss;
+    ka.lse = lse; ka.delta = delta_ws;
+    ka.kmask = key_mask; ka.kmask_ld = key_mask_ld;
+    ka.B = B; ka.Hq = Hq; ka.Hkv = Hkv; ka.S = S; ka.sl2 = sl2; ka.scale = shape->scale;
+    ka.rope = tab;
+    const int64_t nkb = (S + kKB - 1) / kKB;
+    const dim3 grid((unsigned)(((nkb + 1) / 2) * Hkv * B)), block(kDkvWaves * 64);
+    if (rope) SMT_ATTN_LAUNCH_BWD(attn_dkdv_kernel, key_mask, shape->dtype, true, grid, block, stream, ka);
+    else SMT_ATTN_LAUNCH_BWD(attn_dkdv_kernel, key_mask, shape->dtype, false, grid, block, stream, ka);
+    return check_launch("attn_dkdv_kernel");
+}
 
 }
 
@@ -954,41 +1128,8 @@
                        const smt_attn_tensor* dq, const smt_attn_tensor* dk, const smt_attn_tensor* dv,
                        const uint64_t* key_mask, int64_t key_mask_ld, const smt_attn_shape* shape,
                        hipStream_t stream) {
-    int rc;
-    const char* fn = key_mask ? "smt_attn_bwd_kmask" : "smt_attn_bwd";
-    if ((rc = check_shape(shape, fn)) || (rc = check_tensor(q, "q", fn)) || (rc = check_tensor(k, "k", fn)) ||
-        (rc = check_tensor(v, "v", fn)) || (rc = check_tensor(o, "o", fn)) || (rc = check_tensor(d_o, "do", fn)) ||
-        (rc = check_tensor(dq, "dq", fn)) || (rc = check_tensor(dk, "dk", fn)) || (rc = check_tensor(dv, "dv", fn)))
-        return rc;
-    if (!lse || !delta_ws) return fail(-1, "%s: null lse / delta workspace", fn);
-    if (!al16(lse) || !al16(delta_ws) || (shape->S & 3)) return fail(-2, "%s: lse / delta need 16-byte rows (S %% 4 == 0)", fn);
-    if (key_mask && key_mask_ld < (shape->S + 63) / 64)
-        return fail(-1, "%s: key_mask_ld %lld < ceil(S / 64)", fn, (long long)key_mask_ld);
-    const int B = shape->B, Hq = shape->Hq, Hkv = shape->Hkv, S = shape->S;
-    const float sl2 = shape->scale * 1.4426950408889634f;
-
-    DqArgs qa;
-    qa.q = tns(q); qa.k = tns(k); qa.v = tns(v); qa.dout = tns(d_o); qa.o = tns(o);
-    qa.dq = static_cast<uint16_t*>(dq->ptr); qa.dq_sb = dq->sb; qa.dq_sh = dq->sh; qa.dq_ss = dq->ss;
-    qa.lse = lse; qa.delta = delta_ws;
-    qa.kmask = key_mask; qa.kmask_ld = key_mask_ld;
-    qa.B = B; qa.Hq = Hq; qa.Hkv = Hkv; qa.S = S; qa.sl2 = sl2; qa.scale = shape->scale;
-    const int64_t nqb = (S + kDqQB - 1) / kDqQB;
-    const dim3 qgrid((unsigned)(nqb * Hq * B)), qblock(64 * kDqWaves);
-    SMT_ATTN_LAUNCH(attn_dq_kernel, key_mask, shape->dtype, qgrid, qblock, stream, qa);
-    if ((rc = check_launch("attn_dq_kernel"))) return rc;
-
-    DkvArgs ka;
-    ka.q = tns(q); ka.k = tns(k); ka.v = tns(v); ka.dout = tns(d_o);
-    ka.dk = static_cast<uint16_t*>(dk->ptr); ka.dk_sb = dk->sb; ka.dk_sh = dk->sh; ka.dk_ss = dk->ss;
-    ka.dv = static_cast<uint16_t*>(dv->ptr); ka.dv_sb = dv->sb; ka.dv_sh = dv->sh; ka.dv_ss = dv->ss;
-    ka.lse = lse; ka.delta = delta_ws;
-    ka.kmask = key_mask; ka.kmask_ld = key_mask_ld;
-    ka.B = B; ka.Hq = Hq; ka.Hkv = Hkv; ka.S = S; ka.sl2 = sl2; ka.scale = shape->scale;
-    const int64_t nkb = (S + kKB - 1) / kKB;
-    const dim3 grid((unsigned)(((nkb + 1) / 2) * Hkv * B));
-    SMT_ATTN_LAUNCH(attn_dkdv_kernel, key_mask, shape->dtype, grid, dim3(kDkvWaves * 64), stream, ka);
-    return check_launch("attn_dkdv_kernel");
+    return attn_bwd(key_mask ? "smt_attn_bwd_kmask" : "smt_attn_bwd", q, k, v, o, d_o, lse, delta_ws, dq, dk, dv, key_mask,
+                    key_mask_ld, nullptr, shape, stream);
 }
 
 int smt_attn_bwd(const smt_attn_tensor* q, const smt_attn_tensor* k, const smt_attn_tensor* v,
@@ -998,4 +1139,14 @@
     return smt_attn_bwd_kmask(q, k, v, o, d_o, lse, delta_ws, dq, dk, dv, nullptr, 0, shape, stream);
 }
 
-}
+int smt_attn_bwd_rope_kmask(const smt_attn_tensor* q, const smt_attn_tensor* k, const smt_attn_tensor* v,
+                            const smt_attn_tensor* o, const smt_attn_tensor* d_o, const float* lse, float* delta_ws,
+                            const smt_attn_tensor* dq, const smt_attn_tensor* dk, const smt_attn_tensor* dv,
+                            const uint64_t* key_mask, int64_t key_mask_ld, const smt_attn_shape* shape,
+                            const void* cos, const void* sin, int64_t cb, int64_t cs, hipStream_t stream) {
+    const RopeTab tab{static_cast<const uint16_t*>(cos), static_cast<const uint16_t*>(sin), cb, cs};
+    return attn_bwd("smt_attn_bwd_rope_kmask", q, k, v, o, d_o, lse, delta_ws, dq, dk, dv, key_mask, key_mask_ld, &tab,
+                    shape, stream);
+}
+
+}
diff --git a/sparse_matrix_tuning_amd/csrc/llama_kernels.hip b/sparse_matrix_tuning_amd/csrc/llama_kernels.hip
--- a/sparse_matrix_tuning_amd/csrc/llama_kernels.hip
+++ b/sparse_matrix_tuning_amd/csrc/llama_kernels.hip
@@ -7,6 +7,7 @@
 #include "smt_hip.h"
 #include "smt_model_ops.h"
 #include "silu_math.h"
+#include "rope_math.h"
 #include "fp8_math.h"
 #include "smt_fp8.h"
 
@@ -30,19 +31,9 @@
 
 inline bool aligned16(const void* p) { return (reinterpret_cast<uintptr_t>(p) & 15u) == 0; }
 
-template <int F> __device__ __forceinline__ float u2f(uint32_t b16) {
-    if constexpr (F == SMT_DTYPE_FP16) return (float)__builtin_bit_cast(_Float16, (uint16_t)b16);
-    else return __uint_as_float(b16 << 16);
-}
-template <int F> __device__ __forceinline__ uint32_t f2u(float f) {
-    if constexpr (F == SMT_DTYPE_FP16) return (uint32_t)__builtin_bit_cast(uint16_t, (_Float16)f);
-    else return (uint32_t)__builtin_bit_cast(uint16_t, (__bf16)f);
-}
-template <int F> __device__ __forceinline__ float rnd(float f) {
-    uint32_t b = f2u<F>(f);
-    if constexpr (F == SMT_DTYPE_FP16) asm("" : "+v"(b));
-    return u2f<F>(b);
-}
+template <int F> __device__ __forceinline__ float u2f(uint32_t b16) { return smt_u2f<F>(b16); }
+template <int F> __device__ __forceinline__ uint32_t f2u(float f) { return smt_f2u<F>(f); }
+template <int F> __device__ __forceinline__ float rnd(float f) { return smt_rnd16<F>(f); }
 
 struct F8 { float v[8]; };
 
@@ -380,13 +371,7 @@
     F8 olo, ohi;
 #pragma unroll
     for (int j = 0; j < 8; ++j) {
-        if (!BWD) {
-            olo.v[j] = rnd<F>(lo.v[j] * clo.v[j]) + rnd<F>(-hi.v[j] * slo.v[j]);
-            ohi.v[j] = rnd<F>(hi.v[j] * chi.v[j]) + rnd<F>(lo.v[j] * shi.v[j]);
-        } else {
-            olo.v[j] = rnd<F>(lo.v[j] * clo.v[j]) + rnd<F>(hi.v[j] * shi.v[j]);
-            ohi.v[j] = rnd<F>(hi.v[j] * chi.v[j]) - rnd<F>(lo.v[j] * slo.v[j]);
-        }
+        smt_rope_pair<BWD, F>(lo.v[j], hi.v[j], clo.v[j], chi.v[j], slo.v[j], shi.v[j], olo.v[j], ohi.v[j]);
     }
     st8<F>(op + d, olo);
     st8<F>(op + half + d, ohi);
@@ -420,13 +405,7 @@
         F8 olo, ohi;
 #pragma unroll
         for (int j = 0; j < 8; ++j) {
-            if (!BWD) {
-                olo.v[j] = rnd<F>(lo.v[j] * clo.v[j]) + rnd<F>(-hi.v[j] * slo.v[j]);
-                ohi.v[j] = rnd<F>(hi.v[j] * chi.v[j]) + rnd<F>(lo.v[j] * shi.v[j]);
-            } else {
-                olo.v[j] = rnd<F>(lo.v[j] * clo.v[j]) + rnd<F>(hi.v[j] * shi.v[j]);
-                ohi.v[j] = rnd<F>(hi.v[j] * chi.v[j]) - rnd<F>(lo.v[j] * slo.v[j]);
-            }
+            smt_rope_pair<BWD, F>(lo.v[j], hi.v[j], clo.v[j], chi.v[j], slo.v[j], shi.v[j], olo.v[j], ohi.v[j]);
         }
         st8<F>(op + d, olo);
         st8<F>(op + half + d, ohi);
diff --git a/sparse_matrix_tuning_amd/csrc/rope_math.h b/sparse_matrix_tuning_amd/csrc/rope_math.h
--- /dev/null
+++ b/sparse_matrix_tuning_amd/csrc/rope_math.h
@@ -0,0 +1,31 @@
+#pragma once
+
+#include <stdint.h>
+
+#include "smt_hip.h"
+
+template <int F> __device__ __forceinline__ float smt_u2f(uint32_t b16) {
+    if constexpr (F == SMT_DTYPE_FP16) return (float)__builtin_bit_cast(_Float16, (uint16_t)b16);
+    else return __uint_as_float(b16 << 16);
+}
+template <int F> __device__ __forceinline__ uint32_t smt_f2u(float f) {
+    if constexpr (F == SMT_DTYPE_FP16) return (uint32_t)__builtin_bit_cast(uint16_t, (_Float16)f);
+    else return (uint32_t)__builtin_bit_cast(uint16_t, (__bf16)f);
+}
+template <int F> __device__ __forceinline__ float smt_rnd16(float f) {
+    uint32_t b = smt_f2u<F>(f);
+    if constexpr (F == SMT_DTYPE_FP16) asm("" : "+v"(b));
+    return smt_u2f<F>(b);
+}
+
+template <bool BWD, int F>
+__device__ __forceinline__ void smt_rope_pair(float lo, float hi, float clo, float chi, float slo, float shi,
+                                              float& olo, float& ohi) {
+    if (!BWD) {
+        olo = smt_rnd16<F>(lo * clo) + smt_rnd16<F>(-hi * slo);
+        ohi = smt_rnd16<F>(hi * chi) + smt_rnd16<F>(lo * shi);
+    } else {
+        olo = smt_rnd16<F>(lo * clo) + smt_rnd16<F>(hi * shi);
+        ohi = smt_rnd16<F>(hi * chi) - smt_rnd16<F>(lo * slo);
+    }
+}
diff --git a/sparse_matrix_tuning_amd/fused_llama.py b/sparse_matrix_tuning_amd/fused_llama.py
--- a/sparse_matrix_tuning_amd/fused_llama.py
+++ b/sparse_matrix_tuning_amd/fused_llama.py
@@ -248,12 +248,17 @@
     return _hip.RopeTensor(inp.data_ptr(), out.data_ptr(), sb, sh, ss, ob, oh, os_, inp.shape[1], 0)
 
 
-def _rope_launch(fn_name, q, k, cos, sin, q_layout=None, k_layout=None, in_place=False):
-    B, _Hq, S, D = q.shape
+def _rope_tables(cos, sin, B):
     if cos.dim() != 3 or cos.stride(-1) != 1 or cos.shape != sin.shape or cos.stride() != sin.stride():
         cos, sin = cos.contiguous(), sin.contiguous()
     if cos.shape[0] != B:
         cos, sin = cos.expand(B, -1, -1), sin.expand(B, -1, -1)
+    return cos, sin
+
+
+def _rope_launch(fn_name, q, k, cos, sin, q_layout=None, k_layout=None, in_place=False):
+    B, _Hq, S, D = q.shape
+    cos, sin = _rope_tables(cos, sin, B)
     q = _rope_ready(q)
     k = _rope_ready(k)
     qs, qst = q_layout or (q.shape, q.stride())
@@ -568,31 +573,7 @@
 
     @staticmethod
     def forward(ctx, q, k, v, scale, key_mask=None, joint=False):
-        for t, n in ((q, "q"), (k, "k"), (v, "v")):
-            _need(t, "flash attention " + n, like=q)
-        B, Hq, S, D = q.shape
-        Hkv = k.shape[1]
-        if D != 128 or k.shape != (B, Hkv, S, D) or v.shape != k.shape or Hq % Hkv or S % 4:
-            raise NotImplementedError(f"flash attention: head_dim 128, Hq % Hkv == 0, S % 4 == 0 "
-                                      f"(q {tuple(q.shape)}, k {tuple(k.shape)})")
-        q, k, v = _attn_ready(q), _attn_ready(k), _attn_ready(v)
-        for t in (q, k, v):
-            if S * t.stride(2) * 2 >= 2 ** 31:
-                raise NotImplementedError("flash attention: per-head extent must stay below 2 GiB")
-        o = torch.empty(B, S, Hq, D, dtype=q.dtype, device=q.device)
-        lse = torch.empty(B, Hq, S, dtype=torch.float32, device=q.device)
-        ov = o.transpose(1, 2)
-        shape = _hip.AttnShape(B, Hq, Hkv, S, float(scale), _dt(q))
-        km, km_ld = None, 0
-        if key_mask is not None:
-            if key_mask.S != S or key_mask.bits.shape[0] != B or key_mask.bits.device != q.device:
-                raise ValueError(f"flash attention: key mask for [{key_mask.bits.shape[0]}, {key_mask.S}] keys, "
-                                 f"batch has [{B}, {S}]")
-            km, km_ld = key_mask.bits.data_ptr(), key_mask.bits.shape[1]
-        rc = _hip.load().smt_attn_fwd_kmask(ctypes.byref(_attn_tensor(q)), ctypes.byref(_attn_tensor(k)),
-                                            ctypes.byref(_attn_tensor(v)), ctypes.byref(_attn_tensor(ov)),
-                                            lse.data_ptr(), km, km_ld, ctypes.byref(shape), _stream(q))
-        _hip._check(rc, "smt_attn_fwd")
+        q, k, v, o, lse = _flash_fwd(q, k, v, scale, key_mask)
         ctx.save_for_backward(q, k, v, o, lse, key_mask.bits if key_mask is not None else None)
         ctx.scale = float(scale)
         ctx.joint = bool(joint)
@@ -601,33 +582,116 @@
     @staticmethod
     def backward(ctx, do):
         q, k, v, o, lse, km = ctx.saved_tensors
-        B, Hq, S, D = q.shape
-        Hkv = k.shape[1]
-        do = do if (do.stride(-1) == 1 and not any(s % 8 for s in do.stride()[:3]) and do.data_ptr() % 16 == 0) \
-            else do.contiguous()
-        if ctx.joint:
-            J = torch.empty(B, S, (Hq + 2 * Hkv) * D, dtype=q.dtype, device=q.device)
-            dq = J[:, :, :Hq * D].view(B, S, Hq, D).transpose(1, 2)
-            dk = J[:, :, Hq * D:(Hq + Hkv) * D].view(B, S, Hkv, D).transpose(1, 2)
-            dv = J[:, :, (Hq + Hkv) * D:].view(B, S, Hkv, D).transpose(1, 2)
+        rope = getattr(ctx, "rope", None)
+        dq, dk, dv = _flash_bwd(q, k, v, o, lse, km, do, ctx.scale, ctx.joint, rope=rope)
+        if ctx.joint and rope is None:
             dq._smt_joint = dk._smt_joint = True
-        else:
-            dq = torch.empty_strided(q.shape, q.stride(), dtype=q.dtype, device=q.device)
-            dk = torch.empty_strided(k.shape, k.stride(), dtype=k.dtype, device=k.device)
-            dv = torch.empty_strided(v.shape, v.stride(), dtype=v.dtype, device=v.device)
+        return dq, dk, dv, None, None, None
+
+
+def _flash_fwd(q, k, v, scale, key_mask):
+    for t, n in ((q, "q"), (k, "k"), (v, "v")):
+        _need(t, "flash attention " + n, like=q)
+    B, Hq, S, D = q.shape
+    Hkv = k.shape[1]
+    if D != 128 or k.shape != (B, Hkv, S, D) or v.shape != k.shape or Hq % Hkv or S % 4:
+        raise NotImplementedError(f"flash attention: head_dim 128, Hq % Hkv == 0, S % 4 == 0 "
+                                  f"(q {tuple(q.shape)}, k {tuple(k.shape)})")
+    q, k, v = _attn_ready(q), _attn_ready(k), _attn_ready(v)
+    for t in (q, k, v):
+        if S * t.stride(2) * 2 >= 2 ** 31:
+            raise NotImplementedError("flash attention: per-head extent must stay below 2 GiB")
+    o = torch.empty(B, S, Hq, D, dtype=q.dtype, device=q.device)
+    lse = torch.empty(B, Hq, S, dtype=torch.float32, device=q.device)
+    ov = o.transpose(1, 2)
+    shape = _hip.AttnShape(B, Hq, Hkv, S, float(scale), _dt(q))
+    km, km_ld = None, 0
+    if key_mask is not None:
+        if key_mask.S != S or key_mask.bits.shape[0] != B or key_mask.bits.device != q.device:
+            raise ValueError(f"flash attention: key mask for [{key_mask.bits.shape[0]}, {key_mask.S}] keys, "
+                             f"batch has [{B}, {S}]")
+        km, km_ld = key_mask.bits.data_ptr(), key_mask.bits.shape[1]
+    rc = _hip.load().smt_attn_fwd_kmask(ctypes.byref(_attn_tensor(q)), ctypes.byref(_attn_tensor(k)),
+                                        ctypes.byref(_attn_tensor(v)), ctypes.byref(_attn_tensor(ov)),
+                                        lse.data_ptr(), km, km_ld, ctypes.byref(shape), _stream(q))
+    _hip._check(rc, "smt_attn_fwd")
+    return q, k, v, o, lse
+
+
+def _flash_bwd(q, k, v, o, lse, km, do, scale, joint, rope=None, delta=None):
+    B, Hq, S, D = q.shape
+    Hkv = k.shape[1]
+    do = do if (do.stride(-1) == 1 and not any(s % 8 for s in do.stride()[:3]) and do.data_ptr() % 16 == 0) \
+        else do.contiguous()
+    if joint:
+        J = torch.empty(B, S, (Hq + 2 * Hkv) * D, dtype=q.dtype, device=q.device)
+        dq = J[:, :, :Hq * D].view(B, S, Hq, D).transpose(1, 2)
+        dk = J[:, :, Hq * D:(Hq + Hkv) * D].view(B, S, Hkv, D).transpose(1, 2)
+        dv = J[:, :, (Hq + Hkv) * D:].view(B, S, Hkv, D).transpose(1, 2)
+    else:
+        dq = torch.empty_strided(q.shape, q.stride(), dtype=q.dtype, device=q.device)
+        dk = torch.empty_strided(k.shape, k.stride(), dtype=k.dtype, device=k.device)
+        dv = torch.empty_strided(v.shape, v.stride(), dtype=v.dtype, device=v.device)
+    if delta is None:
         delta = torch.empty(B, Hq, S, dtype=torch.float32, device=q.device)
-        if do.dtype != q.dtype:
-            do = do.to(q.dtype)
-        shape = _hip.AttnShape(B, Hq, Hkv, S, ctx.scale, _dt(q))
-        T = _attn_tensor
-        rc = _hip.load().smt_attn_bwd_kmask(ctypes.byref(T(q)), ctypes.byref(T(k)), ctypes.byref(T(v)),
-                                            ctypes.byref(T(o.transpose(1, 2))), ctypes.byref(T(do.transpose(1, 2))),
-                                            lse.data_ptr(), delta.data_ptr(), ctypes.byref(T(dq)),
-                                            ctypes.byref(T(dk)), ctypes.byref(T(dv)),
-                                            km.data_ptr() if km is not None else None,
-                                            km.shape[1] if km is not None else 0, ctypes.byref(shape), _stream(q))
+    if do.dtype != q.dtype:
+        do = do.to(q.dtype)
+    shape = _hip.AttnShape(B, Hq, Hkv, S, scale, _dt(q))
+    T = _attn_tensor
+    args = [ctypes.byref(T(q)), ctypes.byref(T(k)), ctypes.byref(T(v)), ctypes.byref(T(o.transpose(1, 2))),
+            ctypes.byref(T(do.transpose(1, 2))), lse.data_ptr(), delta.data_ptr(), ctypes.byref(T(dq)),
+            ctypes.byref(T(dk)), ctypes.byref(T(dv)), km.data_ptr() if km is not None else None,
+            km.shape[1] if km is not None else 0, ctypes.byref(shape)]
+    if rope is None:
+        rc = _hip.load().smt_attn_bwd_kmask(*args, _stream(q))
         _hip._check(rc, "smt_attn_bwd")
-        return dq, dk, dv, None, None, None
+    else:
+        cos, sin = _rope_tables(*rope, B)
+        rc = _hip.load().smt_attn_bwd_rope_kmask(*args, cos.data_ptr(), sin.data_ptr(), cos.stride(0), cos.stride(1),
+                                                 _stream(q))
+        _hip._check(rc, "smt_attn_bwd_rope")
+    return dq, dk, dv
+
+
+class RopeFlashAttnFn(torch.autograd.Function):
+
+    @staticmethod
+    def forward(ctx, q_raw, k_raw, v, cos, sin, scale, key_mask=None, joint=False):
+        for t, n in ((q_raw, "q"), (k_raw, "k"), (cos, "cos"), (sin, "sin")):
+            _need(t, "rope " + n, like=q_raw)
+        q, k = _rope_launch("smt_rope_fwd", q_raw, k_raw, cos, sin)
+        ctx.rope = (cos.detach(), sin.detach())
+        return FlashAttnFn.forward(ctx, q, k, v, scale, key_mask, joint)
+
+    @staticmethod
+    def backward(ctx, do):
+        return FlashAttnFn.backward(ctx, do)[:3] + (None, None, None, None, None)
+
+
+_FOLD_ENV = "SMT_ATTN_ROPE_FOLD"
+
+
+def fused_attention_forward(self, hidden_states, position_embeddings=None, attention_mask=None,
+                            past_key_values=None, **kwargs):
+    prev = self.__dict__["_smt_prev_attn_forward"]
+    dropout = 0.0 if not self.training else self.attention_dropout
+    if (os.environ.get(_FOLD_ENV, "1") == "0" or past_key_values is not None or kwargs.get("use_cache")
+            or position_embeddings is None or self.head_dim != 128 or dropout
+            or self.config._attn_implementation != ATTN_NAME or _ml().apply_rotary_pos_emb is not fused_apply_rotary_pos_emb
+            or not (attention_mask is None or isinstance(attention_mask, KeyMask))
+            or kwargs.get("is_causal") is False or not getattr(self, "is_causal", True)):
+        return prev(hidden_states, position_embeddings=position_embeddings, attention_mask=attention_mask,
+                    past_key_values=past_key_values, **kwargs)
+    input_shape = hidden_states.shape[:-1]
+    hidden_shape = (*input_shape, -1, self.head_dim)
+    q = self.q_proj(hidden_states).view(hidden_shape).transpose(1, 2)
+    k = self.k_proj(hidden_states).view(hidden_shape).transpose(1, 2)
+    v = self.v_proj(hidden_states).view(hidden_shape).transpose(1, 2)
+    cos, sin = position_embeddings
+    o = RopeFlashAttnFn.apply(q, k, v, cos, sin, self.scaling, attention_mask,
+                              getattr(self, "_smt_joint_qkv_grad", False))
+    o = o.reshape(*input_shape, -1).contiguous()
+    return self.o_proj(o), None
 
 
 def flash_attention(q, k, v, scale=None, key_mask: "KeyMask" = None, joint: bool = False):
@@ -708,7 +772,12 @@
         if "smt_prev_attn" not in _EAGER:
             _EAGER["smt_prev_attn"] = cfg._attn_implementation
         cfg._attn_implementation = register_attention()
-        counts["attention"] = sum(1 for m in model.modules() if isinstance(m, ml.LlamaAttention))
+        for m in model.modules():
+            if isinstance(m, ml.LlamaAttention):
+                counts["attention"] += 1
+                if "_smt_prev_attn_forward" not in m.__dict__:
+                    m.__dict__["_smt_prev_attn_forward"] = m.forward
+                    m.forward = fused_attention_forward.__get__(m, type(m))
     for m in model.modules():
         if isinstance(m, ml.LlamaRMSNorm):
             m.forward = fused_rmsnorm_forward.__get__(m, type(m))
@@ -743,3 +812,8 @@
             if isinstance(m, (ml.LlamaRMSNorm, ml.LlamaMLP, ml.LlamaDecoderLayer)) and "forward" in m.__dict__:
                 del m.__dict__["forward"]
             m.__dict__.pop("_smt_next_layer", None)
+            if "_smt_prev_attn_forward" in m.__dict__:
+                prev = m.__dict__.pop("_smt_prev_attn_forward")
+                m.__dict__.pop("forward", None)
+                if getattr(prev, "__func__", None) is not type(m).forward:
+                    m.forward = prev
```

Result: no change. 39910, median of 6 (+0.4%).
